# team-attention/nobs-whisper

Measured on AMD Instinct MI355X. Metric: audio-sec/s (RTF⁻¹) large-v3 greedy, batch 128; 1/2/4/8 MI355X, higher is better.
Workload: dtype bf16

## Files before the change

### include/whisper_mi355x.h

```cpp
#ifndef WHISPER_MI355X_H
#define WHISPER_MI355X_H

#include "whisper.h"

#ifdef __cplusplus
extern "C" {
#endif

#define WHISPER_MI355X_ERR_RUNTIME (-10)

enum whisper_mi355x_dtype { WHISPER_MI355X_F16 = 0, WHISPER_MI355X_BF16 = 1, WHISPER_MI355X_FP8_ENC = 2 };

WHISPER_API struct whisper_context * whisper_mi355x_init(const char * path_model, struct whisper_context_params params,
                                                         int dtype, bool load_weights);

WHISPER_API int whisper_mi355x_weight_arena(struct whisper_context * ctx, void ** dev_ptr, size_t * bytes);

WHISPER_API int whisper_mi355x_rccl_unique_id(char out[128]);
WHISPER_API int whisper_mi355x_broadcast_weights(struct whisper_context * ctx, const char unique_id[128], int rank, int world);

WHISPER_API int whisper_mi355x_full_batch(struct whisper_context * ctx, struct whisper_state * state,
                                          struct whisper_full_params params, const float * const * pcm,
                                          const int * n_samples, int n_jobs, bool pcm_on_device, int fixed_tokens);
WHISPER_API int whisper_mi355x_full_batch_forced(struct whisper_context * ctx, struct whisper_state * state,
                                                 struct whisper_full_params params, const float * const * pcm,
                                                 const int * n_samples, int n_jobs, bool pcm_on_device, int fixed_tokens,
                                                 const int * forced, const int * spot, int n_spot, float * spot_logits);
#define WHISPER_MI355X_BEAM_COMPLETED 1
#define WHISPER_MI355X_BEAM_FAILED 2
#define WHISPER_MI355X_BEAM_WINNER 4
WHISPER_API int whisper_mi355x_beam_info(struct whisper_state * state, int job, int beam, int * tokens, int cap,
                                         double * sum_logprobs_all, int * flags);
WHISPER_API int whisper_mi355x_cand_info(struct whisper_state * state, int job, int cand, int * tokens, int cap,
                                         double * sum_logprobs_all, int * flags);
WHISPER_API void whisper_mi355x_set_sample_seed(struct whisper_state * state, uint64_t seed);
WHISPER_API int whisper_mi355x_batch_n_segments(struct whisper_state * state, int job);
WHISPER_API const char * whisper_mi355x_batch_segment_text(struct whisper_state * state, int job, int i_segment);
WHISPER_API int64_t whisper_mi355x_batch_segment_t0(struct whisper_state * state, int job, int i_segment);
WHISPER_API int64_t whisper_mi355x_batch_segment_t1(struct whisper_state * state, int job, int i_segment);
WHISPER_API int whisper_mi355x_batch_segment_n_tokens(struct whisper_state * state, int job, int i_segment);
WHISPER_API whisper_token_data whisper_mi355x_batch_token_data(struct whisper_state * state, int job, int i_segment, int i_token);
WHISPER_API bool whisper_mi355x_batch_segment_speaker_turn_next(struct whisper_state * state, int job, int i_segment);
WHISPER_API int whisper_mi355x_batch_lang_id(struct whisper_state * state, int job);
WHISPER_API long whisper_mi355x_batch_decoded_tokens(struct whisper_state * state);
WHISPER_API long whisper_mi355x_decoded_tokens_total(void);
WHISPER_API void * whisper_mi355x_debug_ws(struct whisper_state * state, int which);

struct whisper_mi355x_window_decision {
    int32_t seek;
    int32_t temp_idx;
    int32_t failed0;
    int32_t logprob_fail0;
    int32_t result_len0;
    int32_t no_speech;
    float   avg_logprob0;
    float   entropy0;
    float   no_speech_prob;
    float   pad;
};
WHISPER_API int whisper_mi355x_window_decisions(struct whisper_state * state, int job,
                                                struct whisper_mi355x_window_decision * out, int cap);

WHISPER_API int whisper_mi355x_full_parallel(struct whisper_context * ctx, struct whisper_state * state,
                                             struct whisper_full_params params, const float * pcm, int n_samples,
                                             int n_processors, int snap_ms, bool pcm_on_device);
WHISPER_API int whisper_mi355x_parallel_cuts(struct whisper_state * state, int * cuts, int cap);

WHISPER_API int whisper_mi355x_phase_ms(struct whisper_state * state, double out[5]);

WHISPER_API double whisper_mi355x_align_ms(struct whisper_state * state);
WHISPER_API int whisper_mi355x_align_cost(struct whisper_state * state, int job, float * out, long cap_floats,
                                          int * rows, int * frames);

WHISPER_API double whisper_mi355x_token_times_ms(struct whisper_state * state);
struct whisper_mi355x_token_span {
    int64_t t0, t1;
    int32_t is_text, pad;
};
WHISPER_API int whisper_mi355x_debug_signal_energy(struct whisper_context * ctx, const float * pcm, const int * n_samples,
                                                   int n_clips, float * energy_out);
WHISPER_API int whisper_mi355x_debug_token_vad(struct whisper_context * ctx, const float * energy, const int * n_samples,
                                               int n_clips, const int * seg_clip, const int * seg_n_tokens, int n_segs,
                                               struct whisper_mi355x_token_span * spans);

WHISPER_API int whisper_mi355x_get_mel(struct whisper_state * state, float * out, int cap_floats);
WHISPER_API int whisper_mi355x_get_encoder_out(struct whisper_state * state, float * out, int cap_floats);
WHISPER_API int whisper_mi355x_set_audio_ctx(struct whisper_state * state, int audio_ctx);

WHISPER_API int whisper_mi355x_kernel_timing(struct whisper_state * state, int class_mask);
WHISPER_API int whisper_mi355x_kernel_stats(struct whisper_state * state, int cls, double out[3]);
#define WHISPER_MI355X_KSTAT_PDEC_GIVE_UPS 100
WHISPER_API long whisper_mi355x_pdec_give_ups(struct whisper_state * state);
#define WHISPER_MI355X_KSTAT_BEAM_GATHER 101
#define WHISPER_MI355X_KSTAT_VAD_FRONTEND 102
#define WHISPER_MI355X_KSTAT_VAD_LSTM 103
#define WHISPER_MI355X_KSTAT_VAD_GATHER 104
#define WHISPER_MI355X_KSTAT_LOGITS_STAGE 105

WHISPER_API int whisper_mi355x_debug_gemm(struct whisper_context * ctx, int epi, const void * A, int M, int K,
                                          const void * B, int N, const float * bias, void * out, int reps, float * ms);
WHISPER_API void whisper_mi355x_set_gemm_variant(int variant);
WHISPER_API void whisper_mi355x_set_gemm_stamps(void * dev);
WHISPER_API int whisper_mi355x_debug_gemm_small(struct whisper_context * ctx, int epi, const void * A, int M, int K,
                                                const void * B, int N, const float * bias, void * out,
                                                const float * ln_w, const float * ln_b, int reps, float * ms);
WHISPER_API int whisper_mi355x_debug_dequant(struct whisper_context * ctx, int type, const void * qs, const void * qh,
                                             const void * dm, long rows, int K, void * out);
WHISPER_API int whisper_mi355x_debug_dequant_multi(struct whisper_context * ctx, const int * type, int n,
                                                   const void * const * qs, const void * const * qh,
                                                   const void * const * dm, const long * rows, const int * K,
                                                   void * const * out);
WHISPER_API int whisper_mi355x_debug_gemm_small_q(struct whisper_context * ctx, int epi, const void * A, int M, int K,
                                                  int type, const void * qs, const void * qh, const void * dm, int N,
                                                  const float * bias, float scale, void * out, const float * ln_w,
                                                  const float * ln_b);
WHISPER_API void whisper_mi355x_set_dec_splits(int splits);
WHISPER_API void whisper_mi355x_set_dec_bm(int rows);
WHISPER_API void whisper_mi355x_set_pdec_spin(long ticks);
WHISPER_API void whisper_mi355x_set_pdec_stamps(void * dev);
WHISPER_API void whisper_mi355x_set_pdec_blocks(int on);
WHISPER_API int whisper_mi355x_debug_gemm_fp8(struct whisper_context * ctx, int epi, const void * A8,
                                              const float * a_scale, int M, int K, const void * B8,
                                              const float * b_scale, int N, const float * bias, void * out,
                                              int reps, float * ms);
WHISPER_API int whisper_mi355x_debug_gemm_w8(struct whisper_context * ctx, int epi, const void * A, int M, int K,
                                             const void * B8, const float * b_scale, int N, const float * bias,
                                             void * out, const float * ln_w, const float * ln_b, void * y);
WHISPER_API int whisper_mi355x_debug_quant_fp8(struct whisper_context * ctx, const void * x, long rows, int K,
                                               void * q, float * s);
WHISPER_API int whisper_mi355x_debug_attn_encoder(struct whisper_context * ctx, const void * qkv, int B, int T, int d,
                                                  int H, int variant, void * out, int reps, float * ms);
WHISPER_API int whisper_mi355x_debug_gemm_ln(struct whisper_context * ctx, const void * A, int M, int K,
                                             const void * B, int N, const float * bias, float * x,
                                             const float * ln_w, const float * ln_b, void * y, int reps, float * ms);

WHISPER_API int whisper_mi355x_debug_xattn(struct whisper_context * ctx, const void * enc, const int * slot,
                                           const void * q, const void * wkt, const void * wv, const float * bv,
                                           int n, int n_ctx, int d, float scale, int splits, float rescale_thr,
                                           void * out, int reps, float * ms);

WHISPER_API int whisper_mi355x_debug_attn_self_step(struct whisper_context * ctx, const float * slabs, int splits,
                                                    const float * bias, float scale, void * cache, const int * slot,
                                                    const int * pos, int n, int L, int layer, int H, int n_ctx,
                                                    void * out);
WHISPER_API int whisper_mi355x_debug_attn_cross_step(struct whisper_context * ctx, const float * slabs, int splits,
                                                     const float * bias, float scale, const void * cache,
                                                     const int * slot, const int * n_kv, int n, int L, int layer,
                                                     int H, int n_ctx, void * out);
WHISPER_API int whisper_mi355x_debug_attn_prefill(struct whisper_context * ctx, const void * q, int q_stride,
                                                  const void * cache, const int * slot, const int * n_kv,
                                                  const void * tiles, int n_tiles, int L, int layer, int H, int n_ctx,
                                                  void * out);

struct whisper_mi355x_cand {
    int32_t id, tid;
    float   p, plog, pt, ptsum, no_speech_prob, pad;
};
WHISPER_API int whisper_mi355x_debug_logits_topk(struct whisper_context * ctx, const float * logits, int n,
                                                 const int * rules, const float * temperature, int k, int split,
                                                 struct whisper_mi355x_cand * cand, struct whisper_mi355x_cand * greedy);
WHISPER_API int whisper_mi355x_debug_kv_gather(struct whisper_context * ctx, void * cache, int n_slots, int L, int H,
                                               int n_ctx, const int * copies, int n_copies, int * n_staged);

WHISPER_API int whisper_mi355x_debug_sample(struct whisper_context * ctx, const float * probs,
                                            const struct whisper_mi355x_cand * rec_in, int n, int n_vocab, uint64_t seed,
                                            const int * counters, const uint32_t * words, struct whisper_mi355x_cand * rec_out);

struct whisper_mi355x_seq_ctl {
    int32_t is_initial, last_ts, penult_ts, has_ts, seek_delta;
    float   temperature;
    int32_t suppress_blank, no_timestamps, suppress_eot, tid0_initial;
    int32_t want_probs, want_nosp;
};
WHISPER_API int whisper_mi355x_debug_logits(struct whisper_context * ctx, const float * logits, int n,
                                            const struct whisper_mi355x_seq_ctl * ctl, int form,
                                            struct whisper_mi355x_cand * out, float * probs);
WHISPER_API int whisper_mi355x_debug_decode_advance(struct whisper_context * ctx, int n, int ct, int beg,
                                                    const struct whisper_mi355x_cand * tout, int * ints,
                                                    struct whisper_mi355x_seq_ctl * ctl, const unsigned * err,
                                                    struct whisper_mi355x_cand * ring, unsigned * ring_err);

WHISPER_API int  whisper_mi355x_suppress_mask(struct whisper_context * ctx, bool suppress_nst, const char * regex,
                                              uint32_t * words, int cap_words);
WHISPER_API long whisper_mi355x_suppress_builds(struct whisper_context * ctx);
WHISPER_API int whisper_mi355x_debug_logits_deny(struct whisper_context * ctx, const float * logits, int n,
                                                 const struct whisper_mi355x_seq_ctl * ctl, int form,
                                                 struct whisper_mi355x_cand * out, float * probs, const uint32_t * deny);
WHISPER_API int whisper_mi355x_debug_logits_topk_deny(struct whisper_context * ctx, const float * logits, int n,
                                                      const int * rules, const float * temperature, int k, int split,
                                                      struct whisper_mi355x_cand * cand, struct whisper_mi355x_cand * greedy,
                                                      const uint32_t * deny);

WHISPER_API int whisper_mi355x_grammar_mask(struct whisper_context * ctx, const whisper_grammar_element ** rules,
                                            size_t n_rules, size_t i_start, const whisper_token * accepted_tokens,
                                            int n_accepted, uint32_t * words, int cap_words);
struct whisper_mi355x_grammar_stats { long rows_device, rows_patched, rows_host; double kernel_ms; long kernel_launches; };
WHISPER_API int whisper_mi355x_grammar_stats(struct whisper_state * state, struct whisper_mi355x_grammar_stats * out);
WHISPER_API int whisper_mi355x_debug_grammar_reject(struct whisper_context * ctx, const whisper_grammar_element ** rules,
                                                    size_t n_rules, size_t i_start, const whisper_token * accepted_tokens,
                                                    const int * n_accepted, int n_rows, uint32_t * words, int * flags);
WHISPER_API int whisper_mi355x_debug_logits_gram(struct whisper_context * ctx, const float * logits, int n,
                                                 const struct whisper_mi355x_seq_ctl * ctl, int form,
                                                 struct whisper_mi355x_cand * out, float * probs, const uint32_t * deny,
                                                 const uint32_t * gram, float penalty);
WHISPER_API int whisper_mi355x_debug_logits_topk_gram(struct whisper_context * ctx, const float * logits, int n,
                                                      const int * rules, const float * temperature, int k, int split,
                                                      struct whisper_mi355x_cand * cand, struct whisper_mi355x_cand * greedy,
                                                      const uint32_t * deny, const uint32_t * gram, float penalty);

WHISPER_API int whisper_mi355x_debug_logits_stage(struct whisper_context * ctx, const float * logits, int n,
                                                  const struct whisper_mi355x_seq_ctl * ctl, int flags, float * out_rows);
WHISPER_API int whisper_mi355x_debug_logits_ex(struct whisper_context * ctx, const float * raw, const float * filtered, int n,
                                               const struct whisper_mi355x_seq_ctl * ctl, int form, int flags,
                                               struct whisper_mi355x_cand * out, float * probs);
WHISPER_API int whisper_mi355x_debug_logits_topk_ex(struct whisper_context * ctx, const float * raw, const float * filtered,
                                                    int n, const struct whisper_mi355x_seq_ctl * ctl, int k, int split,
                                                    int flags, struct whisper_mi355x_cand * cand,
                                                    struct whisper_mi355x_cand * greedy);

struct whisper_vad_context;
WHISPER_API double whisper_mi355x_vad_ms(struct whisper_state * state);
WHISPER_API int whisper_mi355x_vad_map(struct whisper_state * state, int job, int * out, int cap);
WHISPER_API int whisper_mi355x_vad_probs_batch(struct whisper_vad_context * vctx, const float * const * pcm,
                                               const int * n_samples, int n_clips, bool pcm_on_device, float * probs_out,
                                               int * n_probs);
WHISPER_API int whisper_mi355x_debug_vad_frontend(struct whisper_vad_context * vctx, const float * pcm, int n_samples,
                                                  float * xg_out);
WHISPER_API int whisper_mi355x_debug_vad_gather(struct whisper_context * ctx, const float * const * pcm,
                                                const int * n_samples, int n_clips, const int * pieces,
                                                const int * n_pieces, float * out);

WHISPER_API int whisper_mi355x_debug_align_scores(struct whisper_context * ctx, const void * q, const void * cross,
                                                  int n_slots, int n_clips, const int * slot, const int * n_rows,
                                                  const int * frames, int n_heads, const int * head_layer,
                                                  const int * head_idx, float * P);
WHISPER_API int whisper_mi355x_debug_align_cost(struct whisper_context * ctx, const float * P, int n_clips,
                                                const int * n_rows, const int * n_sot, const int * frames, int n_heads,
                                                float * cost);
WHISPER_API int whisper_mi355x_debug_align_dtw(struct whisper_context * ctx, const float * cost, int n_clips,
                                               const int * rows, const int * frames, int * fr, int * path,
                                               int * path_len);

WHISPER_API int whisper_mi355x_find_silence_boundaries(int device, const float * const * pcm, const int * n_samples,
                                                       int n_clips, int sample_rate, bool pcm_on_device, int * counts,
                                                       int * boundaries, int cap, float * noise_floor, float * rms_out,
                                                       int rms_stride);
WHISPER_API int whisper_mi355x_resample_len(int n_in, int rate_in);
WHISPER_API int whisper_mi355x_resample_chunk(int device, const float * const * audio, const int * n_in, int n_clips,
                                              int rate_in, bool on_device, float * const * out);
WHISPER_API int whisper_mi355x_resample_operator(int rate_in, int * fsi, int * fso, float * W, long cap);

WHISPER_API int whisper_mi355x_abi_layout(size_t out[8]);

WHISPER_API int whisper_mi355x_state_info(struct whisper_state * state, int out[5]);

WHISPER_API void * whisper_mi355x_state_stream(struct whisper_state * state);

WHISPER_API void * whisper_mi355x_dev_alloc(struct whisper_context * ctx, size_t bytes);
WHISPER_API void   whisper_mi355x_dev_free(struct whisper_context * ctx, void * p);
WHISPER_API int    whisper_mi355x_memcpy(struct whisper_context * ctx, void * dst, const void * src, size_t bytes, int kind);

#ifdef __cplusplus
}
#endif

#endif
```

### nobs-whisper_amd/csrc/capi.cpp

```cpp
#include <cfloat>
#include <cmath>
#include <cstring>
#include <string>
#include <thread>
#include <vector>

#include <rccl/rccl.h>

#include "../../include/whisper_mi355x.h"
#include "engine.h"
#include "suppress.h"

namespace wm { extern int g_gemm_variant; extern int g_dec_splits; extern int g_dec_bm; extern unsigned long long* g_gemm_stamps; }
using namespace wm;

static Context* C(whisper_context* ctx) { return ctx ? &ctx->c : nullptr; }

template <typename F> static int guarded(whisper_state* s, F&& f) {
    try {
        return f();
    } catch (const wm::Error&) {
    } catch (const std::bad_alloc&) {
        fprintf(stderr, "whisper_mi355x: host out of memory\n");
    }
    if (s) recover_state(s);
    return WHISPER_MI355X_ERR_RUNTIME;
}

struct HookStream {
    hipStream_t st = nullptr;
    HookStream() { WM_CHECK(hipStreamCreate(&st)); }
    ~HookStream() { hipStreamDestroy(st); }
};
struct HookBufs {
    std::vector<void*> p;
    void* get(size_t bytes) {
        void* q = nullptr;
        WM_CHECK(hipMalloc(&q, bytes));
        p.push_back(q);
        return q;
    }
    ~HookBufs() { for (void* q : p) hipFree(q); }
};
struct HookEvent {
    hipEvent_t e = nullptr;
    HookEvent() { WM_CHECK(hipEventCreate(&e)); }
    ~HookEvent() { hipEventDestroy(e); }
};
template <typename F> static float timed_ms(hipStream_t st, int reps, bool warm, F run) {
    HookEvent e0, e1;
    if (warm) run();
    WM_CHECK(hipEventRecord(e0.e, st));
    for (int r = 0; r < reps; r++) run();
    WM_CHECK(hipEventRecord(e1.e, st));
    WM_CHECK(hipStreamSynchronize(st));
    float t = 0;
    WM_CHECK(hipEventElapsedTime(&t, e0.e, e1.e));
    return reps > 0 ? t / reps : 0.0f;
}

static DType env_dtype(DType def) {
    const char* e = getenv("WHISPER_MI355X_DTYPE");
    if (!e) return def;
    return (strcmp(e, "bf16") == 0 || strcmp(e, "BF16") == 0) ? DType::BF16 : DType::F16;
}

static whisper_context* make_ctx(const char* path, whisper_context_params cp, int dtype, bool load) {
    int n_dev = 0;
    if (hipGetDeviceCount(&n_dev) != hipSuccess || n_dev == 0) {
        fprintf(stderr, "whisper_mi355x: no HIP device available (this engine has no CPU path)\n");
        return nullptr;
    }
    const int dev = cp.gpu_device >= 0 && cp.gpu_device < n_dev ? cp.gpu_device : 0;
    whisper_context* w = new whisper_context();
    w->c.fp8_enc = dtype == 2;
    if (dtype == 2) dtype = (int)DType::BF16;
    bool ok = false;
    try {
        ok = load_context(&w->c, path, dev, (DType)dtype, load);
    } catch (const wm::Error&) {
    } catch (const std::bad_alloc&) {
    }
    if (!ok) {
        free_context(&w->c);
        delete w;
        return nullptr;
    }
    if (w->c.quant && w->c.fp8_enc) {
        fprintf(stderr, "whisper_mi355x: fp8 mode needs an f16 model file; %s is block-quantized, fp8 off\n", path);
        w->c.fp8_enc = false;
    }
    if (!resolve_dtw(&w->c, cp)) {
        free_context(&w->c);
        delete w;
        return nullptr;
    }
    w->c.owner = w;
    return w;
}

extern "C" {

const char* whisper_version(void) { return "1.7.6-mi355x"; }

struct whisper_context_params whisper_context_default_params(void) {
    whisper_context_params r;
    memset(&r, 0, sizeof(r));
    r.use_gpu = true;
    r.flash_attn = false;
    r.gpu_device = 0;
    r.dtw_token_timestamps = false;
    r.dtw_aheads_preset = WHISPER_AHEADS_NONE;
    r.dtw_n_top = -1;
    r.dtw_aheads.n_heads = 0;
    r.dtw_aheads.heads = nullptr;
    r.dtw_mem_size = 1024 * 1024 * 128;
    return r;
}
struct whisper_context_params* whisper_context_default_params_by_ref(void) {
    return new whisper_context_params(whisper_context_default_params());
}
void whisper_free_context_params(struct whisper_context_params* p) { delete p; }

struct whisper_full_params whisper_full_default_params(enum whisper_sampling_strategy strategy) {
    whisper_full_params r;
    memset(&r, 0, sizeof(r));
    r.strategy = strategy;
    r.n_threads = std::min(4, (int)std::thread::hardware_concurrency());
    r.n_max_text_ctx = 16384;
    r.offset_ms = 0;
    r.duration_ms = 0;
    r.translate = false;
    r.no_context = true;
    r.no_timestamps = false;
    r.single_segment = false;
    r.print_special = false;
    r.print_progress = true;
    r.print_realtime = false;
    r.print_timestamps = true;
    r.token_timestamps = false;
    r.thold_pt = 0.01f;
    r.thold_ptsum = 0.01f;
    r.max_len = 0;
    r.split_on_word = false;
    r.max_tokens = 0;
    r.debug_mode = false;
    r.audio_ctx = 0;
    r.tdrz_enable = false;
    r.suppress_regex = nullptr;
    r.initial_prompt = nullptr;
    r.prompt_tokens = nullptr;
    r.prompt_n_tokens = 0;
    r.language = "en";
    r.detect_language = false;
    r.suppress_blank = true;
    r.suppress_nst = false;
    r.temperature = 0.0f;
    r.max_initial_ts = 1.0f;
    r.length_penalty = -1.0f;
    r.temperature_inc = 0.2f;
    r.entropy_thold = 2.4f;
    r.logprob_thold = -1.0f;
    r.no_speech_thold = 0.6f;
    r.greedy.best_of = -1;
    r.beam_search.beam_size = -1;
    r.beam_search.patience = -1.0f;
// ... 266 lines not shown
float whisper_full_get_token_p_from_state(struct whisper_state* s, int i, int t) { return tdata(seg(s, 0, i), t).p; }
float whisper_full_get_token_p(struct whisper_context* ctx, int i, int t) { return tdata(seg(ctx->c.default_state, 0, i), t).p; }
float whisper_full_get_segment_no_speech_prob_from_state(struct whisper_state* s, int i) { auto g = seg(s, 0, i); return g ? g->no_speech_prob : 0.0f; }
float whisper_full_get_segment_no_speech_prob(struct whisper_context* ctx, int i) { return whisper_full_get_segment_no_speech_prob_from_state(ctx->c.default_state, i); }

int whisper_bench_memcpy(int) { return 0; }
const char* whisper_bench_memcpy_str(int) { return "whisper_mi355x: memcpy benchmark not implemented\n"; }
int whisper_bench_ggml_mul_mat(int) { return 0; }
const char* whisper_bench_ggml_mul_mat_str(int) { return "whisper_mi355x: ggml mul_mat benchmark not applicable (no ggml)\n"; }
void whisper_log_set(ggml_log_callback, void*) {}

struct whisper_context* whisper_mi355x_init(const char* path, struct whisper_context_params p, int dtype, bool load) {
    return make_ctx(path, p, dtype, load);
}
int whisper_mi355x_weight_arena(struct whisper_context* ctx, void** ptr, size_t* bytes) {
    if (!ctx) return -1;
    *ptr = ctx->c.arena;
    *bytes = ctx->c.arena_bytes;
    return 0;
}
int whisper_mi355x_rccl_unique_id(char out[128]) {
    ncclUniqueId id;
    if (ncclGetUniqueId(&id) != ncclSuccess) return -1;
    static_assert(sizeof(id) == 128, "ncclUniqueId size");
    memcpy(out, &id, 128);
    return 0;
}
int whisper_mi355x_broadcast_weights(struct whisper_context* ctx, const char uid[128], int rank, int world) {
    if (!ctx) return -1;
    if (world <= 1) return 0;
    hipSetDevice(ctx->c.device);
    ncclUniqueId id;
    memcpy(&id, uid, 128);
    ncclComm_t comm;
    if (ncclCommInitRank(&comm, world, id, rank) != ncclSuccess) return -2;
    hipStream_t st = nullptr;
    ncclResult_t r = ncclInternalError;
    const int rc = guarded(nullptr, [&] {
        WM_CHECK(hipStreamCreate(&st));
        r = ncclBroadcast(ctx->c.arena, ctx->c.arena, ctx->c.arena_bytes, ncclChar, 0, comm, st);
        WM_CHECK(hipStreamSynchronize(st));
        return 0;
    });
    if (st) hipStreamDestroy(st);
    ncclCommDestroy(comm);
    if (rc != 0) return rc;
    return r == ncclSuccess ? 0 : -3;
}

int whisper_mi355x_full_batch(struct whisper_context* ctx, struct whisper_state* s, struct whisper_full_params p,
                              const float* const* pcm, const int* n, int n_jobs, bool on_device, int fixed_tokens) {
    if (!ctx || !s || n_jobs <= 0 || fixed_tokens > ctx->c.hp.n_text_ctx / 2 - 4) return -1;
    FullOpts o;
    o.fixed_tokens = fixed_tokens;
    return guarded(s, [&] { return full_batch(&ctx->c, s, p, pcm, n, n_jobs, on_device, o, false); });
}
int whisper_mi355x_full_batch_forced(struct whisper_context* ctx, struct whisper_state* s, struct whisper_full_params p,
                                     const float* const* pcm, const int* n, int n_jobs, bool on_device, int fixed_tokens,
                                     const int* forced, const int* spot, int n_spot, float* spot_logits) {
    if (!ctx || !s || n_jobs <= 0 || fixed_tokens <= 0 || fixed_tokens > ctx->c.hp.n_text_ctx / 2 - 4 || !forced || n_spot < 0 ||
        (n_spot && (!spot || !spot_logits)))
        return -1;
    for (int k = 0; k < n_spot; k++)
        if (spot[k] < 0 || spot[k] >= n_jobs) return -1;
    FullOpts o;
    o.fixed_tokens = fixed_tokens;
    o.forced = forced;
    o.spot = spot;
    o.n_spot = n_spot;
    o.spot_logits = spot_logits;
    return guarded(s, [&] { return full_batch(&ctx->c, s, p, pcm, n, n_jobs, on_device, o, false); });
}
int whisper_mi355x_beam_info(struct whisper_state* s, int job, int beam, int* tokens, int cap, double* sum_logprobs_all,
                             int* flags) {
    if (!s || job < 0 || job >= (int)s->beam_info.size() || beam < 0 || beam >= (int)s->beam_info[job].size()) return -1;
    const whisper_state::BeamRec& r = s->beam_info[job][beam];
    for (int i = 0; tokens && i < cap && i < (int)r.tokens.size(); i++) tokens[i] = r.tokens[i];
    if (sum_logprobs_all) *sum_logprobs_all = r.sum_logprobs_all;
    if (flags) *flags = r.flags;
    return (int)r.tokens.size();
}
int whisper_mi355x_cand_info(struct whisper_state* s, int job, int cand, int* tokens, int cap, double* sum_logprobs_all,
                             int* flags) {
    if (!s || job < 0 || job >= (int)s->cand_info.size() || cand < 0 || cand >= (int)s->cand_info[job].size()) return -1;
    const whisper_state::BeamRec& r = s->cand_info[job][cand];
    for (int i = 0; tokens && i < cap && i < (int)r.tokens.size(); i++) tokens[i] = r.tokens[i];
    if (sum_logprobs_all) *sum_logprobs_all = r.sum_logprobs_all;
    if (flags) *flags = r.flags;
    return (int)r.tokens.size();
}
void whisper_mi355x_set_sample_seed(struct whisper_state* s, uint64_t seed) {
    if (s) s->sample_seed = seed;
}
int whisper_mi355x_batch_n_segments(struct whisper_state* s, int job) {
    return s && job >= 0 && job < (int)s->results.size() ? (int)s->results[job].size() : 0;
}
const char* whisper_mi355x_batch_segment_text(struct whisper_state* s, int job, int i) { auto g = seg(s, job, i); return g ? g->text.c_str() : nullptr; }
int64_t whisper_mi355x_batch_segment_t0(struct whisper_state* s, int job, int i) { auto g = seg(s, job, i); return g ? g->t0 : 0; }
int64_t whisper_mi355x_batch_segment_t1(struct whisper_state* s, int job, int i) { auto g = seg(s, job, i); return g ? g->t1 : 0; }
int whisper_mi355x_batch_segment_n_tokens(struct whisper_state* s, int job, int i) { auto g = seg(s, job, i); return g ? (int)g->tokens.size() : 0; }
whisper_token_data whisper_mi355x_batch_token_data(struct whisper_state* s, int job, int i, int t) { return tdata(seg(s, job, i), t); }
bool whisper_mi355x_batch_segment_speaker_turn_next(struct whisper_state* s, int job, int i) { auto g = seg(s, job, i); return g && g->speaker_turn_next; }
int whisper_mi355x_batch_lang_id(struct whisper_state* s, int job) {
    return s && job >= 0 && job < (int)s->lang_ids.size() ? s->lang_ids[job] : -1;
}
long whisper_mi355x_batch_decoded_tokens(struct whisper_state* s) { return s ? s->decoded_tokens : 0; }
int whisper_mi355x_window_decisions(struct whisper_state* s, int job, struct whisper_mi355x_window_decision* out, int cap) {
    if (!s || job < 0 || job >= (int)s->decisions.size()) return 0;
    const auto& d = s->decisions[job];
    if ((int)d.size() > cap) return -(int)d.size();
    for (size_t i = 0; i < d.size(); i++) out[i] = d[i];
    return (int)d.size();
}
int whisper_mi355x_phase_ms(struct whisper_state* s, double out[5]) {
    if (!s) return -1;
    for (int i = 0; i < 5; i++) out[i] = s->phase_ms[i];
    return 0;
}
double whisper_mi355x_align_ms(struct whisper_state* s) { return s ? s->align_ms : 0.0; }
int whisper_mi355x_align_cost(struct whisper_state* s, int job, float* out, long cap, int* rows, int* frames) {
    return guarded(nullptr, [&]() -> int {
        if (!s || job < 0 || job >= (int)s->align_info.size()) return -1;
        const whisper_state::AlignInfo& a = s->align_info[job];
        if (rows) *rows = a.rows;
        if (frames) *frames = a.frames;
        if (a.rows <= 0 || !a.cost) return 0;
        const long n = (long)a.rows * a.frames;
        if (!out || cap < n) return -2;
        hipSetDevice(s->device);
        WM_CHECK(hipMemcpy(out, a.cost, (size_t)n * sizeof(float), hipMemcpyDeviceToHost));
        return 0;
    });
}
int whisper_mi355x_get_mel(struct whisper_state* s, float* out, int cap) {
    return guarded(nullptr, [&]() -> int {
        if (!s || !s->ctx || !s->ws.mel) return -1;
        Context* c = s->ctx;
        const int nm = c->hp.n_mels, nl = s->n_len;
        if ((long)nm * nl > cap) return -nm * nl;
        hipSetDevice(c->device);
        int n_samp = 0;
        WM_CHECK(hipMemcpy(&n_samp, s->ws.n_samp, sizeof(int), hipMemcpyDeviceToHost));
        float* tmp;
        WM_CHECK(hipMalloc((void**)&tmp, (size_t)nm * nl * 4));
        launch_mel_normalize(s->ws.mel, nl, n_samp, s->ws.mel_max, nm, tmp, s->stream);
        WM_CHECK(hipMemcpyAsync(out, tmp, (size_t)nm * nl * 4, hipMemcpyDeviceToHost, s->stream));
        WM_CHECK(hipStreamSynchronize(s->stream));
        WM_CHECK(hipFree(tmp));
        return nl;
    });
}
int whisper_mi355x_get_encoder_out(struct whisper_state* s, float* out, int cap) {
    return guarded(nullptr, [&]() -> int {
        if (!s || !s->ctx || !s->ws.hn || s->last_enc_windows < 1) return -1;
        Context* c = s->ctx;
        const long n = (long)enc_ctx(c, s) * c->hp.n_audio_state;
        if (n > cap) return -1;
        hipSetDevice(c->device);
        std::vector<uint16_t> h(n);
        WM_CHECK(hipMemcpy(h.data(), s->ws.hn, n * 2, hipMemcpyDeviceToHost));
        for (long i = 0; i < n; i++) {
            if (c->dt == DType::F16) out[i] = h2f(h[i]);
            else { uint32_t u = (uint32_t)h[i] << 16; memcpy(&out[i], &u, 4); }
        }
        return 0;
    });
}
int whisper_mi355x_set_audio_ctx(struct whisper_state* s, int audio_ctx) {
    if (!s || !s->ctx) return -1;
    if (audio_ctx > s->ctx->hp.n_audio_ctx) return -5;
    s->audio_ctx = audio_ctx;
    return 0;
}
int whisper_mi355x_state_info(struct whisper_state* s, int out[5]) {
    if (!s || !out) return -1;
    out[0] = s->direct ? 1 : 0;
    out[1] = s->ws.cap_jobs;
    out[2] = s->ws.cap_cross;
    out[3] = (int)s->dec_graphs.size();
    out[4] = s->pooled ? 1 : 0;
    return 5;
}
void* whisper_mi355x_state_stream(struct whisper_state* s) { return s ? (void*)s->stream : nullptr; }
int whisper_mi355x_kernel_timing(struct whisper_state* s, int class_mask) {
    if (!s) return -1;
    s->ktime_mask = class_mask;
    for (auto& k : s->kstat) k = KStat();
    for (auto& k : s->vad_kstat) k = KStat();
    return 0;
}
int whisper_mi355x_kernel_stats(struct whisper_state* s, int cls, double out[3]) {
    if (s && cls == WHISPER_MI355X_KSTAT_PDEC_GIVE_UPS) {
        out[0] = s->pdec_lost_ms;
        out[1] = (double)s->pdec_give_ups;
        out[2] = 0.0;
        return 0;
    }
    if (s && cls == WHISPER_MI355X_KSTAT_BEAM_GATHER && s->ctx) {
        const Hparams& hp = s->ctx->hp;
        const double row_bytes = (double)hp.n_text_layer * 2 * hp.n_text_head * 128;
        out[0] = s->gather_rows * row_bytes;
        out[1] = s->gather_rows_full * row_bytes;
        out[2] = 0.0;
        return 0;
    }
    if (s && cls >= WHISPER_MI355X_KSTAT_VAD_FRONTEND && cls <= WHISPER_MI355X_KSTAT_VAD_GATHER) {
        const KStat& k = s->vad_kstat[cls - WHISPER_MI355X_KSTAT_VAD_FRONTEND];
        out[0] = k.ms; out[1] = (double)k.count; out[2] = k.work;
        return 0;
    }
    if (cls == WHISPER_MI355X_KSTAT_LOGITS_STAGE) cls = K_LOGITS_STAGE;
    if (!s || cls < 0 || cls >= K_NCLASS) return -1;
    out[0] = s->kstat[cls].ms;
    out[1] = (double)s->kstat[cls].count;
    out[2] = s->kstat[cls].work;
    return 0;
}

void whisper_mi355x_set_gemm_variant(int v) { wm::g_gemm_variant = v; }
void whisper_mi355x_set_gemm_stamps(void* dev) { wm::g_gemm_stamps = (unsigned long long*)dev; }
void whisper_mi355x_set_dec_splits(int splits) { wm::g_dec_splits = splits; }
void whisper_mi355x_set_dec_bm(int rows) { wm::g_dec_bm = rows; }
void whisper_mi355x_set_pdec_spin(long ticks) {
    wm::g_pdec_spin_ticks = ticks;
    wm::g_pdec_gen.fetch_add(1, std::memory_order_release);
}
void whisper_mi355x_set_pdec_stamps(void* dev) {
    wm::g_pdec_stamps = (unsigned long long*)dev;
    wm::g_pdec_gen.fetch_add(1, std::memory_order_release);
}
void* whisper_mi355x_debug_ws(struct whisper_state* s, int which) {
    if (!s) return nullptr;
    const wm::Workspace& w = s->ws;
    void* p[9] = {w.dx, w.dh, nullptr, w.datt, w.dff, w.dq, w.qx, w.xo, w.xml};
    return which >= 0 && which < 9 ? p[which] : nullptr;
}
long whisper_mi355x_decoded_tokens_total(void) { return wm::g_decoded_tokens_total.load(); }
long whisper_mi355x_pdec_give_ups(struct whisper_state* s) { return s ? s->pdec_give_ups : wm::g_pdec_give_ups_total.load(); }
void whisper_mi355x_set_pdec_blocks(int on) { wm::g_pdec_blocks = on != 0; }
int whisper_mi355x_debug_gemm(struct whisper_context* ctx, int epi, const void* A, int M, int K, const void* B, int N,
                              const float* bias, void* out, int reps, float* ms) {
    return guarded(nullptr, [&]() -> int {
        if (!ctx) return -1;
        const int T = ctx->c.hp.n_audio_ctx;
        if (epi == EPI_CROSSKV && (M % T != 0 || K % 64 != 0 || N % (2 * K) != 0)) return -1;
        hipSetDevice(ctx->c.device);
        HookBufs b;
        HookStream hs;
        GemmArgs g = gemm_plain(A, M, K, B, N, bias, out, N);
        if (M <= 128) {
            g.splitk_ws_elems = 64L * M * N;
            g.splitk_ws = (float*)b.get(g.splitk_ws_elems * sizeof(float));
        }
        if (epi == EPI_CROSSKV) {
            std::vector<int> slots(M / T);
            for (int i = 0; i < M / T; i++) slots[i] = i;
            int* dslot = (int*)b.get(slots.size() * sizeof(int));
            WM_CHECK(hipMemcpy(dslot, slots.data(), slots.size() * sizeof(int), hipMemcpyHostToDevice));
            g.cache = out; g.row_slot = dslot; g.d = K; g.H = K / 64; g.ctx = T; g.L = N / (2 * K); g.layer = 0;
        }
        const float t = timed_ms(hs.st, reps, true, [&] { launch_gemm(ctx->c.dt, epi, g, hs.st); });
        if (ms) *ms = t;
        return 0;
    });
}
int whisper_mi355x_debug_gemm_small(struct whisper_context* ctx, int epi, const void* A, int M, int K, const void* B,
                                    int N, const float* bias, void* out, const float* ln_w, const float* ln_b, int reps,
                                    float* ms) {
    return guarded(nullptr, [&]() -> int {
        if (!ctx || !gemm_small_ok(M, K, ln_w != nullptr)) return -1;
        hipSetDevice(ctx->c.device);
        HookStream hs;
        GemmArgs g = gemm_plain(A, M, K, B, N, bias, out, N);
        g.a_ln_w = ln_w; g.a_ln_b = ln_b;
        const float t = timed_ms(hs.st, reps, true, [&] { launch_gemm_small(ctx->c.dt, epi, g, ln_w != nullptr, hs.st); });
        if (ms) *ms = t;
        return 0;
    });
}
static bool debug_qmat(QMat* q, int type, const void* qs, const void* qh, const void* dm) {
    const bool known = type == 2 || type == 3 || type == 6 || type == 7 || type == 8;
    if (!known || !qs || !dm || ((type == 6 || type == 7) && !qh)) return false;
    q->type = type;
    q->qs = (const uint8_t*)qs;
    q->qh = (const uint32_t*)qh;
    q->dm = (const uint16_t*)dm;
    return true;
}
int whisper_mi355x_debug_dequant(struct whisper_context* ctx, int type, const void* qs, const void* qh, const void* dm,
                                 long rows, int K, void* out) {
    return guarded(nullptr, [&]() -> int {
        QMat q;
        if (!ctx || !out || rows < 1 || K < 1 || !debug_qmat(&q, type, qs, qh, dm)) return -1;
        hipSetDevice(ctx->c.device);
        launch_dequant(ctx->c.dt, q, rows, K, out, nullptr);
        WM_CHECK(hipDeviceSynchronize());
        return 0;
    });
}
int whisper_mi355x_debug_dequant_multi(struct whisper_context* ctx, const int* type, int n, const void* const* qs,
                                       const void* const* qh, const void* const* dm, const long* rows, const int* K,
                                       void* const* out) {
    return guarded(nullptr, [&]() -> int {
        if (!ctx || !type || !qs || !qh || !dm || !rows || !K || !out || n < 1 || n > 6) return -1;
        DequantJobs J;
        J.n = n;
        for (int j = 0; j < n; j++) {
            if (!out[j] || rows[j] < 1 || K[j] < 1 || !debug_qmat(&J.q[j], type[j], qs[j], qh[j], dm[j])) return -1;
            J.rows[j] = rows[j];
            J.K[j] = K[j];
            J.out[j] = out[j];
        }
        hipSetDevice(ctx->c.device);
        launch_dequant_multi(ctx->c.dt, J, nullptr);
        WM_CHECK(hipDeviceSynchronize());
        return 0;
    });
}
int whisper_mi355x_debug_gemm_small_q(struct whisper_context* ctx, int epi, const void* A, int M, int K, int type,
                                      const void* qs, const void* qh, const void* dm, int N, const float* bias,
                                      float scale, void* out, const float* ln_w, const float* ln_b) {
    return guarded(nullptr, [&]() -> int {
        QMat q;
        if (!ctx || !A || !out || N < 1 || !gemm_small_ok(M, K, ln_w != nullptr) || (ln_w && !ln_b) ||
            !debug_qmat(&q, type, qs, qh, dm))
            return -1;
        hipSetDevice(ctx->c.device);
        HookStream hs;
        GemmArgs g = gemm_plain(A, M, K, nullptr, N, bias, out, N);
        g.q = q;
        g.sc_div = N; g.sc_mod = 1; g.sc_lim = 1; g.scale = scale;
        g.a_ln_w = ln_w; g.a_ln_b = ln_b;
        launch_gemm_small(ctx->c.dt, epi, g, ln_w != nullptr, hs.st);
        WM_CHECK(hipStreamSynchronize(hs.st));
        return 0;
    });
}
int whisper_mi355x_debug_gemm_fp8(struct whisper_context* ctx, int epi, const void* A8, const float* a_scale, int M,
                                  int K, const void* B8, const float* b_scale, int N, const float* bias, void* out,
                                  int reps, float* ms) {
    return guarded(nullptr, [&]() -> int {
        if (!ctx) return -1;
        hipSetDevice(ctx->c.device);
        HookStream hs;
        const GemmArgs g = gemm_plain(A8, M, K, B8, N, bias, out, N);
        const float t = timed_ms(hs.st, reps, true, [&] { launch_gemm_fp8(ctx->c.dt, epi, g, a_scale, b_scale, hs.st); });
        if (ms) *ms = t;
        return 0;
    });
}
int whisper_mi355x_debug_gemm_w8(struct whisper_context* ctx, int epi, const void* A, int M, int K, const void* B8,
                                 const float* b_scale, int N, const float* bias, void* out, const float* ln_w,
                                 const float* ln_b, void* y) {
    return guarded(nullptr, [&]() -> int {
        if (!ctx || !b_scale || M < 1 || M > 128 || K % 64 || (epi == EPI_RESID && (!ln_w || !y))) return -1;
        hipSetDevice(ctx->c.device);
        HookBufs b;
        HookStream hs;
        GemmArgs g = gemm_plain(A, M, K, B8, N, bias, out, N);
        g.w8_scale = b_scale;
        if (epi == EPI_RESID) { g.ln_w = ln_w; g.ln_b = ln_b; g.ln_out = y; }
        g.splitk_ws_elems = 16L * M * N;
        g.splitk_ws = (float*)b.get(g.splitk_ws_elems * sizeof(float));
        launch_gemm(ctx->c.dt, epi, g, hs.st);
        WM_CHECK(hipStreamSynchronize(hs.st));
        return 0;
    });
}
int whisper_mi355x_debug_quant_fp8(struct whisper_context* ctx, const void* x, long rows, int K, void* q, float* s) {
    return guarded(nullptr, [&]() -> int {
        if (!ctx) return -1;
        hipSetDevice(ctx->c.device);
        launch_quant_rows_fp8(ctx->c.dt, x, rows, K, q, s, nullptr);
        WM_CHECK(hipDeviceSynchronize());
        return 0;
// ... 862 lines not shown
```

### nobs-whisper_amd/csrc/engine.cpp

```cpp
#include <optional>
#include <algorithm>
#include <chrono>
#include <cmath>
#include <cstring>
#include <exception>
#include <thread>

#include "engine.h"
#include "suppress.h"
#include "token_times.h"

namespace wm {

static size_t esize(DType) { return 2; }

static void dfree(void*& p) {
    if (p) { void* q = p; p = nullptr; WM_CHECK(hipFree(q)); }
}
template <typename T> static void dfree(T*& p) {
    void* q = (void*)p;
    p = nullptr;
    dfree(q);
}
template <typename T> static void dalloc(T*& p, size_t bytes) {
    void* q = nullptr;
    p = nullptr;
    WM_CHECK(hipMalloc(&q, bytes));
    p = (T*)q;
}

static hipEvent_t kt_event(whisper_state* s) {
    if (!s->kpool.empty()) { hipEvent_t e = s->kpool.back(); s->kpool.pop_back(); return e; }
    hipEvent_t e;
    WM_CHECK(hipEventCreate(&e));
    return e;
}
static void kt_record(whisper_state* s, hipEvent_t e, hipStream_t st) {
    if (!s->capture_ev) { WM_CHECK(hipEventRecord(e, st)); return; }
    hipStreamCaptureStatus cs;
    unsigned long long id = 0;
    hipGraph_t g = nullptr;
    const hipGraphNode_t* deps = nullptr;
    size_t nd = 0;
    WM_CHECK(hipStreamGetCaptureInfo_v2(st, &cs, &id, &g, &deps, &nd));
    hipGraphNode_t node;
    WM_CHECK(hipGraphAddEventRecordNode(&node, g, deps, nd, e));
    WM_CHECK(hipStreamUpdateCaptureDependencies(st, &node, 1, hipStreamSetCaptureDependencies));
}
struct KT {
    whisper_state* s;
    int cls;
    double work;
    hipStream_t st;
    hipEvent_t a = nullptr;
    int sub = 0;
    KT(whisper_state* s_, int c, double w, hipStream_t st_ = nullptr, bool on = true)
        : s(s_), cls(c), work(w), st(st_ ? st_ : s_->stream) {
        if (on && ((s->ktime_mask >> c) & 1)) { a = kt_event(s); kt_record(s, a, st); }
    }
    ~KT() {
        if (!a) return;
        hipEvent_t b = kt_event(s);
        kt_record(s, b, st);
        (s->capture_ev ? *s->capture_ev : s->kpending).push_back({cls, a, b, work, sub});
    }
};
static void drop_graphs(whisper_state* s) {
    for (auto& g : s->dec_graphs) {
        hipGraphExecDestroy(g.exec);
        for (auto& e : g.ev) { hipEventDestroy(e.a); hipEventDestroy(e.b); }
    }
    s->dec_graphs.clear();
}
static void kt_flush_graph(whisper_state* s, const whisper_state::DecGraph& g) {
    for (auto& p : g.ev) {
        if (!((s->ktime_mask >> p.cls) & 1)) continue;
        float ms = 0.0f;
        const hipError_t e = hipEventElapsedTime(&ms, p.a, p.b);
        if (e != hipSuccess) {
            static bool warned = false;
            if (!warned) fprintf(stderr, "whisper_mi355x: graph kernel timing unavailable (%s)\n", hipGetErrorString(e));
            warned = true;
            continue;
        }
        s->kstat[p.cls].ms += ms;
        s->kstat[p.cls].work += p.cls == K_ATTN_SELF ? s->cur_self_work * p.work : p.work;
        s->kstat[p.cls].count++;
    }
}
void kt_flush(whisper_state* s) {
    if (s->kpending.empty()) return;
    WM_CHECK(hipStreamSynchronize(s->stream));
    for (auto& p : s->kpending) {
        float ms = 0.0f;
        WM_CHECK(hipEventElapsedTime(&ms, p.a, p.b));
        s->kstat[p.cls].ms += ms;
        s->kstat[p.cls].work += p.cls == K_ATTN_SELF ? s->cur_self_work * p.work : p.work;
        s->kstat[p.cls].count++;
        if (p.cls == K_VAD) {
            s->vad_kstat[p.sub].ms += ms;
            s->vad_kstat[p.sub].work += p.work;
            s->vad_kstat[p.sub].count++;
        }
        s->kpool.push_back(p.a);
        s->kpool.push_back(p.b);
    }
    s->kpending.clear();
}
static void tgemm_ws(whisper_state* s, int cls, DType dt, int epi, const GemmArgs& g0, hipStream_t st, float* ws,
                     long ws_elems) {
    GemmArgs g = g0;
    if (cls == K_GEMM_DEC) { g.splitk_ws = ws; g.splitk_ws_elems = ws_elems; g.slab_wt = 1; }
    const double work = cls == K_GEMM_ENC ? 2.0 * g.M * g.N * g.K
                                          : 2.0 * g.N * g.K + 2.0 * g.M * g.K + 4.0 * g.M * g.N;
    KT kt(s, cls, work, st);
    launch_gemm(dt, epi, g, st);
}
static void tgemm(whisper_state* s, int cls, DType dt, int epi, const GemmArgs& g0, hipStream_t st) {
    tgemm_ws(s, cls, dt, epi, g0, st, s->ws.splitk, s->ws.splitk_elems);
}

static whisper_state* create_state(Context* c) {
    WM_CHECK(hipSetDevice(c->device));
    whisper_state* s = new whisper_state();
    s->ctx = c;
    s->device = c->device;
    try {
        WM_CHECK(hipStreamCreateWithFlags(&s->stream, hipStreamNonBlocking));
        WM_CHECK(hipStreamCreateWithFlags(&s->stream2, hipStreamNonBlocking));
        WM_CHECK(hipEventCreateWithFlags(&s->ev_fork, hipEventDisableTiming));
        WM_CHECK(hipEventCreateWithFlags(&s->ev_join, hipEventDisableTiming));
    } catch (...) {
        if (s->ev_join) hipEventDestroy(s->ev_join);
        if (s->ev_fork) hipEventDestroy(s->ev_fork);
        if (s->stream2) hipStreamDestroy(s->stream2);
        if (s->stream) hipStreamDestroy(s->stream);
        delete s;
        throw;
    }
    std::lock_guard<std::mutex> lk(c->pool_mu);
    c->live.push_back(s);
    return s;
}

static void reset_for_reuse(whisper_state* s) {
    s->direct = false;
    s->results.clear();
    s->lang_ids.clear();
    s->decisions.clear();
    s->prompt_past.clear();
    s->rng = std::mt19937(0);
    s->lang_id = 0;
    s->audio_ctx = 0;
    s->n_len = s->n_len_org = 0;
    s->logits_host.clear();
    for (double& t : s->phase_ms) t = 0;
    s->align_ms = 0;
    s->tokts_ms = 0;
    s->vad_ms = 0;
    s->vad_maps.clear();
    s->align_info.clear();
    s->decoded_tokens = 0;
    s->last_enc_windows = 0;
    s->mel_ready = false;
    s->ktime_mask = 0;
    for (auto& k : s->kstat) k = KStat();
    for (auto& k : s->vad_kstat) k = KStat();
    s->cur_self_work = 0;
    s->pdec_give_ups = 0;
    s->pdec_lost_ms = 0;
    s->pdec_off_until = 0;
    s->pdec_off = false;
    s->mode = StepMode{};
    s->deny_on = false;
    s->gram_on = false;
    s->filter_on = s->tdrz_on = false;
    s->ws.gd.host_masks.clear();
    s->ws.gd.rows_device = s->ws.gd.rows_patched = s->ws.gd.rows_host = 0;
    s->beam_info.clear();
    s->sample_seed = 0;
    s->cand_info.clear();
    s->gather_rows = s->gather_rows_full = 0;
    std::fill(s->ws.cross_fresh.begin(), s->ws.cross_fresh.end(), 0);
}

static int pool_states() {
    const char* e = getenv("WHISPER_MI355X_STATE_POOL");
    return e ? std::max(0, atoi(e)) : 2;
}
static const int kPoolMaxJobs = 16;

whisper_state* new_state(Context* c) {
    {
        std::lock_guard<std::mutex> lk(c->pool_mu);
        if (!c->pool.empty()) {
            whisper_state* s = c->pool.back();
            c->pool.pop_back();
            reset_for_reuse(s);
            s->pooled = true;
            return s;
        }
    }
    return create_state(c);
}

static void free_ws(Workspace& w);

static void destroy_state(whisper_state* s) {
    if (s->twin) {
        destroy_state(s->twin);
        s->twin = nullptr;
    }
    if (Context* c = s->ctx) {
        std::lock_guard<std::mutex> lk(c->pool_mu);
        c->live.erase(std::remove(c->live.begin(), c->live.end(), s), c->live.end());
    }
    hipSetDevice(s->device);
    hipStreamSynchronize(s->stream);
    hipStreamSynchronize(s->stream2);
    drop_graphs(s);
    try { free_ws(s->ws); } catch (const Error&) {}
    for (auto& p : s->kpending) { hipEventDestroy(p.a); hipEventDestroy(p.b); }
    for (hipEvent_t e : s->kpool) hipEventDestroy(e);
    hipEventDestroy(s->ev_fork);
    hipEventDestroy(s->ev_join);
    hipStreamDestroy(s->stream2);
    hipStreamDestroy(s->stream);
    delete s;
}

void free_state(whisper_state* s) {
    if (!s) return;
    Context* c = s->ctx;
    if (!c) {
        destroy_state(s);
        return;
    }
    hipSetDevice(c->device);
    const bool healthy = hipStreamSynchronize(s->stream) == hipSuccess && hipStreamSynchronize(s->stream2) == hipSuccess &&
                         s->kpending.empty();
    if (healthy && s->ws.cap_jobs <= kPoolMaxJobs) {
        std::lock_guard<std::mutex> lk(c->pool_mu);
        if ((int)c->pool.size() < pool_states()) {
            c->pool.push_back(s);
            return;
        }
    }
    destroy_state(s);
}

void drain_state_pool(Context* c) {
    std::vector<whisper_state*> p;
    {
        std::lock_guard<std::mutex> lk(c->pool_mu);
        p.swap(c->pool);
    }
    for (whisper_state* s : p) destroy_state(s);
}

void orphan_states(Context* c) {
    std::lock_guard<std::mutex> lk(c->pool_mu);
    for (whisper_state* s : c->live) s->ctx = nullptr;
    c->live.clear();
}

void recover_state(whisper_state* s) {
    if (!s) return;
    hipSetDevice(s->device);
    for (hipStream_t st : {s->stream, s->stream2}) {
        hipStreamCaptureStatus cs = hipStreamCaptureStatusNone;
        if (hipStreamIsCapturing(st, &cs) == hipSuccess && cs != hipStreamCaptureStatusNone) {
            hipGraph_t g = nullptr;
            hipStreamEndCapture(st, &g);
            if (g) hipGraphDestroy(g);
        }
    }
    s->capture_ev = nullptr;
    s->mode = StepMode{};
    hipStreamSynchronize(s->stream);
    hipStreamSynchronize(s->stream2);
    (void)hipGetLastError();
    for (auto& p : s->kpending) { s->kpool.push_back(p.a); s->kpool.push_back(p.b); }
    s->kpending.clear();
}

static void free_align(Workspace& w) {
    dfree(w.al_clips); dfree(w.al_P); dfree(w.al_stats); dfree(w.al_cost); dfree(w.al_trace); dfree(w.al_fr);
    if (w.h_al) { char* q = w.h_al; w.h_al = nullptr; WM_CHECK(hipHostFree(q)); }
    w.al_P_elems = 0;
    w.al_cap = w.al_rows = 0;
}

static void free_ws(Workspace& w) {
    free_align(w);
    dfree(w.mel_img); dfree(w.h1); dfree(w.hn); dfree(w.qkv); dfree(w.att); dfree(w.ff); dfree(w.x);
    dfree(w.cross); dfree(w.self); dfree(w.dx); dfree(w.dh); dfree(w.dq); dfree(w.datt); dfree(w.dff);
    dfree(w.lrow); dfree(w.logits); dfree(w.probs); dfree(w.tok); dfree(w.ctl); dfree(w.tout); dfree(w.lrec); dfree(w.win_job);
    dfree(w.pcm); dfree(w.mel); dfree(w.mel_ptrs); dfree(w.splitk); dfree(w.enc); dfree(w.qx); dfree(w.xo);
    dfree(w.xml); dfree(w.kvslot); dfree(w.hs); dfree(w.qtiles); dfree(w.wdq); dfree(w.pd_sync);
    dfree(w.sslot); dfree(w.cand); dfree(w.kvcp); dfree(w.kvstage); dfree(w.sctr);
    dfree(w.energy); dfree(w.tt_clips); dfree(w.tt_segs); dfree(w.tt_spans); dfree(w.deny); dfree(w.gram);
    if (w.h_gram) hipHostFree(w.h_gram);
    dfree(w.frows);
    if (w.h_frows) hipHostFree(w.h_frows);
    gram_dev_free(w.gd);
    vad_scratch_free(w.vad);
    if (w.h_sslot) hipHostFree(w.h_sslot);
    if (w.h_sctr) hipHostFree(w.h_sctr);
    if (w.h_cand) hipHostFree(w.h_cand);
    if (w.h_kvcp) hipHostFree(w.h_kvcp);
    if (w.h_pd_err) hipHostFree(w.h_pd_err);
    if (w.h_ring) hipHostFree(w.h_ring);
    for (auto& e : w.ring_ev)
        if (e) hipEventDestroy(e);
    if (w.h_ints) hipHostFree(w.h_ints);
    if (w.h_qtiles) hipHostFree(w.h_qtiles);
    if (w.h_tout) hipHostFree(w.h_tout);
    if (w.h_ctl) hipHostFree(w.h_ctl);
    w = Workspace();
}

static const int kXDirectMaxTok = 8;
static const float kXattnThr = 8.0f;

static bool pick_direct(Context* c, int n_jobs) {
    if (!c->cross_direct) return false;
    const char* e = getenv("WHISPER_MI355X_CROSS");
    if (e && strcmp(e, "direct") == 0) return true;
    if (e && strcmp(e, "cache") == 0) return false;
    return n_jobs > 32;
}

static int enc_batch() {
    static const int v = getenv("WHISPER_MI355X_ENC_BATCH") ? std::max(1, atoi(getenv("WHISPER_MI355X_ENC_BATCH"))) : 128;
    return v;
}

static void ensure_cross(Context* c, whisper_state* s, int slots) {
    Workspace& w = s->ws;
    if (w.cross && w.cap_cross >= slots) return;
    const Hparams& hp = c->hp;
    WM_CHECK(hipStreamSynchronize(s->stream));
    WM_CHECK(hipStreamSynchronize(s->stream2));
    drop_graphs(s);
    dfree(w.cross);
    w.cap_cross = 0;
    std::fill(w.cross_fresh.begin(), w.cross_fresh.end(), 0);
    dalloc(w.cross, (size_t)slots * hp.n_text_layer * 2 * hp.n_audio_ctx * hp.n_audio_state * esize(c->dt));
    w.cap_cross = slots;
}

static void ensure_ws_impl(Context* c, whisper_state* s, int n_jobs, int n_clips) {
    Workspace& w = s->ws;
    const Hparams& hp = c->hp;
    const size_t d = hp.n_audio_state, nm = hp.n_mels, T = hp.n_audio_ctx, E = esize(c->dt);
    const int n_enc = std::min(n_clips, enc_batch());
    if (n_enc > w.cap_enc || n_jobs > w.cap_jobs) drop_graphs(s);
    if (!w.deny) dalloc(w.deny, (size_t)suppress_words(hp.n_vocab) * sizeof(uint32_t));
    if (n_enc > w.cap_enc) {
        dfree(w.mel_img); dfree(w.h1); dfree(w.hn); dfree(w.qkv); dfree(w.att); dfree(w.ff); dfree(w.x);
        dfree(w.win_job); dfree(w.hs);
        w.cap_enc = 0;
        dalloc(w.mel_img, (size_t)n_enc * 3002 * nm * E);
        dalloc(w.h1, (size_t)n_enc * 3002 * d * E);
        WM_CHECK(hipMemset(w.h1, 0, (size_t)n_enc * 3002 * d * E));
        dalloc(w.hn, (size_t)n_enc * T * d * E);
        dalloc(w.qkv, (size_t)n_enc * T * 3 * d * E);
        dalloc(w.att, (size_t)n_enc * T * d * E);
        dalloc(w.ff, (size_t)n_enc * T * 4 * d * E);
        dalloc(w.x, (size_t)n_enc * T * d * 4);
        if (c->fp8_enc) {
            dalloc(w.hs, (size_t)n_enc * T * sizeof(float));
        }
        dalloc(w.win_job, (size_t)n_enc * 3 * sizeof(int));
        w.win_seek = w.win_job + n_enc;
        w.win_slot = w.win_job + 2 * n_enc;
        w.cap_enc = n_enc;
    }
    if (n_jobs > w.cap_jobs) {
        const int L = hp.n_text_layer;
        const int n_tok = n_jobs * (hp.n_text_ctx / 2 + 8);
        dfree(w.cross); dfree(w.self); dfree(w.dx); dfree(w.dh); dfree(w.dq); dfree(w.datt); dfree(w.dff);
        dfree(w.lrow); dfree(w.logits); dfree(w.probs); dfree(w.tok); dfree(w.ctl); dfree(w.tout); dfree(w.lrec); dfree(w.mel_ptrs);
        dfree(w.splitk); dfree(w.enc); dfree(w.qx); dfree(w.xo); dfree(w.xml); dfree(w.kvslot); dfree(w.qtiles);
        free_align(w);
        for (auto& a : s->align_info) a = {};
        if (w.h_ring) { WM_CHECK(hipHostFree(w.h_ring)); w.h_ring = nullptr; w.ring = nullptr; }
        dfree(w.sslot); dfree(w.cand); dfree(w.kvcp); dfree(w.sctr); dfree(w.gram);
        dfree(w.frows);
        for (void** h : {(void**)&w.h_qtiles, (void**)&w.h_ints, (void**)&w.h_tout, (void**)&w.h_ctl, (void**)&w.h_sslot,
                         (void**)&w.h_cand, (void**)&w.h_kvcp, (void**)&w.h_sctr, (void**)&w.h_gram, (void**)&w.h_frows})
            if (*h) { void* q = *h; *h = nullptr; WM_CHECK(hipHostFree(q)); }
        w.cap_jobs = w.cap_tok = w.cap_cross = w.cap_xq = 0;
        w.splitk_elems = std::max(16L * std::min(n_tok, 256) * 4 * (long)d, std::min(16384L * n_tok, 12L << 22));
        dalloc(w.splitk, w.splitk_elems * 4);
        w.cross_fresh.assign(n_jobs, 0);
        {
            std::vector<int> ident(n_jobs);
            for (int k = 0; k < n_jobs; k++) ident[k] = k;
            dalloc(w.kvslot, (size_t)n_jobs * sizeof(int));
            WM_CHECK(hipMemcpy(w.kvslot, ident.data(), (size_t)n_jobs * sizeof(int), hipMemcpyHostToDevice));
        }
        dalloc(w.self, (size_t)n_jobs * L * 2 * hp.n_text_ctx * d * E);
        dalloc(w.dx, (size_t)n_tok * d * 4);
        dalloc(w.dh, (size_t)n_tok * d * E);
        dalloc(w.dq, (size_t)n_tok * d * E);
        dalloc(w.datt, (size_t)n_tok * d * E);
        dalloc(w.dff, (size_t)n_tok * 4 * d * E);
        dalloc(w.lrow, (size_t)n_jobs * d * E);
        dalloc(w.logits, (size_t)n_jobs * hp.n_vocab * 4);
        dalloc(w.probs, (size_t)n_jobs * 2 * hp.n_vocab * 4);
        dalloc(w.tok, ((size_t)5 * n_tok + n_jobs) * sizeof(int));
        w.pos = w.tok + n_tok;
        w.slot = w.tok + 2 * n_tok;
        w.nkv_self = w.tok + 3 * n_tok;
        w.nkv_cross = w.tok + 4 * n_tok;
        w.lrows = w.tok + 5 * n_tok;
        dalloc(w.ctl, (size_t)n_jobs * sizeof(SeqCtl));
        dalloc(w.tout, (size_t)n_jobs * sizeof(TokOut));
        dalloc(w.lrec, logits_rec_bytes(n_jobs));
        dalloc(w.mel_ptrs, (size_t)n_jobs * (2 * sizeof(void*) + 3 * sizeof(int)));
        w.pcm_ptrs = (const float**)(w.mel_ptrs + n_jobs);
        w.n_samp = (int*)(w.pcm_ptrs + n_jobs);
        w.n_len = w.n_samp + n_jobs;
        w.mel_max = w.n_len + n_jobs;
        WM_CHECK(hipHostMalloc((void**)&w.h_ints, ((size_t)5 * n_tok + n_jobs) * sizeof(int) + 64, 0));
        dalloc(w.qtiles, (size_t)n_tok * sizeof(int2));
        WM_CHECK(hipHostMalloc((void**)&w.h_qtiles, (size_t)n_tok * sizeof(int2), 0));
        WM_CHECK(hipHostMalloc((void**)&w.h_tout, (size_t)n_jobs * sizeof(TokOut), 0));
        WM_CHECK(hipHostMalloc((void**)&w.h_ctl, (size_t)n_jobs * sizeof(SeqCtl), 0));
        dalloc(w.sslot, (size_t)n_jobs * sizeof(int));
        dalloc(w.cand, (size_t)n_jobs * kTopkMax * sizeof(TokOut));
        dalloc(w.kvcp, (size_t)n_jobs * sizeof(KvCopy));
        WM_CHECK(hipHostMalloc((void**)&w.h_sslot, (size_t)n_jobs * sizeof(int), 0));
        WM_CHECK(hipHostMalloc((void**)&w.h_cand, (size_t)n_jobs * kTopkMax * sizeof(TokOut), 0));
        WM_CHECK(hipHostMalloc((void**)&w.h_kvcp, (size_t)n_jobs * sizeof(KvCopy), 0));
        dalloc(w.sctr, (size_t)n_jobs * 4 * sizeof(int));
        WM_CHECK(hipHostMalloc((void**)&w.h_sctr, (size_t)n_jobs * 4 * sizeof(int), 0));
        dalloc(w.gram, (size_t)n_jobs * grammar_words(hp.n_vocab) * sizeof(uint32_t));
        WM_CHECK(hipHostMalloc((void**)&w.h_gram, (size_t)n_jobs * grammar_words(hp.n_vocab) * sizeof(uint32_t), 0));
        w.cap_jobs = n_jobs;
        w.cap_tok = n_tok;
    }
    if (s->direct && !w.enc) {
        const int H = hp.n_text_head;
        w.cap_xq = std::max(kXDirectMaxTok * w.cap_jobs, 128);
        const size_t xo_rows = (size_t)std::max(w.cap_xq, 512) + w.cap_jobs + 512;
        dalloc(w.enc, (size_t)w.cap_jobs * T * d * E);
        dalloc(w.qx, (size_t)w.cap_xq * 2 * H * d * E);
        dalloc(w.xo, xo_rows * H * d * 4);
        dalloc(w.xml, xo_rows * H * 2 * 4);
    }
    if (!s->direct) ensure_cross(c, s, n_clips);
    if (c->quant && !w.wdq) dalloc(w.wdq, (size_t)16 * d * d * E);
}

static void ensure_ws(Context* c, whisper_state* s, int n_jobs, int n_clips = -1) {
    try {
        ensure_ws_impl(c, s, n_jobs, n_clips < 0 ? n_jobs : n_clips);
    } catch (const Error&) {
        hipStreamSynchronize(s->stream);
        hipStreamSynchronize(s->stream2);
        drop_graphs(s);
        free_ws(s->ws);
        throw;
    }
}

static inline int mel_n_len(int n) { return (n + 16000 * 30) / 160; }
static inline int mel_n_len_org(int n) { return 1 + (int)(((int64_t)n + 200 - 400) / 160); }

int compute_mel(Context* c, whisper_state* s, const float* const* pcm, const int* n, int n_jobs, bool on_device) {
    s->direct = pick_direct(c, n_jobs);
    ensure_ws(c, s, n_jobs);
    Workspace& w = s->ws;
    const int nm = c->hp.n_mels;
    size_t pcm_tot = 0, mel_tot = 0;
    int max_frames = 1;
    for (int j = 0; j < n_jobs; j++) {
        pcm_tot += ((size_t)n[j] + 63) & ~(size_t)63;
        mel_tot += (size_t)nm * mel_n_len(n[j]);
        max_frames = std::max(max_frames, std::min((n[j] + 200) / 160 + 1, mel_n_len(n[j])));
    }
    if (!on_device && pcm_tot > w.cap_pcm) {
        dfree(w.pcm);
        w.cap_pcm = 0;
        dalloc(w.pcm, pcm_tot * 4);
        w.cap_pcm = pcm_tot;
    }
    if (mel_tot > w.cap_mel) {
        dfree(w.mel);
        w.cap_mel = 0;
        dalloc(w.mel, mel_tot * 4);
        w.cap_mel = mel_tot;
    }
    std::vector<const float*> pp(n_jobs);
    std::vector<float*> mp(n_jobs);
    std::vector<int> ints(3 * n_jobs);
    size_t po = 0, mo = 0;
    for (int j = 0; j < n_jobs; j++) {
        if (on_device) pp[j] = pcm[j];
        else {
            pp[j] = w.pcm + po;
            if (n[j] > 0) WM_CHECK(hipMemcpyAsync(w.pcm + po, pcm[j], (size_t)n[j] * 4, hipMemcpyHostToDevice, s->stream));
            po += ((size_t)n[j] + 63) & ~(size_t)63;
        }
        mp[j] = w.mel + mo;
        mo += (size_t)nm * mel_n_len(n[j]);
        ints[j] = n[j];
        ints[n_jobs + j] = mel_n_len(n[j]);
    }
    const size_t cap = w.cap_jobs;
    std::vector<char> blk(cap * (2 * sizeof(void*) + 2 * sizeof(int)));
    memcpy(blk.data(), mp.data(), n_jobs * sizeof(void*));
    memcpy(blk.data() + cap * sizeof(void*), pp.data(), n_jobs * sizeof(void*));
    memcpy(blk.data() + 2 * cap * sizeof(void*), ints.data(), n_jobs * sizeof(int));
    memcpy(blk.data() + 2 * cap * sizeof(void*) + cap * sizeof(int), ints.data() + n_jobs, n_jobs * sizeof(int));
    WM_CHECK(hipMemcpyAsync(w.mel_ptrs, blk.data(), blk.size(), hipMemcpyHostToDevice, s->stream));
    {
        double bytes = 0;
        for (int j = 0; j < n_jobs; j++)
            bytes += 4.0 * n[j] + 4.0 * nm * std::min((n[j] + 200) / 160 + 1, mel_n_len(n[j]));
        KT kt(s, K_MEL, bytes);
        launch_mel(w.pcm_ptrs, w.n_samp, c->w.mel_tab, c->w.filt_t, nm, w.mel_ptrs, w.n_len, w.mel_max, n_jobs, max_frames,
                   s->stream);
    }
    WM_CHECK(hipStreamSynchronize(s->stream));
    s->n_len = mel_n_len(n[0]);
    s->n_len_org = mel_n_len_org(n[0]);
    s->mel_ready = true;
    return 0;
}

template <typename T> static void tt_grow(T*& p, int& cap, size_t need) {
    if ((size_t)cap >= need) return;
    dfree(p);
// ... 58 lines not shown
        f.s2 = (float*)p; p += d * sizeof(float);
        launch_quant_rows_fp8(c->dt, L.wqkv, 3 * d, (int)d, f.wqkv, f.sqkv, nullptr);
        launch_quant_rows_fp8(c->dt, L.w1, 4 * d, (int)d, f.w1, f.s1, nullptr);
        launch_quant_rows_fp8(c->dt, L.w2, d, (int)(4 * d), f.w2, f.s2, nullptr);
    }
    c->dec8.assign(nd, Context::Fp8Dec{});
    for (size_t l = 0; l < nd; l++) {
        Context::Fp8Dec& f = c->dec8[l];
        const LayerW& L = c->w.dec[l];
        auto q = [&](const void* w, size_t rows, size_t cols, void*& q8, float*& sc) {
            q8 = p; p += rows * cols;
            sc = (float*)p; p += rows * sizeof(float);
            launch_quant_rows_fp8(c->dt, w, (long)rows, (int)cols, q8, sc, nullptr);
        };
        q(L.wqkv, 3 * t, t, f.wqkv, f.sqkv);
        q(L.wo, t, t, f.wo, f.so);
        q(L.wxq, t, t, f.wxq, f.sxq);
        q(L.wxo, t, t, f.wxo, f.sxo);
        q(L.w1, 4 * t, t, f.w1, f.s1);
        q(L.w2, t, 4 * t, f.w2, f.s2);
    }
    WM_CHECK(hipDeviceSynchronize());
    c->fp8_ready = true;
}

static void tgemm_fp8(whisper_state* s, int epi, const GemmArgs& g, const float* sa, const float* sb, hipStream_t st) {
    KT kt(s, K_GEMM_ENC, 2.0 * g.M * g.N * g.K, st);
    launch_gemm_fp8(s->ctx->dt, epi, g, sa, sb, st);
}

static int enc_gelu_epi(DType dt) { return dt == DType::BF16 ? EPI_GELU_F : EPI_GELU; }

using LayerMats = Context::LayerMats;
static char* dequant_layer(Context* c, const LayerW& L, char* p, LayerMats& m, hipStream_t st) {
    const int d = c->hp.n_audio_state;
    const size_t E = esize(c->dt);
    DequantJobs J;
    bool one_type = true;
    auto one = [&](const QMat& q, long rows, int K, const void*& dst) {
        if (!q.type) return;
        if (J.n && q.type != J.q[0].type) one_type = false;
        J.q[J.n] = q; J.rows[J.n] = rows; J.K[J.n] = K; J.out[J.n] = p; J.n++;
        dst = p;
        p += (size_t)rows * K * E;
    };
    one(L.qqkv, 3L * d, d, m.wqkv);
    one(L.qo, d, d, m.wo);
    one(L.qxq, d, d, m.wxq);
    one(L.qxo, d, d, m.wxo);
    one(L.q1, 4L * d, d, m.w1);
    one(L.q2, d, 4 * d, m.w2);
    if (one_type) launch_dequant_multi(c->dt, J, st);
    else
        for (int j = 0; j < J.n; j++) launch_dequant(c->dt, J.q[j], J.rows[j], J.K[j], J.out[j], st);
    return p;
}

static void ensure_expanded(Context* c, hipStream_t st) {
    if (!c->quant || c->expanded.load(std::memory_order_acquire)) return;
    hipStreamCaptureStatus cs = hipStreamCaptureStatusNone;
    WM_CHECK(hipStreamIsCapturing(st, &cs));
    if (cs != hipStreamCaptureStatusNone) return;
    std::lock_guard<std::mutex> lk(c->exp_mu);
    if (c->expanded.load(std::memory_order_relaxed)) return;
    const size_t d = c->hp.n_audio_state;
    dalloc(c->arena_exp, (12 * c->w.enc.size() + 14 * c->w.dec.size()) * d * d * esize(c->dt));
    char* p = c->arena_exp;
    auto fill = [&](const std::vector<LayerW>& layers, std::vector<LayerMats>& out) {
        out.resize(layers.size());
        for (size_t l = 0; l < layers.size(); l++) {
            const LayerW& L = layers[l];
            out[l] = LayerMats{L.wqkv, L.wo, L.wxq, L.wxo, L.w1, L.w2};
            p = dequant_layer(c, L, p, out[l], st);
        }
    };
    fill(c->w.enc, c->exp_enc);
    fill(c->w.dec, c->exp_dec);
    WM_CHECK(hipStreamSynchronize(st));
    c->expanded.store(true, std::memory_order_release);
}

static LayerMats layer_mats(Context* c, whisper_state* s, bool dec, int l, hipStream_t st) {
    const LayerW& L = dec ? c->w.dec[l] : c->w.enc[l];
    LayerMats m{L.wqkv, L.wo, L.wxq, L.wxo, L.w1, L.w2};
    if (!c->quant) return m;
    ensure_expanded(c, st);
    if (c->expanded.load(std::memory_order_acquire)) return dec ? c->exp_dec[l] : c->exp_enc[l];
    dequant_layer(c, L, (char*)s->ws.wdq, m, st);
    return m;
}

int encode_windows(Context* c, whisper_state* s, const int* jobs, const int* seeks, const int* slots, int n_win) {
    const Hparams& hp = c->hp;
    Workspace& w = s->ws;
    const int d = hp.n_audio_state, nm = hp.n_mels, T = enc_ctx(c, s), H = hp.n_audio_head;
    const DType dt = c->dt;
    const size_t E = esize(dt);
    const int KCLS = K_GEMM_ENC;
    const Weights& W = c->w;
    hipStream_t st = s->stream;
    const bool fp8 = c->fp8_enc && d % 128 == 0;
    if (fp8) ensure_fp8(c);
    for (int b0 = 0; b0 < n_win; b0 += w.cap_enc) {
        const int nb = std::min(w.cap_enc, n_win - b0);
        int* hi = w.h_ints;
        for (int i = 0; i < nb; i++) { hi[i] = jobs[b0 + i]; hi[nb + i] = seeks[b0 + i]; hi[2 * nb + i] = slots[b0 + i]; }
        WM_CHECK(hipMemcpyAsync(w.win_job, hi, 3 * nb * sizeof(int), hipMemcpyHostToDevice, st));
        const int* d_job = w.win_job;
        const int* d_seek = w.win_job + nb;
        const int* d_slot = w.win_job + 2 * nb;
        launch_mel_window(dt, w.mel_ptrs, w.n_len, w.n_samp, w.mel_max, d_job, d_seek, nb, nm, 2 * T, w.mel_img, st);
        {
            GemmArgs g = gemm_plain(w.mel_img, nb * 2 * T, 3 * nm, W.conv1_w, d, W.conv1_b, w.h1, d);
            g.a_rpb = 2 * T; g.a_bstride = (long)3002 * nm; g.a_rstride = nm;
            g.o_rpb = 2 * T; g.o_bstride = 3002; g.o_off = 1;
            tgemm(s, KCLS, dt, EPI_GELU, g, st);
        }
        {
            GemmArgs g = gemm_plain(w.h1, nb * T, 3 * d, W.conv2_w, d, W.conv2_b, w.x, d);
            g.a_rpb = T; g.a_bstride = (long)3002 * d; g.a_rstride = 2 * d;
            g.pos = W.pos_e; g.pos_rows = T;
            tgemm(s, KCLS, dt, EPI_GELU_POS, g, st);
        }
        const int M = nb * T;
        for (int l = 0; l < hp.n_audio_layer; l++) {
            const LayerW& L = W.enc[l];
            if (fp8) {
                const Context::Fp8Layer& F = c->enc8[l];
                launch_layernorm_fp8(w.x, M, d, L.ln1_w, L.ln1_b, w.hn, w.hs, st);
                tgemm_fp8(s, EPI_STORE, gemm_plain(w.hn, M, d, F.wqkv, 3 * d, L.bqkv, w.qkv, 3 * d), w.hs, F.sqkv, st);
                {
                    KT kt(s, K_ATTN_ENC, 4.0 * nb * H * (double)T * T * 64);
                    launch_attn_encoder(dt, w.qkv, w.att, nb, T, d, H, st);
                }
                tgemm(s, KCLS, dt, EPI_RESID, gemm_plain(w.att, M, d, L.wo, d, L.bo, w.x, d), st);
                launch_layernorm_fp8(w.x, M, d, L.ln2_w, L.ln2_b, w.hn, w.hs, st);
                tgemm_fp8(s, EPI_GELU_F, gemm_plain(w.hn, M, d, F.w1, 4 * d, L.b1, w.ff, 4 * d), w.hs, F.s1, st);
                launch_quant_rows_fp8(dt, w.ff, M, 4 * d, w.qkv, w.hs, st);
                tgemm_fp8(s, EPI_RESID, gemm_plain(w.qkv, M, 4 * d, F.w2, d, L.b2, w.x, d), w.hs, F.s2, st);
                continue;
            }
            const LayerMats Wm = layer_mats(c, s, false, l, st);
            launch_layernorm(dt, w.x, nullptr, M, d, L.ln1_w, L.ln1_b, w.hn, st);
            tgemm(s, KCLS, dt, EPI_STORE, gemm_plain(w.hn, M, d, Wm.wqkv, 3 * d, L.bqkv, w.qkv, 3 * d), st);
            {
                KT kt(s, K_ATTN_ENC, 4.0 * nb * H * (double)T * T * 64);
                launch_attn_encoder(dt, w.qkv, w.att, nb, T, d, H, st);
            }
            tgemm(s, KCLS, dt, EPI_RESID, gemm_plain(w.att, M, d, Wm.wo, d, L.bo, w.x, d), st);
            launch_layernorm(dt, w.x, nullptr, M, d, L.ln2_w, L.ln2_b, w.hn, st);
            tgemm(s, KCLS, dt, enc_gelu_epi(dt), gemm_plain(w.hn, M, d, Wm.w1, 4 * d, L.b1, w.ff, 4 * d), st);
            tgemm(s, KCLS, dt, EPI_RESID, gemm_plain(w.ff, M, 4 * d, Wm.w2, d, L.b2, w.x, d), st);
        }
        launch_layernorm(dt, w.x, nullptr, M, d, W.lnpost_w, W.lnpost_b, w.hn, st);
        if (s->direct) {
            for (int k = 0; k < nb; k++) {
                WM_CHECK(hipMemcpyAsync((char*)w.enc + (size_t)slots[b0 + k] * T * d * E, (const char*)w.hn + (size_t)k * T * d * E,
                                        (size_t)T * d * E, hipMemcpyDeviceToDevice, st));
                w.cross_fresh[slots[b0 + k]] = 0;
            }
        } else {
            GemmArgs g = gemm_plain(w.hn, M, d, W.wkv_cross, 2 * hp.n_text_layer * d, W.bkv_cross, nullptr, 0);
            g.scale = c->k_scale;
            g.cache = w.cross; g.row_slot = d_slot; g.L = hp.n_text_layer; g.H = hp.n_text_head; g.ctx = hp.n_audio_ctx; g.d = d;
            g.rpw = T;
            tgemm(s, KCLS, dt, EPI_CROSSKV, g, st);
            for (int k = 0; k < nb; k++) w.cross_fresh[slots[b0 + k]] = 1;
        }
        WM_CHECK(hipStreamSynchronize(st));
    }
    s->last_enc_windows = n_win;
    return 0;
}

static void decoder_upload(Context* c, whisper_state* s, int n_tok, int n_rows, bool tiles) {
    const Hparams& hp = c->hp;
    Workspace& w = s->ws;
    int* hi = w.h_ints;
    const int ct = w.cap_tok;
    double self_kv = 0;
    for (int i = 0; i < n_tok; i++) {
        hi[3 * ct + i] = hi[ct + i] + 1;
        hi[4 * ct + i] = enc_ctx(c, s);
        self_kv += hi[ct + i] + 1;
    }
    s->cur_self_work = self_kv * hp.n_text_head * 64 * 2 * 2;
    WM_CHECK(hipMemcpyAsync(w.tok, hi, ((size_t)5 * ct + n_rows) * sizeof(int), hipMemcpyHostToDevice, s->stream));
    if (!tiles) return;
    int nt = 0;
    for (int i = 0; i < n_tok; i++) {
        const bool cont = i > 0 && hi[2 * ct + i] == hi[2 * ct + i - 1] && hi[ct + i] > hi[ct + i - 1] &&
                          w.h_qtiles[nt - 1].y < 64;
        if (cont) w.h_qtiles[nt - 1].y++;
        else w.h_qtiles[nt++] = make_int2(i, 1);
    }
    w.n_qtiles = nt;
    WM_CHECK(hipMemcpyAsync(w.qtiles, w.h_qtiles, (size_t)nt * sizeof(int2), hipMemcpyHostToDevice, s->stream));
}

struct DecView {
    int r0, n;
    hipStream_t st;
    float* splitk;
    long splitk_elems;
    float *xo, *xml;
};

static int small_m_max() {
    const char* e = getenv("WHISPER_MI355X_SMALLM");
    if (!e) return 4;
    const int v = atoi(e);
    return v == 1 ? 32 : std::max(0, std::min(32, v));
}

static int quant_small_max() {
    const char* e = getenv("WHISPER_MI355X_QSMALL_MAX");
    return e ? atoi(e) : 32;
}

static int pdec_max() {
    const char* e = getenv("WHISPER_MI355X_PDEC");
    return e ? std::max(0, std::min(kPdecMaxRows, atoi(e))) : kPdecMaxRows;
}

static int small_rows_max(Context* c) { return c->quant ? std::max(quant_small_max(), small_m_max()) : small_m_max(); }

static bool dec_fp8(Context* c) { return c->fp8_enc && !c->dec8.empty(); }

static int dec_path_sig() {
    return small_m_max() | (std::min(std::max(quant_small_max(), 0), 1023) << 6) |
           (std::min(std::max(attn_cross_wide_max(), 0), 1023) << 16) | (pdec_max() << 26) | ((g_pdec_blocks & 1) << 29);
}

static bool pdec_blocks(Context* c) {
    return c->quant && (g_pdec_blocks || !c->expanded.load(std::memory_order_acquire));
}

static bool pdec_use(Context* c, whisper_state* s, int n, bool xdirect) {
    if (xdirect || s->pdec_off || s->mode.split_slots || n < 1 || n > pdec_max()) return false;
    if (dec_fp8(c)) return false;
    const bool quant = c->w.dec[0].qqkv.type != 0;
    for (const LayerW& L : c->w.dec)
        for (const QMat* q : {&L.qqkv, &L.qo, &L.qxq, &L.qxo, &L.q1, &L.q2})
            if ((q->type != 0) != quant) return false;
    const bool blocks = pdec_blocks(c);
    if (blocks && c->dt != DType::F16) return false;
    if (!pdec_supported(c->hp.n_text_state, c->hp.n_text_head, blocks)) return false;
    static const int cus = [] {
        int dev = 0, v = 0;
        hipGetDevice(&dev);
        hipDeviceGetAttribute(&v, hipDeviceAttributeMultiprocessorCount, dev);
        return v;
    }();
    return cus == 256;
}

static int dec_groups(int n_tok) { return cdiv(n_tok, 128); }

enum StepPath { STEP_PDEC, STEP_SMALL, STEP_SPLITK };
struct StepPlan {
    int n;
    int groups, gsz;
    StepPath path, tail_path;
    bool xdirect;
    bool w8;
    bool pdec_ok;
    bool pipe;
};
static StepPlan step_plan(Context* c, whisper_state* s, int n, bool xdirect, bool pdec_ok = true) {
    StepPlan P{};
    P.n = n; P.groups = dec_groups(n); P.gsz = cdiv(n, P.groups);
    P.xdirect = xdirect; P.w8 = dec_fp8(c); P.pdec_ok = pdec_ok;
    const int d = c->hp.n_text_state;
    const bool pd = pdec_ok && pdec_use(c, s, n, xdirect);
    auto path = [&](int rows) {
        if (pd) return STEP_PDEC;
        const bool small = !P.w8 && !s->mode.split_slots && rows <= small_rows_max(c) && gemm_small_ok(rows, d, true) &&
                           gemm_small_ok(rows, 4 * d, false);
        return small ? STEP_SMALL : STEP_SPLITK;
    };
    P.path = path(P.gsz);
    P.tail_path = P.groups == 1 ? P.path : path(n - (P.groups - 1) * P.gsz);
    return P;
}

static const PdecLayer* pdec_layers(Context* c, bool blocks) {
    std::lock_guard<std::mutex> lk(c->pdec_mu);
    void*& slot = blocks || !c->quant ? c->pdec_layers : c->pdec_layers_exp;
    if (!slot) {
        std::vector<PdecLayer> h(c->hp.n_text_layer);
        for (int l = 0; l < c->hp.n_text_layer; l++) {
            const LayerW& L = c->w.dec[l];
            LayerMats m{L.wqkv, L.wo, L.wxq, L.wxo, L.w1, L.w2};
            if (c->quant && !blocks) m = c->exp_dec[l];
            auto mat = [&](const void* w, const QMat& q) {
                return q.type && blocks ? PdecMat{q.qs, q.qh, q.dm, q.type} : PdecMat{w, nullptr, nullptr, 0};
            };
            h[l] = PdecLayer{mat(m.wqkv, L.qqkv), mat(m.wo, L.qo), mat(m.wxq, L.qxq), mat(m.wxo, L.qxo), mat(m.w1, L.q1),
                             mat(m.w2, L.q2), L.bqkv, L.bo, L.bxq, L.bxo, L.b1, L.b2,
                             L.ln1_w, L.ln1_b, L.lnx_w, L.lnx_b, L.ln2_w, L.ln2_b};
        }
        void* p = nullptr;
        WM_CHECK(hipMalloc(&p, h.size() * sizeof(PdecLayer)));
        WM_CHECK(hipMemcpy(p, h.data(), h.size() * sizeof(PdecLayer), hipMemcpyHostToDevice));
        slot = p;
    }
    return (const PdecLayer*)slot;
}

static void pdec_prepare(Context* c, whisper_state* s) {
    Workspace& w = s->ws;
    pdec_layers(c, pdec_blocks(c));
    if (w.pd_sync) return;
    dalloc(w.pd_sync, pdec_granules(c->hp.n_text_state, c->hp.n_text_layer, c->hp.n_text_head).bytes);
// ... 2455 lines not shown
```

### nobs-whisper_amd/csrc/engine.h

```cpp
#pragma once
#include <map>
#include <memory>
#include <atomic>
#include <cstring>
#include <mutex>
#include <random>
#include <string>
#include <unordered_map>
#include <vector>

#include "../../include/whisper_mi355x.h"
#include "beam.h"
#include "common.h"
#include "grammar.h"
#include "kernels.h"
#include "parallel.h"
#include "vad.h"

namespace wm {

struct Hparams {
    int32_t n_vocab, n_audio_ctx, n_audio_state, n_audio_head, n_audio_layer;
    int32_t n_text_ctx, n_text_state, n_text_head, n_text_layer, n_mels, ftype;
};
// ... 104 lines not shown
    GramTable gram_tab{};
    void* gram_tab_mem[4] = {nullptr, nullptr, nullptr, nullptr};
    std::mutex vad_mu;
    std::string vad_path;
    std::shared_ptr<VadModel> vad;
};

struct GramDev {
    GramElem* elems = nullptr;
    int* rule_off = nullptr;
    size_t cap_elems = 0, cap_rules = 0;
    GramRow *rows = nullptr, *h_rows = nullptr;
    unsigned *over = nullptr, *h_over = nullptr;
    int cap_rows = 0;
    std::unordered_map<std::string, std::vector<uint32_t>> host_masks;
    long rows_device = 0, rows_patched = 0, rows_host = 0;
};
void gram_dev_free(GramDev& d);
void gram_dev_rules(GramDev& d, const GrammarRules& g, hipStream_t st);
void gram_masks(Context* c, GramDev& d, const GrammarRules& g, const Grammar* const* states, int n, uint32_t* gram,
                uint32_t* h_stage, int* flags, hipStream_t st, whisper_state* s);

struct TokenData {
    int id, tid;
    float p, plog, pt, ptsum;
    int64_t t_dtw = -1;
    int64_t t0 = -1, t1 = -1;
    float vlen = 0.0f;
};
inline whisper_token_data token_data(const TokenData& x) {
    whisper_token_data r;
    memset(&r, 0, sizeof(r));
    r.id = x.id; r.tid = x.tid; r.p = x.p; r.plog = x.plog; r.pt = x.pt; r.ptsum = x.ptsum;
    r.t0 = x.t0; r.t1 = x.t1; r.t_dtw = x.t_dtw; r.vlen = x.vlen;
    return r;
}

struct Segment {
    int64_t t0, t1;
    std::string text;
    float no_speech_prob;
    std::vector<TokenData> tokens;
    bool speaker_turn_next = false;
};

struct Workspace {
    int cap_jobs = 0, cap_enc = 0, cap_tok = 0;
    int cap_cross = 0;
    size_t cap_mel = 0, cap_pcm = 0;
    void *mel_img = nullptr, *h1 = nullptr, *hn = nullptr, *qkv = nullptr, *att = nullptr, *ff = nullptr;
    float* x = nullptr;
    float* hs = nullptr;
    void *cross = nullptr, *self = nullptr;
    std::vector<char> cross_fresh;
    int* kvslot = nullptr;
    void* wdq = nullptr;
    void *enc = nullptr, *qx = nullptr;
    float *xo = nullptr, *xml = nullptr;
    int cap_xq = 0;
    float* dx = nullptr;
    void *dh = nullptr, *dq = nullptr, *datt = nullptr, *dff = nullptr, *lrow = nullptr;
    float *logits = nullptr, *probs = nullptr;
    float* splitk = nullptr;
    long splitk_elems = 0;
    int *tok = nullptr, *pos = nullptr, *slot = nullptr, *nkv_self = nullptr, *nkv_cross = nullptr, *lrows = nullptr;
    SeqCtl* ctl = nullptr;
    TokOut* tout = nullptr;
    void* lrec = nullptr;
    uint32_t* deny = nullptr;
    bool deny_held = false;
    Context::DenyKey deny_key;
    uint32_t* gram = nullptr;
    uint32_t* h_gram = nullptr;
    GramDev gd;
    float *frows = nullptr, *h_frows = nullptr;
    int *win_job = nullptr, *win_seek = nullptr, *win_slot = nullptr;
    unsigned* pd_sync = nullptr;
    unsigned* h_pd_err = nullptr;
    char* ring = nullptr;
    char* h_ring = nullptr;
    hipEvent_t ring_ev[2] = {nullptr, nullptr};
    int *sslot = nullptr, *h_sslot = nullptr;
    int *sctr = nullptr, *h_sctr = nullptr;
    TokOut *cand = nullptr, *h_cand = nullptr;
    KvCopy *kvcp = nullptr, *h_kvcp = nullptr;
    void* kvstage = nullptr;
    long kvstage_units = 0;
    float* pcm = nullptr;
    float* mel = nullptr;
    float** mel_ptrs = nullptr;
    const float** pcm_ptrs = nullptr;
    int *n_samp = nullptr, *n_len = nullptr, *mel_max = nullptr;
    int* h_ints = nullptr;
    int2* qtiles = nullptr;
    int2* h_qtiles = nullptr;
    int n_qtiles = 0;
    TokOut* h_tout = nullptr;
    SeqCtl* h_ctl = nullptr;
    AlignClip* al_clips = nullptr;
    float *al_P = nullptr, *al_stats = nullptr, *al_cost = nullptr;
    size_t al_P_elems = 0;
    unsigned char* al_trace = nullptr;
    int* al_fr = nullptr;
    char* h_al = nullptr;
    int al_cap = 0, al_rows = 0;
    float* energy = nullptr;
    size_t cap_energy = 0;
    TtClip* tt_clips = nullptr;
    TtSeg* tt_segs = nullptr;
    TtSpan* tt_spans = nullptr;
    int tt_cap_clips = 0, tt_cap_segs = 0, tt_cap_spans = 0;
    VadScratch vad;
};

enum KClass { K_GEMM_ENC = 0, K_ATTN_ENC, K_ATTN_CROSS, K_ATTN_SELF, K_GEMM_DEC, K_LOGITS, K_MEL, K_PDEC, K_OTHER,
              K_ALIGN_SCORES, K_ALIGN_COST, K_ALIGN_DTW, K_TOPK, K_KV_GATHER, K_SAMPLE, K_TOKTS, K_GRAMMAR, K_VAD, K_LOGITS_STAGE, K_NCLASS };
struct KStat { double ms = 0, work = 0; long count = 0; };

struct StepMode {
    int topk = 0;
    bool split_slots = false, sample = false;
    int key() const { return topk | (split_slots ? 1 << 8 : 0) | (sample ? 1 << 9 : 0); }
};

}

struct whisper_state {
    wm::Context* ctx = nullptr;
    int device = 0;
    hipStream_t stream = nullptr;
    hipStream_t stream2 = nullptr;
    hipEvent_t ev_fork = nullptr, ev_join = nullptr;
    wm::Workspace ws;
    bool direct = false;
    std::vector<std::vector<wm::Segment>> results;
    std::vector<int> lang_ids;
    std::vector<std::vector<whisper_mi355x_window_decision>> decisions;
    std::vector<int> prompt_past;
    std::mt19937 rng{0};
    int lang_id = 0;
    int n_len = 0, n_len_org = 0;
    int audio_ctx = 0;
    std::vector<float> logits_host;
    double phase_ms[5] = {0, 0, 0, 0, 0};
    double align_ms = 0;
    double tokts_ms = 0;
    double vad_ms = 0;
    std::vector<std::vector<wm::VadPiece>> vad_maps;
    std::vector<int> par_cuts;
    struct AlignInfo { int rows = 0, frames = 0; const float* cost = nullptr; };
    std::vector<AlignInfo> align_info;
    long decoded_tokens = 0;
    int last_enc_windows = 0;
    bool mel_ready = false;
    bool pooled = false;
    int ktime_mask = 0;
    wm::KStat kstat[wm::K_NCLASS];
    wm::KStat vad_kstat[3];
    struct KPending { int cls; hipEvent_t a, b; double work; int sub = 0; };
    std::vector<KPending> kpending;
    std::vector<hipEvent_t> kpool;
    struct DecGraph { int n_tok, n_rows, mask; bool direct; int sig; int pdec; int gen; int par; int beam; hipGraphExec_t exec; std::vector<KPending> ev; uint64_t seed = 0; int actx = 0; bool deny = false; bool gram = false; float gram_pen = 0.0f; bool filt = false; bool tdrz = false; };
    std::vector<DecGraph> dec_graphs;
    std::vector<KPending>* capture_ev = nullptr;
    double cur_self_work = 0;
    whisper_state* twin = nullptr;
    long pdec_give_ups = 0;
    double pdec_lost_ms = 0;
    double pdec_off_until = 0;
    bool pdec_off = false;
    wm::StepMode mode;
    bool deny_on = false;
    bool gram_on = false;
    wm::GrammarRules gram_rules;
    float gram_penalty = 0.0f;
    bool filter_on = false, tdrz_on = false;
    struct BeamRec { std::vector<int> tokens; double sum_logprobs_all = 0; int flags = 0; };
    std::vector<std::vector<BeamRec>> beam_info;
    uint64_t sample_seed = 0;
    std::vector<std::vector<BeamRec>> cand_info;
    double gather_rows = 0, gather_rows_full = 0;
};

struct whisper_context {
    wm::Context c;
};

namespace wm {
inline int enc_ctx(const Context* c, const whisper_state* s) { return s->audio_ctx > 0 ? s->audio_ctx : c->hp.n_audio_ctx; }
bool load_context(Context* c, const char* path, int device, DType dt, bool load_weights);
void free_context(Context* c);
whisper_state* new_state(Context* c);
void free_state(whisper_state* s);
void recover_state(whisper_state* s);
void drain_state_pool(Context* c);
void orphan_states(Context* c);
bool resolve_dtw(Context* c, const whisper_context_params& cp);

struct FullOpts {
    int fixed_tokens = 0;
    const int* forced = nullptr;
    const int* spot = nullptr;
    int n_spot = 0;
    float* spot_logits = nullptr;
    bool pieces = false;
    bool* stopped = nullptr;
};
extern std::atomic<long> g_decoded_tokens_total;
int full_batch(Context* c, whisper_state* s, const whisper_full_params& p, const float* const* pcm, const int* n,
               int n_jobs, bool on_device, const FullOpts& o, bool single_api);
int full_parallel(Context* c, whisper_state* s, const whisper_full_params& p, const float* pcm, int n_samples,
                  int n_processors, int snap_ms, bool on_device);
int deny_lookup(Context* c, bool suppress_nst, const char* regex, std::vector<uint32_t>* words);
int grammar_check(const whisper_full_params& p, GrammarRules& rules);
std::shared_ptr<VadModel> vad_lookup(Context* c, const char* path);
const GramVocab& gram_vocab(Context* c);

int compute_mel(Context* c, whisper_state* s, const float* const* pcm, const int* n, int n_jobs, bool on_device);
int encode_windows(Context* c, whisper_state* s, const int* jobs, const int* seeks, const int* slots, int n_win);
int decode_tokens(Context* c, whisper_state* s, const int* tokens, const int* pos, const int* slots, int n_tok,
                  const int* logit_rows, int n_logit_rows);
std::vector<std::pair<float, int>> rank_languages(const float* logits);
}
```

### nobs-whisper_amd/csrc/kernels.h

```cpp
#pragma once
#include <atomic>

#include "common.h"
#include "gemm_plan.h"
#include "grammar.h"

namespace wm {

void launch_mel(const float* const* d_pcm, const int* d_n, const void* d_tab, const float* d_filt_t, int n_mel,
                float* const* d_mel, const int* d_nlen, int* d_max, int n_jobs, int max_frames, hipStream_t st);
void launch_mel_window(DType dt, float* const* d_mel, const int* d_nlen, const int* d_n, const int* d_max,
                       const int* d_win_job, const int* d_win_seek, int n_win, int n_mel, int frames, void* out,
                       hipStream_t st);
void launch_mel_normalize(const float* d_mel, int nl, int n_samples, const int* d_max, int n_mel, float* out, hipStream_t st);
void launch_silence_boundaries(const float* const* pcm, const int* n_samples, int n_clips, int max_n, int sample_rate,
                               float* rms, int rms_stride, int* counts, int* bounds, int cap, float* floor_out,
                               hipStream_t st);
void launch_resample(const float* const* in, const int* n_in, int n_clips, int max_out, const float* W, int ldw, int fsi,
                     int fso, float* const* out, const int* n_out, hipStream_t st);

void launch_layernorm(DType dt, const float* x, const int* rows, int M, int D, const float* w, const float* b,
                      void* y, hipStream_t st);
void launch_embed(DType dt, const void* tok_emb, bool te_f32, const float* pos_emb, const int* tok, const int* pos,
                  int n, int D, float* x, hipStream_t st);
void launch_embed_ln(DType dt, const void* tok_emb, bool te_f32, const float* pos_emb, const int* tok, const int* pos,
                     int n, int D, float* x, const float* w, const float* b, void* y, hipStream_t st);


struct QMat {
    int type = 0;
    const uint8_t* qs = nullptr;
    const uint32_t* qh = nullptr;
    const uint16_t* dm = nullptr;
};

struct GemmArgs {
    const void* A; long a_rpb, a_bstride, a_rstride;
    const void* B;
    const float* bias;
    int M, N, K;
    void* out; long ldo; long o_rpb, o_bstride, o_off;
    const float* pos; int pos_rows;
    float scale; int sc_div, sc_mod, sc_lim;
    void* cache; const int* row_slot; const int* row_pos; int L, layer, H, ctx, d;
    int rpw;
    float* splitk_ws; long splitk_ws_elems;
    const float* ln_w; const float* ln_b; void* ln_out;
    const float* a_ln_w; const float* a_ln_b;
    QMat q;
    int slab_wt;
    const float* w8_scale;
    unsigned long long* stamps;
};
extern unsigned long long* g_gemm_stamps;
inline GemmArgs gemm_plain(const void* A, int M, int K, const void* B, int N, const float* bias, void* out, long ldo) {
    GemmArgs g{};
    g.A = A; g.a_rpb = M > 0 ? M : 1; g.a_bstride = 0; g.a_rstride = K;
    g.B = B; g.bias = bias; g.M = M; g.N = N; g.K = K;
    g.out = out; g.ldo = ldo; g.o_rpb = M > 0 ? M : 1; g.o_bstride = 0; g.o_off = 0;
    g.sc_div = 0; g.sc_mod = 1; g.sc_lim = 0; g.scale = 1.0f;
    return g;
}

GemmKnobs current_knobs();
void launch_gemm(DType dt, int epi, const GemmArgs& a, hipStream_t st);
void launch_gemm_fp8(DType dt, int epi, const GemmArgs& a, const float* a_scale, const float* b_scale, hipStream_t st);
void launch_quant_rows_fp8(DType dt, const void* x, long rows, int K, void* q, float* s, hipStream_t st);
void launch_layernorm_fp8(const float* x, int M, int D, const float* w, const float* b, void* q, float* s,
                          hipStream_t st);
void init_gelu_table();
int launch_gemm_partials(DType dt, const GemmArgs& a, hipStream_t st);
bool gemm_small_ok(int M, int K, bool lna);
void launch_dequant(DType dt, const QMat& q, long rows, int K, void* out, hipStream_t st);
struct DequantJobs {
    int n = 0;
    QMat q[6];
    long rows[6];
    int K[6];
    void* out[6];
    long start[7];
};
void launch_dequant_multi(DType dt, DequantJobs J, hipStream_t st);
void launch_gemm_small(DType dt, int epi, const GemmArgs& a, bool lna, hipStream_t st);

void launch_attn_encoder(DType dt, const void* qkv, void* out, int B, int T, int d, int H, hipStream_t st,
                         int variant = -1);
void launch_attn_prefill(DType dt, const void* q, int q_stride, const void* cache, const int* slot, const int* n_kv,
                         const void* tiles, int n_tiles, int L, int layer, int H, int ctx, int d, void* out,
                         hipStream_t st);

struct DecSlabs {
    const float* ws; int splits; long zstride; int ld; const float* bias; float scale;
};
void launch_attn_self_step(DType dt, const DecSlabs& sl, void* cache, const int* slot, const int* pos, int n, int L,
                           int layer, int H, int ctx, int d, void* out, hipStream_t st);
int attn_cross_wide_max();
void launch_attn_cross_step(DType dt, const DecSlabs& sl, const void* cache, const int* slot, const int* n_kv, int n,
                            int L, int layer, int H, int ctx, int d, void* out, hipStream_t st);

bool xattn_supported(int d);
int xattn_splits(int n, int Tn);
void launch_xattn_qproj(DType dt, const void* q, const void* wkt, int n, int d, int H, float scale, void* qx,
                        hipStream_t st);
void launch_xattn_step(DType dt, const void* enc, const int* slot, const void* qx, int n, int Tn, int d, int splits,
                       float thr, float* opart, float* ml, hipStream_t st);
void launch_xattn_combine(DType dt, const float* opart, const float* ml, int splits, const void* wv, const float* bv, int n,
                          int d, int H, void* out, hipStream_t st);

struct AlignClip {
    int slot, row0, n_rows, n_sot, frames, pad;
    long p_off, st_off, cost_off, tr_off, fr_off, path_off;
};
void launch_align_scores(DType dt, const void* q, int q_stride, const void* cross, const AlignClip* clips, int n_clips,
                         int max_rows, int L, int layer, int H, int ctx, int n_keys, const int2* heads, int n_heads,
                         float* P, hipStream_t st);
void launch_align_cost(const float* P, const AlignClip* clips, int n_clips, int A, int max_rows, int max_frames, float* stats,
                       float* cost, hipStream_t st);
void launch_align_dtw(const float* cost, const AlignClip* clips, int n_clips, int max_n, unsigned char* trace, int* fr,
                      int* path, int* path_len, hipStream_t st);

constexpr int kPdecMaxRows = 4;
struct PdecMat {
    const void* w;
    const uint32_t* qh;
    const uint16_t* dm;
    int qt;
};
struct PdecLayer {
    PdecMat qkv, o, xq, xo, f1, f2;
    const float *bqkv, *bo, *bxq, *bxo, *b1, *b2;
    const float *ln1_w, *ln1_b, *lnx_w, *lnx_b, *ln2_w, *ln2_b;
};
struct PdecGranules {
    long x0, x1, x2, qkv, so, qx, xo, ff, part;
    long err_bytes, zero_bytes, bytes;
};
PdecGranules pdec_granules(int d, int L, int H);
struct PdecLds {
    int xs, xf, sc, red, qf, res, ost, lred, lnp, part, lflag, gtab, bytes, rows, cmax;
};
constexpr int kPdecGeluHalf = 0x4900;
__host__ __device__ inline PdecLds pdec_lds(int d, int M, int S) {
    auto up = [](int b) { return (b + 15) & ~15; };
    PdecLds l{};
    l.rows = M <= 2 ? M : kPdecMaxRows;
    const int c1 = 2 * ((3 * d / 2 + 255) / 256), c4 = 2 * ((2 * d + 255) / 256);
    l.cmax = c1 > c4 ? c1 : c4;
    int o = 0;
    l.xs = o; o += up(l.rows * 4 * d * 2);
    l.xf = o; o += up(l.rows * d * 4);
    l.sc = o; o += 1536 * 4;
    l.red = o; o += up((8 + 256) * 4);
    l.qf = o; o += 192 * 4;
    l.res = o; o += up(68 * 4);
    l.ost = o; o += up(l.rows * l.cmax * 4);
    l.lred = o; o += 2 * kPdecMaxRows * 4 * 8;
    l.lnp = o; o += up(6 * d * 4);
    l.part = o; o += up(S * 66 * 4);
    l.lflag = o; o += 16;
    l.gtab = o; o += M <= 2 ? up(2 * kPdecGeluHalf * 2) : 0;
    l.bytes = o;
    return l;
}
struct PdecArgs {
    const PdecLayer* layers;
    int L, M, d, n_text_ctx, n_audio_ctx;
    int n_audio_len;
    const void* tok_emb; int te_f32; const float* pos_d;
    const float *lnd_w, *lnd_b;
    const int *tok, *pos, *slot;
    void* self_cache; const void* cross_cache;
    float k_scale;
    int s_cross;
    int quant;
    void* sync;
// ... 70 lines not shown
```

### nobs-whisper_amd/csrc/kernels/attn.hip

```cpp
#include "../common.h"
#include "../kernels.h"

namespace wm {

typedef uint32_t u32x4 __attribute__((ext_vector_type(4)));

__device__ __forceinline__ int swz(int row, int ch) { return ch ^ ((row >> 1) & 7); }

template <typename T, int MINW = 1, bool PK = true>
__global__ void __launch_bounds__(512, MINW) attn_enc2_kernel(const T* __restrict__ qkv, T* __restrict__ out, int Tn, int d,
                                                             int nqb = 0, int H = 0) {
    typedef typename Frag<T>::type FT;
    typedef short v4s __attribute__((ext_vector_type(4)));
    typedef __attribute__((address_space(3))) v4s* lds_v4s_t;
    int qb = blockIdx.x, h = blockIdx.y, b = blockIdx.z;
    if (nqb > 0) {
        const int L = blockIdx.x, G = gridDim.x;
        const int p = (L & 7) * (G >> 3) + (L >> 3);
        qb = p % nqb;
        h = (p / nqb) % H;
        b = p / (nqb * H);
    }
    const int tid = threadIdx.x, wave = tid >> 6, lane = tid & 63;
    const int hh = lane >> 5, ql = lane & 31;
// ... 175 lines not shown
                                              const int* __restrict__ n_kv_arr, int L, int layer, int H, int ctx, int d,
                                              T* __restrict__ out) {
    const int i = blockIdx.x, h = blockIdx.y;
    constexpr int NG = NTH / 8, NW = NTH / 64;
    const int tid = threadIdx.x, lane8 = tid & 7, grp = tid >> 3;
    const int n_kv = n_kv_arr[i];
    const long s = slot[i];
    const T* K = cache + (((s * L + layer) * 2 + 0) * H + h) * (long)ctx * 64;
    const T* V = cache + (((s * L + layer) * 2 + 1) * H + h) * (long)ctx * 64;
    __shared__ float sc[1536];
    __shared__ float red[NTH];
    __shared__ float acc_s[NG][65];

    constexpr int CHR = NG * U;
    const u32x4 zero = {0, 0, 0, 0};
    auto load_rows = [&](const T* base, int t0, u32x4 (&raw)[U]) {
#pragma unroll
        for (int u = 0; u < U; u++) {
            const int t = t0 + NG * u;
            raw[u] = t < n_kv ? *(const u32x4*)(base + (long)t * 64 + lane8 * 8) : zero;
        }
    };
    u32x4 ra[U], rb[U];
    load_rows(K, grp, ra);
    float qv[8];
    if constexpr (FQ) {
        if (tid < 64) {
            const float* p = sl.ws + (long)i * sl.ld + h * 64 + tid;
            float pz[16], v = 0.0f;
#pragma unroll
            for (int z = 0; z < 16; z++)
                if (z < sl.splits) pz[z] = p[z * sl.zstride];
#pragma unroll
            for (int z = 0; z < 16; z++)
                if (z < sl.splits) v += pz[z];
            if (sl.bias) v = v + sl.bias[h * 64 + tid];
            red[tid] = (float)(T)(v * sl.scale);
        }
        __syncthreads();
#pragma unroll
        for (int e = 0; e < 8; e++) qv[e] = red[lane8 * 8 + e];
        __syncthreads();
    } else {
        const u32x4 raw = *(const u32x4*)(q + (long)i * q_stride + h * 64 + lane8 * 8);
        const T* qe = (const T*)&raw;
#pragma unroll
        for (int e = 0; e < 8; e++) qv[e] = (float)qe[e];
    }
    float lmax = -INFINITY;
    auto scores = [&](int t0, const u32x4 (&raw)[U]) {
#pragma unroll
        for (int u = 0; u < U; u++) {
            const int t = t0 + NG * u;
            const T* ke = (const T*)&raw[u];
            float a = 0.0f;
#pragma unroll
            for (int e = 0; e < 8; e++) a += qv[e] * (float)ke[e];
            a = sum8(a);
            if (t < n_kv) {
                if (lane8 == 0) sc[t] = a;
                lmax = fmaxf(lmax, a);
            }
        }
    };
    {
        int t0 = grp;
        for (; t0 + CHR < n_kv; t0 += 2 * CHR) {
            load_rows(K, t0 + CHR, rb);
            scores(t0, ra);
            if (t0 + 2 * CHR < n_kv) load_rows(K, t0 + 2 * CHR, ra);
            scores(t0 + CHR, rb);
        }
        if (t0 < n_kv) scores(t0, ra);
    }
    load_rows(V, grp, ra);
    const int wave = tid >> 6, lane = tid & 63;
    for (int o = 32; o > 0; o >>= 1) lmax = fmaxf(lmax, __shfl_xor(lmax, o));
    if (lane == 0) red[wave] = lmax;
    __syncthreads();
    float mx = red[0];
#pragma unroll
    for (int w = 1; w < NW; w++) mx = fmaxf(mx, red[w]);
    float lsum = 0.0f;
    for (int t = tid; t < n_kv; t += NTH) {
        const float e = expf(sc[t] - mx);
        sc[t] = e;
        lsum += e;
    }
    __syncthreads();
    red[tid] = lsum;
    __syncthreads();
    if (wave == 0) {
        float r;
        if constexpr (NTH == 256) {
            r = (red[lane] + red[lane + 128]) + (red[lane + 64] + red[lane + 192]);
        } else {
            r = red[lane];
#pragma unroll
            for (int w = 1; w < NW; w++) r = r + red[lane + 64 * w];
        }
        for (int o = 32; o > 0; o >>= 1) r = r + __shfl_down(r, o);
        if (lane == 0) red[0] = r;
    }
    __syncthreads();
    const float inv = 1.0f / red[0];
    for (int t = tid; t < n_kv; t += NTH) sc[t] = (float)(T)(sc[t] * inv);
    __syncthreads();
    float acc[8];
#pragma unroll
    for (int e = 0; e < 8; e++) acc[e] = 0.0f;
    auto pv = [&](int t0, const u32x4 (&raw)[U]) {
#pragma unroll
        for (int u = 0; u < U; u++) {
            const int t = t0 + NG * u;
            const T* ve = (const T*)&raw[u];
            const float p = t < n_kv ? sc[t] : 0.0f;
#pragma unroll
            for (int e = 0; e < 8; e++) acc[e] += p * (float)ve[e];
        }
    };
    {
        int t0 = grp;
        for (; t0 + CHR < n_kv; t0 += 2 * CHR) {
            load_rows(V, t0 + CHR, rb);
            pv(t0, ra);
            if (t0 + 2 * CHR < n_kv) load_rows(V, t0 + 2 * CHR, ra);
            pv(t0 + CHR, rb);
        }
        if (t0 < n_kv) pv(t0, ra);
    }
#pragma unroll
    for (int e = 0; e < 8; e++) acc_s[grp][lane8 * 8 + e] = acc[e];
    __syncthreads();
    if (tid < 64) {
        float a = 0.0f;
        for (int g2 = 0; g2 < NG; g2++) a += acc_s[g2][tid];
        out[(long)i * d + h * 64 + tid] = (T)a;
    }
}

template <typename T>
__global__ void __launch_bounds__(256) attn_cross_step_kernel(const DecSlabs sl, const T* __restrict__ cache,
                                                              const int* __restrict__ slot, const int* __restrict__ n_kv_arr,
                                                              int L, int layer, int H, int ctx, int d, T* __restrict__ out) {
    attn_dec_body<T, true>(nullptr, 0, sl, cache, slot, n_kv_arr, L, layer, H, ctx, d, out);
}
template <typename T>
__global__ void __launch_bounds__(1024) attn_cross_step_wide_kernel(const DecSlabs sl, const T* __restrict__ cache,
                                                                    const int* __restrict__ slot, const int* __restrict__ n_kv_arr,
                                                                    int L, int layer, int H, int ctx, int d, T* __restrict__ out) {
    attn_dec_body<T, true, 1024, 4>(nullptr, 0, sl, cache, slot, n_kv_arr, L, layer, H, ctx, d, out);
}

template <typename T, int HPB>
__global__ void __launch_bounds__(64 * HPB) attn_self_step_kernel(const DecSlabs sl, T* __restrict__ cache,
                                                                  const int* __restrict__ slot,
                                                                  const int* __restrict__ pos_arr, int L, int layer,
                                                                  int H, int ctx, int d, T* __restrict__ out) {
    const int i = blockIdx.x, w = threadIdx.x >> 6, lane = threadIdx.x & 63;
    const int h = blockIdx.y * HPB + w;
    const int lane8 = lane & 7, grp = lane >> 3;
    __shared__ float qs[HPB][64], ks[HPB][64], vs[HPB][64];
    __shared__ float sc[HPB][448];
    const int pos = pos_arr[i];
    const long s = slot[i];
    T* K = cache + (((s * L + layer) * 2 + 0) * H + h) * (long)ctx * 64;
    T* V = cache + (((s * L + layer) * 2 + 1) * H + h) * (long)ctx * 64;
    constexpr int U = 8;
    const u32x4 zero = {0, 0, 0, 0};
    u32x4 raw[U];
    auto kload = [&](int t0) {
#pragma unroll
        for (int u = 0; u < U; u++) {
            const int t = t0 + 8 * u;
            const u32x4* src = (const u32x4*)(K + (long)t * 64 + lane8 * 8);
            raw[u] = t < pos ? *src : zero;
        }
    };
    kload(grp);
    {
        const float* p = sl.ws + (long)i * sl.ld + h * 64 + lane;
        float pq[16], pk[16], pv[16];
#pragma unroll
        for (int z = 0; z < 16; z++)
            if (z < sl.splits) {
                const float* pz = p + z * sl.zstride;
                pq[z] = pz[0];
                pk[z] = pz[d];
                pv[z] = pz[2 * d];
            }
        float vq = 0.0f, vk = 0.0f, vv = 0.0f;
#pragma unroll
        for (int z = 0; z < 16; z++)
            if (z < sl.splits) {
                vq += pq[z];
                vk += pk[z];
                vv += pv[z];
            }
        if (sl.bias) {
            vq = vq + sl.bias[h * 64 + lane];
            vk = vk + sl.bias[d + h * 64 + lane];
            vv = vv + sl.bias[2 * d + h * 64 + lane];
        }
        const T tq = (T)(vq * sl.scale), tk = (T)(vk * sl.scale), tv = (T)vv;
        K[(long)pos * 64 + lane] = tk;
        V[(long)pos * 64 + lane] = tv;
        qs[w][lane] = (float)tq;
        ks[w][lane] = (float)tk;
        vs[w][lane] = (float)tv;
    }
    __syncthreads();
    float qv[8];
#pragma unroll
    for (int e = 0; e < 8; e++) qv[e] = qs[w][lane8 * 8 + e];
    float lmax = -INFINITY;
    for (int t0 = grp; t0 < pos; t0 += 8 * U) {
        if (t0 != grp) kload(t0);
#pragma unroll
        for (int u = 0; u < U; u++) {
            const int t = t0 + 8 * u;
            const T* ke = (const T*)&raw[u];
            float a = 0.0f;
#pragma unroll
            for (int e = 0; e < 8; e++) a += qv[e] * (float)ke[e];
            a = sum8(a);
            if (t < pos) {
                if (lane8 == 0) sc[w][t] = a;
                lmax = fmaxf(lmax, a);
            }
        }
    }
    {
        float a = 0.0f;
#pragma unroll
        for (int e = 0; e < 8; e++) a += qv[e] * ks[w][lane8 * 8 + e];
        a = sum8(a);
        if (lane == 0) sc[w][pos] = a;
        lmax = fmaxf(lmax, a);
    }
    for (int o = 32; o > 0; o >>= 1) lmax = fmaxf(lmax, __shfl_xor(lmax, o));
    __syncthreads();
    const int n_kv = pos + 1;
    float lsum = 0.0f;
    for (int t = lane; t < n_kv; t += 64) {
        const float e = expf(sc[w][t] - lmax);
        sc[w][t] = e;
        lsum += e;
    }
    for (int o = 32; o > 0; o >>= 1) lsum += __shfl_xor(lsum, o);
    const float inv = 1.0f / lsum;
    for (int t = lane; t < n_kv; t += 64) sc[w][t] = (float)(T)(sc[w][t] * inv);
    __syncthreads();
    float acc[8];
#pragma unroll
    for (int e = 0; e < 8; e++) acc[e] = 0.0f;
    for (int t0 = grp; t0 < pos; t0 += 8 * U) {
        u32x4 vraw[U];
#pragma unroll
        for (int u = 0; u < U; u++) {
            const int t = t0 + 8 * u;
            const u32x4* src = (const u32x4*)(V + (long)t * 64 + lane8 * 8);
            vraw[u] = t < pos ? *src : zero;
        }
#pragma unroll
        for (int u = 0; u < U; u++) {
            const int t = t0 + 8 * u;
            const T* ve = (const T*)&vraw[u];
            const float p = t < pos ? sc[w][t] : 0.0f;
#pragma unroll
            for (int e = 0; e < 8; e++) acc[e] += p * (float)ve[e];
        }
    }
    if (grp == 0) {
        const float p = sc[w][pos];
#pragma unroll
        for (int e = 0; e < 8; e++) acc[e] += p * vs[w][lane8 * 8 + e];
    }
#pragma unroll
    for (int e = 0; e < 8; e++) {
        acc[e] += dpp8_f<0x128>(acc[e]);
        acc[e] += __shfl_xor(acc[e], 16);
        acc[e] += __shfl_xor(acc[e], 32);
    }
    if (grp == 0) {
        T o8[8];
#pragma unroll
        for (int e = 0; e < 8; e++) o8[e] = (T)acc[e];
        *(u32x4*)(out + (long)i * d + h * 64 + lane8 * 8) = *(const u32x4*)o8;
    }
}

template <typename T>
__global__ void __launch_bounds__(256) attn_prefill_kernel(const T* __restrict__ q, int q_stride, const T* __restrict__ cache,
                                                           const int* __restrict__ slot, const int* __restrict__ n_kv_arr,
                                                           const int2* __restrict__ tiles, int L, int layer, int H,
                                                           int ctx, int d, T* __restrict__ out) {
    typedef typename Frag<T>::type FT;
    const int2 tl = tiles[blockIdx.x];
    const int i0 = tl.x, cnt = tl.y, h = blockIdx.y;
    const int tid = threadIdx.x, wave = tid >> 6, lane = tid & 63;
    const long s = slot[i0];
    const T* K = cache + (((s * L + layer) * 2 + 0) * H + h) * (long)ctx * 64;
    const T* V = cache + (((s * L + layer) * 2 + 1) * H + h) * (long)ctx * 64;
    __shared__ u32x4 Ks[64 * 8];
    __shared__ u32x4 Vts[64 * 8];
    __shared__ u32x4 Ps[4][16 * 8];
    const u32x4 zero = {0, 0, 0, 0};
    const int kv_end = n_kv_arr[i0 + cnt - 1];
    FT qf[2];
    {
        const int row = wave * 16 + (lane & 15);
#pragma unroll
        for (int s2 = 0; s2 < 2; s2++) {
            const int ch = s2 * 4 + (lane >> 4);
            const u32x4 v = row < cnt ? *(const u32x4*)(q + (long)(i0 + row) * q_stride + h * 64 + ch * 8) : zero;
            qf[s2] = __builtin_bit_cast(FT, v);
        }
    }
    int nkv[4];
#pragma unroll
    for (int r = 0; r < 4; r++) {
        const int row = wave * 16 + (lane >> 4) * 4 + r;
        nkv[r] = row < cnt ? n_kv_arr[i0 + row] : 0;
    }
    const int n_kt = (kv_end + 63) / 64;
    auto stage_k = [&](int kt) {
#pragma unroll
        for (int i = 0; i < 2; i++) {
            const int c = tid + i * 256, key = c >> 3, kc = c & 7, kg = kt * 64 + key;
            Ks[key * 8 + swz(key, kc)] = kg < kv_end ? *(const u32x4*)(K + (long)kg * 64 + kc * 8) : zero;
        }
    };
    auto scores = [&](int kt, f32x4 (&sacc)[4]) {
#pragma unroll
        for (int j = 0; j < 4; j++) {
            sacc[j] = (f32x4){0.f, 0.f, 0.f, 0.f};
#pragma unroll
            for (int s2 = 0; s2 < 2; s2++) {
                const int row = j * 16 + (lane & 15);
                const FT kf = __builtin_bit_cast(FT, Ks[row * 8 + swz(row, s2 * 4 + (lane >> 4))]);
                sacc[j] = mfma16x16x32(qf[s2], kf, sacc[j]);
            }
#pragma unroll
            for (int r = 0; r < 4; r++) {
                const int key = kt * 64 + j * 16 + (lane & 15);
                if (key >= nkv[r]) sacc[j][r] = -INFINITY;
            }
        }
    };
    float m_i[4], l_i[4];
#pragma unroll
    for (int r = 0; r < 4; r++) { m_i[r] = -INFINITY; l_i[r] = 0.0f; }
    for (int kt = 0; kt < n_kt; kt++) {
        __syncthreads();
        stage_k(kt);
        __syncthreads();
        f32x4 sacc[4];
        scores(kt, sacc);
#pragma unroll
        for (int r = 0; r < 4; r++) {
            float mx = fmaxf(fmaxf(sacc[0][r], sacc[1][r]), fmaxf(sacc[2][r], sacc[3][r]));
            for (int o2 = 1; o2 < 16; o2 <<= 1) mx = fmaxf(mx, __shfl_xor(mx, o2));
            const float mn = fmaxf(m_i[r], mx);
            float sum = 0.0f;
            if (mn != -INFINITY) {
#pragma unroll
                for (int j = 0; j < 4; j++) sum += expf(sacc[j][r] - mn);
            }
            for (int o2 = 1; o2 < 16; o2 <<= 1) sum += __shfl_xor(sum, o2);
            l_i[r] = (m_i[r] == -INFINITY ? 0.0f : l_i[r] * expf(m_i[r] - mn)) + sum;
            m_i[r] = mn;
        }
    }
    float inv[4];
#pragma unroll
    for (int r = 0; r < 4; r++) inv[r] = l_i[r] > 0.0f ? 1.0f / l_i[r] : 0.0f;
    f32x4 o[4];
#pragma unroll
    for (int j = 0; j < 4; j++) o[j] = (f32x4){0.f, 0.f, 0.f, 0.f};
    T* Vt_el = (T*)Vts;
    T* P_el = (T*)Ps[wave];
    for (int kt = 0; kt < n_kt; kt++) {
        __syncthreads();
        stage_k(kt);
#pragma unroll
        for (int i = 0; i < 2; i++) {
            const int c = tid + i * 256, key = c >> 3, kc = c & 7, kg = kt * 64 + key;
            const u32x4 vv = kg < kv_end ? *(const u32x4*)(V + (long)kg * 64 + kc * 8) : zero;
            const T* ve = (const T*)&vv;
#pragma unroll
            for (int e = 0; e < 8; e++) {
                const int dim = kc * 8 + e;
                Vt_el[(dim * 8 + swz(dim, key >> 3)) * 8 + (key & 7)] = ve[e];
            }
        }
        __syncthreads();
        f32x4 sacc[4];
        scores(kt, sacc);
#pragma unroll
        for (int j = 0; j < 4; j++)
#pragma unroll
            for (int r = 0; r < 4; r++) {
                const float p = sacc[j][r] == -INFINITY ? 0.0f : expf(sacc[j][r] - m_i[r]) * inv[r];
                const int row = (lane >> 4) * 4 + r, key = j * 16 + (lane & 15);
                P_el[(row * 8 + swz(row, key >> 3)) * 8 + (key & 7)] = (T)p;
            }
        __builtin_amdgcn_s_waitcnt(0xc07f);
        __builtin_amdgcn_wave_barrier();
#pragma unroll
        for (int s2 = 0; s2 < 2; s2++) {
            const int prow = lane & 15;
            const FT pf = __builtin_bit_cast(FT, Ps[wave][prow * 8 + swz(prow, s2 * 4 + (lane >> 4))]);
#pragma unroll
            for (int j = 0; j < 4; j++) {
                const int vrow = j * 16 + (lane & 15);
                const FT vf = __builtin_bit_cast(FT, Vts[vrow * 8 + swz(vrow, s2 * 4 + (lane >> 4))]);
                o[j] = mfma16x16x32(pf, vf, o[j]);
            }
        }
    }
#pragma unroll
    for (int r = 0; r < 4; r++) {
        const int row = wave * 16 + (lane >> 4) * 4 + r;
        if (row >= cnt) continue;
#pragma unroll
        for (int j = 0; j < 4; j++) out[(long)(i0 + row) * d + h * 64 + j * 16 + (lane & 15)] = (T)o[j][r];
    }
}

void launch_attn_prefill(DType dt, const void* q, int q_stride, const void* cache, const int* slot, const int* n_kv,
                         const void* tiles, int n_tiles, int L, int layer, int H, int ctx, int d, void* out,
                         hipStream_t st) {
    if (n_tiles <= 0) return;
    dim3 grid(n_tiles, H);
    if (dt == DType::F16)
        attn_prefill_kernel<half_t><<<grid, 256, 0, st>>>((const half_t*)q, q_stride, (const half_t*)cache, slot, n_kv,
                                                          (const int2*)tiles, L, layer, H, ctx, d, (half_t*)out);
    else
        attn_prefill_kernel<bf16_t><<<grid, 256, 0, st>>>((const bf16_t*)q, q_stride, (const bf16_t*)cache, slot, n_kv,
                                                          (const int2*)tiles, L, layer, H, ctx, d, (bf16_t*)out);
}

static bool attn_enc_xcd() {
    static const bool v = !getenv("WHISPER_MI355X_ENC_ATTN_XCD") || atoi(getenv("WHISPER_MI355X_ENC_ATTN_XCD")) != 0;
    return v;
}

void launch_attn_encoder(DType dt, const void* qkv, void* out, int B, int Tn, int d, int H, hipStream_t st,
                         int variant_arg) {
    const int variant = variant_arg >= 0 ? variant_arg : 6;
    if (d != H * 64 || (variant != 2 && variant != 6)) WM_FAIL("encoder attention: d %d != 64 x %d heads, or variant %d", d, H, variant);
    const int nqb = cdiv(Tn, 256);
    const dim3 grid(nqb, H, B);
    if (variant == 2) {
        if (dt == DType::F16) attn_enc2_kernel<half_t><<<grid, 512, 0, st>>>((const half_t*)qkv, (half_t*)out, Tn, d);
        else attn_enc2_kernel<bf16_t><<<grid, 512, 0, st>>>((const bf16_t*)qkv, (bf16_t*)out, Tn, d);
        return;
    }
    if ((long)nqb * H * B % 8 == 0 && attn_enc_xcd()) {
        const int G = nqb * H * B;
        if (dt == DType::F16) attn_enc2_kernel<half_t, 4, false><<<G, 512, 0, st>>>((const half_t*)qkv, (half_t*)out, Tn, d, nqb, H);
        else attn_enc2_kernel<bf16_t, 4, false><<<G, 512, 0, st>>>((const bf16_t*)qkv, (bf16_t*)out, Tn, d, nqb, H);
        return;
    }
    if (dt == DType::F16) attn_enc2_kernel<half_t, 4, false><<<grid, 512, 0, st>>>((const half_t*)qkv, (half_t*)out, Tn, d);
    else attn_enc2_kernel<bf16_t, 4, false><<<grid, 512, 0, st>>>((const bf16_t*)qkv, (bf16_t*)out, Tn, d);
}

int attn_cross_wide_max() {
    const char* e = getenv("WHISPER_MI355X_XWIDE_MAX");
    return e ? atoi(e) : 8;
}

void launch_attn_cross_step(DType dt, const DecSlabs& sl, const void* cache, const int* slot, const int* n_kv, int n,
                            int L, int layer, int H, int ctx, int d, void* out, hipStream_t st) {
    if (n <= 0) return;
    if (ctx > 1536) WM_FAIL("attention context %d > 1536", ctx);
    dim3 grid(n, H);
    if (n <= attn_cross_wide_max()) {
        if (dt == DType::F16)
            attn_cross_step_wide_kernel<half_t><<<grid, 1024, 0, st>>>(sl, (const half_t*)cache, slot, n_kv, L, layer, H, ctx, d, (half_t*)out);
        else
            attn_cross_step_wide_kernel<bf16_t><<<grid, 1024, 0, st>>>(sl, (const bf16_t*)cache, slot, n_kv, L, layer, H, ctx, d, (bf16_t*)out);
        return;
    }
    if (dt == DType::F16)
        attn_cross_step_kernel<half_t><<<grid, 256, 0, st>>>(sl, (const half_t*)cache, slot, n_kv, L, layer, H, ctx, d, (half_t*)out);
    else
        attn_cross_step_kernel<bf16_t><<<grid, 256, 0, st>>>(sl, (const bf16_t*)cache, slot, n_kv, L, layer, H, ctx, d, (bf16_t*)out);
}

void launch_attn_self_step(DType dt, const DecSlabs& sl, void* cache, const int* slot, const int* pos, int n, int L,
                           int layer, int H, int ctx, int d, void* out, hipStream_t st) {
    if (n <= 0) return;
    if (ctx > 448) WM_FAIL("self-attention context %d > 448", ctx);
    static const int hpb_env = getenv("WHISPER_MI355X_SELF_HPB") ? atoi(getenv("WHISPER_MI355X_SELF_HPB")) : 0;
    const int want = hpb_env > 0 ? hpb_env : (n <= 32 ? 1 : 4);
    const int hpb = want >= 4 && H % 4 == 0 ? 4 : want >= 2 && H % 2 == 0 ? 2 : 1;
#define WM_SELF(TT, HB) \
    attn_self_step_kernel<TT, HB><<<dim3(n, H / HB), 64 * HB, 0, st>>>(sl, (TT*)cache, slot, pos, L, layer, H, ctx, d, (TT*)out)
#define WM_SELF_H(TT) \
    do { if (hpb == 4) WM_SELF(TT, 4); else if (hpb == 2) WM_SELF(TT, 2); else WM_SELF(TT, 1); } while (0)
    if (dt == DType::F16) WM_SELF_H(half_t);
    else WM_SELF_H(bf16_t);
#undef WM_SELF_H
#undef WM_SELF
}

}
```

### nobs-whisper_amd/csrc/kernels/norm.hip

```cpp
#include "../common.h"
#include "../kernels.h"

namespace wm {

template <typename T, int NPL>
__global__ void __launch_bounds__(256) layernorm_kernel(const float* __restrict__ x, const int* __restrict__ rows, int M, int D,
                                                        const float* __restrict__ w, const float* __restrict__ b,
                                                        T* __restrict__ y) {
    const int wave = threadIdx.x >> 6, lane = threadIdx.x & 63;
    const int i = blockIdx.x * 4 + wave;
    if (i >= M) return;
    const long r = rows ? rows[i] : i;
    const float* xr = x + r * D;
    float v[NPL];
#pragma unroll
    for (int e = 0; e < NPL; e++) {
        const int k = lane + 64 * e;
        v[e] = k < D ? xr[k] : 0.0f;
    }
    double s = 0.0;
#pragma unroll
    for (int e = 0; e < NPL; e++) s += (double)v[e];
    for (int o = 32; o > 0; o >>= 1) s += __shfl_xor(s, o);
    const float mean = (float)(s / D);
    double s2 = 0.0;
#pragma unroll
    for (int e = 0; e < NPL; e++) {
        const int k = lane + 64 * e;
        v[e] = v[e] - mean;
        if (k < D) s2 += (double)(v[e] * v[e]);
    }
    for (int o = 32; o > 0; o >>= 1) s2 += __shfl_xor(s2, o);
    const float variance = (float)(s2 / D);
    const float scale = 1.0f / sqrtf(variance + 1e-5f);
    T* yr = y + (long)i * D;
#pragma unroll
    for (int e = 0; e < NPL; e++) {
        const int k = lane + 64 * e;
        if (k < D) {
            float t = v[e] * scale;
            t = t * w[k];
            yr[k] = (T)(t + b[k]);
        }
    }
}

template <int NPL>
__global__ void __launch_bounds__(256) layernorm_fp8_kernel(const float* __restrict__ x, int M, int D,
                                                            const float* __restrict__ w, const float* __restrict__ b,
                                                            uint8_t* __restrict__ q, float* __restrict__ s) {
    const int wave = threadIdx.x >> 6, lane = threadIdx.x & 63;
    const int i = blockIdx.x * 4 + wave;
    if (i >= M) return;
    const float* xr = x + (long)i * D;
    float v[NPL];
#pragma unroll
    for (int e = 0; e < NPL; e++) {
        const int k = lane + 64 * e;
        v[e] = k < D ? xr[k] : 0.0f;
    }
    double s1 = 0.0;
#pragma unroll
    for (int e = 0; e < NPL; e++) s1 += (double)v[e];
    for (int o = 32; o > 0; o >>= 1) s1 += __shfl_xor(s1, o);
    const float mean = (float)(s1 / D);
    double s2 = 0.0;
#pragma unroll
    for (int e = 0; e < NPL; e++) {
        const int k = lane + 64 * e;
        v[e] = v[e] - mean;
        if (k < D) s2 += (double)(v[e] * v[e]);
    }
    for (int o = 32; o > 0; o >>= 1) s2 += __shfl_xor(s2, o);
    const float variance = (float)(s2 / D);
    const float scale = 1.0f / sqrtf(variance + 1e-5f);
    float amax = 0.f;
#pragma unroll
    for (int e = 0; e < NPL; e++) {
        const int k = lane + 64 * e;
        if (k < D) {
            v[e] = (v[e] * scale) * w[k] + b[k];
            amax = fmaxf(amax, fabsf(v[e]));
        }
    }
    for (int o = 32; o > 0; o >>= 1) amax = fmaxf(amax, __shfl_xor(amax, o));
    const float sc = amax > 0.f ? amax / 448.f : 1.f, inv = 1.f / sc;
    if (lane == 0) s[i] = sc;
    uint8_t* qr = q + (long)i * D;
#pragma unroll
    for (int e = 0; e < NPL; e++) {
        const int k = lane + 64 * e;
        if (k < D) {
            const float t = fminf(fmaxf(v[e] * inv, -448.f), 448.f);
            qr[k] = (uint8_t)(__builtin_amdgcn_cvt_pk_fp8_f32(t, t, 0, false) & 0xff);
        }
    }
}

template <int NV>
__global__ void __launch_bounds__(256) layernorm_fp8_v4_kernel(const float* __restrict__ x, int M, int D,
                                                               const float* __restrict__ w, const float* __restrict__ b,
                                                               uint8_t* __restrict__ q, float* __restrict__ s) {
    const int wave = threadIdx.x >> 6, lane = threadIdx.x & 63;
    const int i = blockIdx.x * 4 + wave;
    if (i >= M) return;
    const float4* xr = (const float4*)(x + (long)i * D);
    float4 v[NV];
    double s1 = 0.0;
#pragma unroll
    for (int e = 0; e < NV; e++) {
        v[e] = xr[lane + 64 * e];
        s1 += (double)v[e].x + (double)v[e].y + (double)v[e].z + (double)v[e].w;
    }
    for (int o = 32; o > 0; o >>= 1) s1 += __shfl_xor(s1, o);
    const float mean = (float)(s1 / D);
    double s2 = 0.0;
#pragma unroll
    for (int e = 0; e < NV; e++) {
        v[e].x -= mean; v[e].y -= mean; v[e].z -= mean; v[e].w -= mean;
        s2 += (double)(v[e].x * v[e].x) + (double)(v[e].y * v[e].y) + (double)(v[e].z * v[e].z) + (double)(v[e].w * v[e].w);
    }
    for (int o = 32; o > 0; o >>= 1) s2 += __shfl_xor(s2, o);
    const float scale = 1.0f / sqrtf((float)(s2 / D) + 1e-5f);
    float amax = 0.f;
#pragma unroll
    for (int e = 0; e < NV; e++) {
        const int k = 4 * (lane + 64 * e);
        const float4 ww = *(const float4*)(w + k), bb = *(const float4*)(b + k);
        v[e].x = (v[e].x * scale) * ww.x + bb.x; v[e].y = (v[e].y * scale) * ww.y + bb.y;
        v[e].z = (v[e].z * scale) * ww.z + bb.z; v[e].w = (v[e].w * scale) * ww.w + bb.w;
        amax = fmaxf(amax, fmaxf(fmaxf(fabsf(v[e].x), fabsf(v[e].y)), fmaxf(fabsf(v[e].z), fabsf(v[e].w))));
    }
    for (int o = 32; o > 0; o >>= 1) amax = fmaxf(amax, __shfl_xor(amax, o));
    const float sc = amax > 0.f ? amax / 448.f : 1.f, inv = 1.f / sc;
    if (lane == 0) s[i] = sc;
    uint32_t* qr = (uint32_t*)(q + (long)i * D);
    auto c = [&](float t) { return fminf(fmaxf(t * inv, -448.f), 448.f); };
#pragma unroll
    for (int e = 0; e < NV; e++) {
        uint32_t u = __builtin_amdgcn_cvt_pk_fp8_f32(c(v[e].x), c(v[e].y), 0, false);
        u = __builtin_amdgcn_cvt_pk_fp8_f32(c(v[e].z), c(v[e].w), u, true);
        qr[lane + 64 * e] = u;
    }
}

void launch_layernorm_fp8(const float* x, int M, int D, const float* w, const float* b, void* q, float* s,
                          hipStream_t st) {
    if (M <= 0) return;
    if (D % 256 == 0 && D <= 2048) {
#define WM_LN8V(N)                                                                                          \
        if (D == 256 * N) {                                                                                 \
            layernorm_fp8_v4_kernel<N><<<cdiv(M, 4), 256, 0, st>>>(x, M, D, w, b, (uint8_t*)q, s);         \
            return;                                                                                         \
        }
        WM_LN8V(2) WM_LN8V(3) WM_LN8V(4) WM_LN8V(5) WM_LN8V(6) WM_LN8V(8)
#undef WM_LN8V
    }
#define WM_LN8(N)                                                                                           \
    if (D <= 64 * N) {                                                                                      \
        layernorm_fp8_kernel<N><<<cdiv(M, 4), 256, 0, st>>>(x, M, D, w, b, (uint8_t*)q, s);                 \
        return;                                                                                             \
    }
    WM_LN8(6) WM_LN8(8) WM_LN8(12) WM_LN8(16) WM_LN8(20) WM_LN8(24) WM_LN8(32)
#undef WM_LN8
    WM_FAIL("layernorm width %d > 2048", D);
}

template <typename TE>
__global__ void embed_kernel(const TE* __restrict__ te, const float* __restrict__ pe, const int* __restrict__ tok,
                             const int* __restrict__ pos, int D, float* __restrict__ x) {
    const int i = blockIdx.x;
    const long t = tok[i], p = pos[i];
    for (int k = threadIdx.x; k < D; k += blockDim.x) x[(long)i * D + k] = (float)te[t * D + k] + pe[p * D + k];
}

template <typename T, int NPT, typename TE>
__global__ void __launch_bounds__(256) embed_ln_kernel(const TE* __restrict__ te, const float* __restrict__ pe,
                                                       const int* __restrict__ tok, const int* __restrict__ pos, int D,
                                                       float* __restrict__ x, const float* __restrict__ w,
                                                       const float* __restrict__ b, T* __restrict__ y) {
    __shared__ double sh[4];
    const int i = blockIdx.x;
    const long t = tok[i], p = pos[i];
    float v[NPT];
#pragma unroll
    for (int k = 0; k < NPT; k++) {
        const int n = threadIdx.x + 256 * k;
        v[k] = 0.0f;
        if (n < D) {
            v[k] = (float)te[t * D + n] + pe[p * D + n];
            x[(long)i * D + n] = v[k];
        }
    }
    block256_layernorm<T, NPT>(v, D, w, b, y + (long)i * D, sh);
}

void launch_embed_ln(DType dt, const void* te, bool te_f32, const float* pe, const int* tok, const int* pos, int n, int D,
                     float* x, const float* w, const float* b, void* y, hipStream_t st) {
    if (n <= 0) return;
    if (D > 2048) WM_FAIL("embed LN width %d > 2048", D);
#define WM_ELN(T, NPT)                                                                                                    \
    if (te_f32) embed_ln_kernel<T, NPT, float><<<n, 256, 0, st>>>((const float*)te, pe, tok, pos, D, x, w, b, (T*)y);       \
    else embed_ln_kernel<T, NPT, T><<<n, 256, 0, st>>>((const T*)te, pe, tok, pos, D, x, w, b, (T*)y)
    if (D <= 1024) {
        if (dt == DType::F16) { WM_ELN(half_t, 4); } else { WM_ELN(bf16_t, 4); }
    } else {
        if (dt == DType::F16) { WM_ELN(half_t, 8); } else { WM_ELN(bf16_t, 8); }
    }
#undef WM_ELN
}

void launch_layernorm(DType dt, const float* x, const int* rows, int M, int D, const float* w, const float* b, void* y,
                      hipStream_t st) {
    if (M <= 0) return;
    const int npl = cdiv(D, 64);
#define WM_LN(N)                                                                                              \
    if (npl <= N) {                                                                                           \
        if (dt == DType::F16) layernorm_kernel<half_t, N><<<cdiv(M, 4), 256, 0, st>>>(x, rows, M, D, w, b, (half_t*)y); \
        else layernorm_kernel<bf16_t, N><<<cdiv(M, 4), 256, 0, st>>>(x, rows, M, D, w, b, (bf16_t*)y);     \
        return;                                                                                               \
    }
    WM_LN(1) WM_LN(2) WM_LN(4) WM_LN(6) WM_LN(8) WM_LN(12) WM_LN(16) WM_LN(20) WM_LN(24) WM_LN(32)
#undef WM_LN
    WM_FAIL("layernorm width %d > 2048", D);
}

void launch_embed(DType dt, const void* te, bool te_f32, const float* pe, const int* tok, const int* pos, int n, int D,
                  float* x, hipStream_t st) {
    if (n <= 0) return;
    if (te_f32) embed_kernel<float><<<n, 256, 0, st>>>((const float*)te, pe, tok, pos, D, x);
    else if (dt == DType::F16) embed_kernel<half_t><<<n, 256, 0, st>>>((const half_t*)te, pe, tok, pos, D, x);
    else embed_kernel<bf16_t><<<n, 256, 0, st>>>((const bf16_t*)te, pe, tok, pos, D, x);
}

}
```

### nobs-whisper_amd/csrc/kernels/xattn.hip

```cpp
#include <algorithm>

#include "../common.h"
#include "../kernels.h"

namespace wm {

typedef uint32_t u32x4 __attribute__((ext_vector_type(4)));
typedef short v4s __attribute__((ext_vector_type(4)));

__device__ __forceinline__ int xsw(int row) { return ((row & 3) << 2) | ((row >> 2) & 3); }
__device__ __forceinline__ int xphys(int row, int ch) { return (ch & ~15) | ((ch & 15) ^ xsw(row)); }

template <int N>
__device__ __forceinline__ void wait_vm() {
    if constexpr (N == 1) asm volatile("s_waitcnt vmcnt(1)" ::: "memory");
    else if constexpr (N == 2) asm volatile("s_waitcnt vmcnt(2)" ::: "memory");
    else if constexpr (N == 3) asm volatile("s_waitcnt vmcnt(3)" ::: "memory");
    else if constexpr (N == 4) asm volatile("s_waitcnt vmcnt(4)" ::: "memory");
    else if constexpr (N == 5) asm volatile("s_waitcnt vmcnt(5)" ::: "memory");
    else if constexpr (N == 6) asm volatile("s_waitcnt vmcnt(6)" ::: "memory");
    else if constexpr (N == 7) asm volatile("s_waitcnt vmcnt(7)" ::: "memory");
    else asm volatile("s_waitcnt vmcnt(0)" ::: "memory");
}
__device__ __forceinline__ v4s ds_read_tr(unsigned lds_addr) {
    v4s r;
    asm volatile("ds_read_b64_tr_b16 %0, %1" : "=v"(r) : "v"(lds_addr));
    return r;
}
template <int CTRL>
__device__ __forceinline__ float dpp_f(float x) {
    return __builtin_bit_cast(float, __builtin_amdgcn_update_dpp(0, __builtin_bit_cast(int, x), CTRL, 0xF, 0xF, false));
}
__device__ __forceinline__ float max16(float x) {
    x = fmaxf(x, dpp_f<0xB1>(x));
    x = fmaxf(x, dpp_f<0x4E>(x));
    x = fmaxf(x, dpp_f<0x141>(x));
    return fmaxf(x, dpp_f<0x140>(x));
}
__device__ __forceinline__ float sum16(float x) {
    x = x + dpp_f<0xB1>(x);
    x = x + dpp_f<0x4E>(x);
    x = x + dpp_f<0x141>(x);
    return x + dpp_f<0x140>(x);
}

__device__ __forceinline__ void lds_barrier() { asm volatile("s_waitcnt lgkmcnt(0)\n\ts_barrier" ::: "memory"); }

template <typename T, int MT, int NT, bool STG = false>
__global__ void __launch_bounds__(256) xattn_qproj_kernel(const T* __restrict__ q, const T* __restrict__ wkt, int n, int d,
                                                          int H, float scale, T* __restrict__ qx) {
    typedef typename Frag<T>::type FT;
    const int lane = threadIdx.x & 63, wave = threadIdx.x >> 6;
    const int c0 = blockIdx.x * 64 * MT + wave * 16 * MT, h = blockIdx.y, i0 = blockIdx.z * 16 * NT;
    constexpr int SW = 64 * MT + 8;
    __shared__ __attribute__((aligned(16))) T simg[STG ? 2 * 16 * NT * SW : 1];
    if (!STG && c0 >= d) return;
    const u32x4 zero = {0, 0, 0, 0};
    FT af[MT][2], bq[NT][2];
#pragma unroll
    for (int mt = 0; mt < MT; mt++) {
        const int c = c0 + mt * 16 + (lane & 15);
#pragma unroll
        for (int ks = 0; ks < 2; ks++)
            af[mt][ks] = __builtin_bit_cast(FT, *(const u32x4*)(wkt + ((long)h * d + c) * 64 + ks * 32 + 8 * (lane >> 4)));
    }
#pragma unroll
    for (int nt = 0; nt < NT; nt++) {
        const int i = i0 + nt * 16 + (lane & 15);
#pragma unroll
        for (int ks = 0; ks < 2; ks++)
            bq[nt][ks] = __builtin_bit_cast(FT, i < n ? *(const u32x4*)(q + (long)i * d + h * 64 + ks * 32 + 8 * (lane >> 4)) : zero);
    }
#pragma unroll
    for (int mt = 0; mt < MT; mt++)
#pragma unroll
        for (int nt = 0; nt < NT; nt++) {
            f32x4 acc = {0.f, 0.f, 0.f, 0.f};
#pragma unroll
            for (int ks = 0; ks < 2; ks++) acc = mfma16x16x32(af[mt][ks], bq[nt][ks], acc);
            const int i = i0 + nt * 16 + (lane & 15);
            T hi[4], lo[4];
#pragma unroll
            for (int r = 0; r < 4; r++) {
                const float v = acc[r] * scale;
                hi[r] = (T)v;
                lo[r] = (T)(v - (float)hi[r]);
            }
            if constexpr (STG) {
                const int tl = nt * 16 + (lane & 15), cl = wave * 16 * MT + mt * 16 + 4 * (lane >> 4);
                *(uint2*)(simg + tl * SW + cl) = *(const uint2*)hi;
                *(uint2*)(simg + (16 * NT + tl) * SW + cl) = *(const uint2*)lo;
                continue;
            }
            if (i >= n) continue;
            const int c = c0 + mt * 16 + 4 * (lane >> 4);
            *(uint2*)(qx + ((long)i * 2 * H + h) * d + c) = *(const uint2*)hi;
            *(uint2*)(qx + ((long)i * 2 * H + H + h) * d + c) = *(const uint2*)lo;
        }
    if constexpr (STG) {
        __syncthreads();
        constexpr int CH = 64 * MT / 8, ROWS = 2 * 16 * NT;
        const int cb = blockIdx.x * 64 * MT;
        for (int e = threadIdx.x; e < ROWS * CH; e += 256) {
            const int row = e / CH, ch = e - row * CH;
            const int part = row / (16 * NT), tl = row - part * 16 * NT, i = i0 + tl;
            if (i < n)
                *(u32x4*)(qx + ((long)i * 2 * H + part * H + h) * d + cb + ch * 8) = *(const u32x4*)(simg + row * SW + ch * 8);
        }
    }
}

template <typename T, int NW, int CT, int AUX>
__global__ void __launch_bounds__(NW * 64) xattn_step_kernel(const T* __restrict__ enc, const int* __restrict__ slot,
                                                             const T* __restrict__ qx, int Tn, int splits, float thr,
                                                             float* __restrict__ opart, float* __restrict__ ml, int ostg = 0) {
    typedef typename Frag<T>::type FT;
    typedef __attribute__((address_space(3))) void* lds_ptr_t;
    constexpr int D = NW * CT * 32, H = D / 64, NQ = (2 * H + 15) / 16;
    constexpr int RC = D / 8;
    constexpr int NS = 3;
    constexpr int TILE = 16 * RC;
    constexpr int NH = (H + 15) / 16;
    constexpr int RSR = 16 * NH + 4;
    constexpr int PS = 20;
    constexpr int STG_B = NS * TILE * 16, RED_B = NW * 16 * RSR * 4, P_B = 32 * PS * (int)sizeof(T);
    static_assert(RC % 16 == 0, "d must be a multiple of 128");
    static_assert(H * 16 <= NW * 64, "one softmax lane per (head, row)");
    static_assert(H <= 32, "heads are the N = 32 side of the P.V MFMA");
    __shared__ __attribute__((aligned(16))) char lds[STG_B + RED_B + P_B + 32 * 4 + 16];
    u32x4* stg = (u32x4*)lds;
    float* red = (float*)(lds + STG_B);
    T* pimg = (T*)(lds + STG_B + RED_B);
    float* alph = (float*)(lds + STG_B + RED_B + P_B);
    int* flag = (int*)(alph + 32);

    const int sp = blockIdx.x, i = blockIdx.y;
    const int tid = threadIdx.x, wave = tid >> 6, lane = tid & 63;
    const int nt_all = (Tn + 15) >> 4;
    const int tb = sp * nt_all / splits, ntile = (sp + 1) * nt_all / splits - tb;
    const T* E = enc + (long)slot[i] * Tn * D;
    const int cw = wave * CT * 32;

    for (int e = tid; e < 32 * PS; e += NW * 64) pimg[e] = (T)0.0f;
    if (tid < 32) alph[tid] = 1.0f;
    if (tid < 2) flag[tid] = 0;

    const u32x4 zero = {0, 0, 0, 0};
    FT qf[CT][NQ];
    {
        const T* Q = qx + (long)i * 2 * H * D;
#pragma unroll
        for (int kk = 0; kk < CT; kk++)
#pragma unroll
            for (int j = 0; j < NQ; j++) {
                const int hp = j * 16 + (lane & 15);
                qf[kk][j] = __builtin_bit_cast(
                    FT, hp < 2 * H ? *(const u32x4*)(Q + (long)hp * D + cw + kk * 32 + 8 * (lane >> 4)) : zero);
            }
#pragma unroll
        for (int kk = 0; kk < CT; kk++)
#pragma unroll
            for (int j = 0; j < NQ; j++) asm volatile("" ::"v"(qf[kk][j]));
    }
    int prow[CT], poff[CT];
#pragma unroll
    for (int k = 0; k < CT; k++) {
        const int qq = (wave + k * NW) * 64 + lane;
        const int row = qq / RC, pc = qq - row * RC;
        prow[k] = row;
        poff[k] = xphys(row, pc) * 8;
    }
    auto issue = [&](int t) {
        const int row0 = (tb + t) * 16;
        u32x4* st = stg + (t % NS) * TILE;
#pragma unroll
        for (int k = 0; k < CT; k++) {
            const int gr = min(row0 + prow[k], Tn - 1);
            __builtin_amdgcn_global_load_lds((const void*)(E + (long)gr * D + poff[k]),
                                             (lds_ptr_t)(st + (wave + k * NW) * 64), 16, 0, AUX);
        }
    };

    f32x16 oacc[CT];
#pragma unroll
    for (int k = 0; k < CT; k++)
#pragma unroll
        for (int r = 0; r < 16; r++) oacc[k][r] = 0.0f;
    float m_run = -INFINITY, l_run = 0.0f;
    const float LOG2E = 1.44269504088896340736f;
    const int hh = lane >> 5;

    issue(0);
    if (ntile > 1) issue(1);
    for (int t = 0; t < ntile; t++) {
        if (t + 1 < ntile) wait_vm<CT>();
        else wait_vm<0>();
        lds_barrier();
        if (t + 2 < ntile) issue(t + 2);
        const u32x4* st = stg + (t % NS) * TILE;

        f32x4 sacc[NQ];
#pragma unroll
        for (int j = 0; j < NQ; j++) sacc[j] = (f32x4){0.f, 0.f, 0.f, 0.f};
        {
            const int row = lane & 15;
            FT ef[CT];
#pragma unroll
            for (int kk = 0; kk < CT; kk++)
                ef[kk] = __builtin_bit_cast(FT, st[row * RC + xphys(row, (cw >> 3) + kk * 4 + (lane >> 4))]);
#pragma unroll
            for (int kk = 0; kk < CT; kk++)
#pragma unroll
                for (int j = 0; j < NQ; j++) sacc[j] = mfma16x16x32(ef[kk], qf[kk][j], sacc[j]);
        }
        {
            constexpr int J0 = H / 16, D0 = H % 16;
            float* rw = red + wave * 16 * RSR;
#pragma unroll
            for (int jh = 0; jh < NH; jh++)
#pragma unroll
                for (int r = 0; r < 4; r++) {
                    float lo;
                    if constexpr (D0 == 0) {
                        lo = sacc[jh + J0][r];
                    } else {
                        const float a = dpp_f<0x100 + D0>(sacc[jh + J0][r]);
                        const float b = jh + J0 + 1 < NQ ? dpp_f<0x110 + 16 - D0>(sacc[min(jh + J0 + 1, NQ - 1)][r]) : 0.0f;
                        lo = (lane & 15) < 16 - D0 ? a : b;
                    }
                    rw[(4 * (lane >> 4) + r) * RSR + jh * 16 + (lane & 15)] = sacc[jh][r] + lo;
                }
        }
        lds_barrier();

        if (tid < 16 * H) {
            const int h = tid >> 4, r = tid & 15;
            float sv = 0.0f;
#pragma unroll
            for (int w = 0; w < NW; w++) {
                sv += red[(w * 16 + r) * RSR + h];
            }
            const float s2 = (tb + t) * 16 + r < Tn ? sv * LOG2E : -INFINITY;
            const float mx = max16(s2);
            float alpha = 1.0f;
            if (mx > m_run + thr) {
                alpha = __builtin_amdgcn_exp2f(m_run - mx);
                m_run = mx;
                flag[t & 1] = 1;
            }
            const T pt = (T)__builtin_amdgcn_exp2f(s2 - m_run);
            l_run = l_run * alpha + sum16((float)pt);
            pimg[h * PS + r] = pt;
            if (r == 0) alph[h] = alpha;
        }
        if (tid == 0) flag[(t + 1) & 1] = 0;
        lds_barrier();

        FT pf;
        {
            const T* pr = pimg + (lane & 31) * PS + 4 * hh;
            const v4s lo = *(const v4s*)pr;
            const v4s hi = *(const v4s*)(pr + 8);
            pf = __builtin_bit_cast(FT, __builtin_shufflevector(lo, hi, 0, 1, 2, 3, 4, 5, 6, 7));
        }
        const int tg = (lane >> 4) & 1, tq = (lane & 15) >> 2, tp = lane & 3;
        const int rlo = 4 * hh + tq, rhi = rlo + 8;
        const unsigned img = (unsigned)(unsigned long)(lds_ptr_t)(const void*)st;
        v4s elo[CT], ehi[CT];
#pragma unroll
        for (int k = 0; k < CT; k++) {
            const int ch = ((cw + k * 32) >> 3) + tg * 2 + (tp >> 1);
            elo[k] = ds_read_tr(img + rlo * RC * 16 + 16 * xphys(rlo, ch) + 8 * (tp & 1));
            ehi[k] = ds_read_tr(img + rhi * RC * 16 + 16 * xphys(rhi, ch) + 8 * (tp & 1));
        }
        const int fl = flag[t & 1];
        const float al = alph[lane & 31];
        asm volatile("s_waitcnt lgkmcnt(0)" ::: "memory");
        __builtin_amdgcn_sched_barrier(0);
        if (fl) {
#pragma unroll
            for (int k = 0; k < CT; k++)
#pragma unroll
                for (int r = 0; r < 16; r++) oacc[k][r] *= al;
        }
#pragma unroll
        for (int k = 0; k < CT; k++) {
            const FT ef = __builtin_bit_cast(FT, __builtin_shufflevector(elo[k], ehi[k], 0, 1, 2, 3, 4, 5, 6, 7));
            oacc[k] = mfma32x32x16(ef, pf, oacc[k]);
        }
    }

    const int h = lane & 31;
    if (ostg) {
        constexpr int OW = CT * 32 + 4;
        static_assert(NW * H * OW * 4 <= STG_B, "O staging fits the E stages");
        __syncthreads();
        float* so = (float*)lds + wave * H * OW;
        if (h < H) {
#pragma unroll
            for (int k = 0; k < CT; k++)
#pragma unroll
                for (int g = 0; g < 4; g++) {
                    const int c = k * 32 + 8 * g + 4 * hh;
                    *(f32x4*)(so + h * OW + c) = (f32x4){oacc[k][4 * g], oacc[k][4 * g + 1], oacc[k][4 * g + 2], oacc[k][4 * g + 3]};
                }
        }
        asm volatile("s_waitcnt lgkmcnt(0)" ::: "memory");
        __builtin_amdgcn_wave_barrier();
        float* ob = opart + ((long)i * splits + sp) * H * D + cw;
        for (int e = lane; e < H * CT * 8; e += 64) {
            const int hr = e / (CT * 8), ch = e - hr * (CT * 8);
            *(f32x4*)(ob + (long)hr * D + ch * 4) = *(const f32x4*)(so + hr * OW + ch * 4);
        }
    } else if (h < H) {
        float* o = opart + (((long)i * splits + sp) * H + h) * D;
#pragma unroll
        for (int k = 0; k < CT; k++)
#pragma unroll
            for (int g = 0; g < 4; g++) {
                const int c = cw + k * 32 + 8 * g + 4 * hh;
                const f32x4 v = {oacc[k][4 * g], oacc[k][4 * g + 1], oacc[k][4 * g + 2], oacc[k][4 * g + 3]};
                *(f32x4*)(o + c) = v;
            }
    }
    if (tid < 16 * H && (tid & 15) == 0) {
        float* p = ml + (((long)i * splits + sp) * H + (tid >> 4)) * 2;
        p[0] = m_run;
        p[1] = l_run;
    }
}

template <typename T, int TOK, int PF, bool EARLYW>
__global__ void __launch_bounds__(512) xattn_combine_kernel(const float* __restrict__ opart, const float* __restrict__ ml,
                                                            int splits, const T* __restrict__ wv, const float* __restrict__ bv,
                                                            int n, int d, int H, T* __restrict__ out) {
    typedef typename Frag<T>::type FT;
    constexpr int DMAX = 1280;
    constexpr int NA = TOK >= 8 ? TOK / 8 : 1, RT = 16 * NA;
    const int h = blockIdx.x, i0 = blockIdx.y * TOK;
    const int tid = threadIdx.x, wave = tid >> 6, lane = tid & 63;
    __shared__ __attribute__((aligned(16))) char lds[RT * DMAX * 2 + TOK * 16 * 4];
    T* aimg = (T*)lds;
    float* red = (float*)lds;
    float* wgt = (float*)(lds + RT * DMAX * 2);
    static_assert(8 * RT * 64 * 4 <= RT * DMAX * 2, "reduce image fits the A image");
    auto slot_of = [&](int row, int ch) { return row * d + ((ch & ~15) | ((ch & 15) ^ (row & 15))) * 8; };
    if (tid < TOK) {
        const int i = i0 + tid;
        if (i < n) {
            const float* p = ml + ((long)i * splits * H + h) * 2;
            float2 q[16];
#pragma unroll
            for (int s = 0; s < 16; s++)
                if (s < splits) q[s] = *(const float2*)(p + (long)s * H * 2);
            float M = -INFINITY;
#pragma unroll
            for (int s = 0; s < 16; s++)
                if (s < splits) M = fmaxf(M, q[s].x);
            float L = 0.0f;
#pragma unroll
            for (int s = 0; s < 16; s++)
                if (s < splits) L += __builtin_amdgcn_exp2f(q[s].x - M) * q[s].y;
            const float inv = 1.0f / L;
#pragma unroll
            for (int s = 0; s < 16; s++)
                if (s < splits) wgt[tid * 16 + s] = __builtin_amdgcn_exp2f(q[s].x - M) * inv;
        } else {
            for (int s = 0; s < splits; s++) wgt[tid * 16 + s] = 0.0f;
        }
    }
    constexpr int KMAX = DMAX / 256;
    const int r16 = lane & 15, kq = lane >> 4;
    FT bfp[KMAX][4];
    auto load_wv = [&]() {
#pragma unroll
        for (int k = 0; k < KMAX; k++) {
            const int ks = wave + 8 * k;
            if (ks < d / 32) {
#pragma unroll
                for (int j = 0; j < 4; j++)
                    bfp[k][j] = __builtin_bit_cast(FT, *(const u32x4*)(wv + ((long)h * 64 + j * 16 + r16) * d + ks * 32 + 8 * kq));
            }
        }
    };
    if constexpr (EARLYW) load_wv();
    const int q4 = d / 4;
    constexpr int NE = (TOK * (DMAX / 4) + 511) / 512;
    float4 a[NE], x[PF][NE];
    const float* src[NE];
#pragma unroll
    for (int j = 0; j < NE; j++) {
        a[j] = make_float4(0.f, 0.f, 0.f, 0.f);
        const int e = min(tid + 512 * j, TOK * q4 - 1);
        const int t = e / q4, c = (e - t * q4) * 4;
        src[j] = opart + ((long)min(i0 + t, n - 1) * splits * H + h) * d + c;
    }
#pragma unroll
    for (int u = 0; u < PF; u++)
        if (u < splits) {
#pragma unroll
            for (int j = 0; j < NE; j++) x[u][j] = *(const float4*)(src[j] + (long)u * H * d);
        }
    __syncthreads();
    for (int s0 = 0; s0 < splits; s0 += PF) {
#pragma unroll
        for (int u = 0; u < PF; u++) {
            const int s = s0 + u;
            if (s >= splits) break;
#pragma unroll
            for (int j = 0; j < NE; j++) {
                const int t = min(tid + 512 * j, TOK * q4 - 1) / q4;
                const float w = wgt[t * 16 + s];
                a[j].x += w * x[u][j].x; a[j].y += w * x[u][j].y; a[j].z += w * x[u][j].z; a[j].w += w * x[u][j].w;
            }
            if (s + PF < splits) {
#pragma unroll
                for (int j = 0; j < NE; j++) x[u][j] = *(const float4*)(src[j] + (long)(s + PF) * H * d);
            }
        }
    }
#pragma unroll
    for (int j = 0; j < NE; j++) {
        const int e = tid + 512 * j;
        if (e >= TOK * q4) break;
        const int t = e / q4, c = (e - t * q4) * 4;
        const float v[4] = {a[j].x, a[j].y, a[j].z, a[j].w};
        T hi[4], lo[4];
#pragma unroll
        for (int k = 0; k < 4; k++) {
            hi[k] = (T)v[k];
            lo[k] = (T)(v[k] - (float)hi[k]);
        }
        const int ch = c >> 3, half = ((c >> 2) & 1) * 4;
        *(uint2*)(aimg + slot_of(t, ch) + half) = *(const uint2*)hi;
        *(uint2*)(aimg + slot_of(TOK + t, ch) + half) = *(const uint2*)lo;
    }
    if constexpr (!EARLYW) load_wv();
    __syncthreads();
    f32x4 acc[NA][4];
#pragma unroll
    for (int a = 0; a < NA; a++)
#pragma unroll
        for (int j = 0; j < 4; j++) acc[a][j] = (f32x4){0.f, 0.f, 0.f, 0.f};
#pragma unroll
    for (int k = 0; k < KMAX; k++) {
        const int ks = wave + 8 * k;
        if (ks >= d / 32) break;
#pragma unroll
        for (int a = 0; a < NA; a++) {
            const FT af = *(const FT*)(aimg + slot_of(a * 16 + r16, ks * 4 + kq));
#pragma unroll
            for (int j = 0; j < 4; j++) acc[a][j] = mfma16x16x32(af, bfp[k][j], acc[a][j]);
        }
    }
    __syncthreads();
#pragma unroll
    for (int a = 0; a < NA; a++)
#pragma unroll
        for (int j = 0; j < 4; j++)
#pragma unroll
            for (int r = 0; r < 4; r++) red[(wave * RT + a * 16 + 4 * kq + r) * 64 + j * 16 + r16] = acc[a][j][r];
    __syncthreads();
    for (int e = tid; e < TOK * 64; e += 512) {
        const int ti = e >> 6, j = e & 63;
        if (i0 + ti >= n) continue;
        float v = 0.0f;
#pragma unroll
        for (int w = 0; w < 8; w++) v += red[(w * RT + ti) * 64 + j] + red[(w * RT + TOK + ti) * 64 + j];
        out[(long)(i0 + ti) * d + h * 64 + j] = (T)(v + bv[h * 64 + j]);
    }
}

int xattn_splits(int n, int Tn) {
    const int nn = std::max(1, n);
    const int s = std::max(1, std::min(16, (256 + nn - 1) / nn));
    return std::min(s, (Tn + 15) / 16);
}

bool xattn_supported(int d) { return d == 384 || d == 512 || d == 768 || d == 1024 || d == 1280; }

void launch_xattn_qproj(DType dt, const void* q, const void* wkt, int n, int d, int H, float scale, void* qx,
                        hipStream_t st) {
    if (n <= 0) return;
    dim3 grid(cdiv(d, 64 * 2), H, cdiv(n, 16 * 4));
    static const int stg = getenv("WHISPER_MI355X_QPROJ_STG") ? atoi(getenv("WHISPER_MI355X_QPROJ_STG")) : 1;
    if (stg && d % 128 == 0) {
        if (dt == DType::F16)
            xattn_qproj_kernel<half_t, 2, 4, true><<<grid, 256, 0, st>>>((const half_t*)q, (const half_t*)wkt, n, d, H, scale, (half_t*)qx);
        else
            xattn_qproj_kernel<bf16_t, 2, 4, true><<<grid, 256, 0, st>>>((const bf16_t*)q, (const bf16_t*)wkt, n, d, H, scale, (bf16_t*)qx);
        return;
    }
    if (dt == DType::F16)
        xattn_qproj_kernel<half_t, 2, 4><<<grid, 256, 0, st>>>((const half_t*)q, (const half_t*)wkt, n, d, H, scale, (half_t*)qx);
    else
        xattn_qproj_kernel<bf16_t, 2, 4><<<grid, 256, 0, st>>>((const bf16_t*)q, (const bf16_t*)wkt, n, d, H, scale, (bf16_t*)qx);
}

template <typename T>
static void launch_step_t(const void* enc, const int* slot, const void* qx, int n, int Tn, int d, int splits, float thr,
                          float* opart, float* ml, hipStream_t st) {
    dim3 grid(splits, n);
    static const int ostg = getenv("WHISPER_MI355X_XSTEP_OSTG") ? atoi(getenv("WHISPER_MI355X_XSTEP_OSTG")) : 1;
#define WM_XSTEP(NW_, CT_) \
    xattn_step_kernel<T, NW_, CT_, 2><<<grid, NW_ * 64, 0, st>>>((const T*)enc, slot, (const T*)qx, Tn, splits, thr, opart, ml, ostg)
    switch (d) {
        case 384: WM_XSTEP(4, 3); break;
        case 512: WM_XSTEP(8, 2); break;
        case 768: WM_XSTEP(8, 3); break;
        case 1024: WM_XSTEP(8, 4); break;
        case 1280: WM_XSTEP(8, 5); break;
        default: WM_FAIL("direct cross attention needs d in {384,512,768,1024,1280}");
    }
#undef WM_XSTEP
}

void launch_xattn_step(DType dt, const void* enc, const int* slot, const void* qx, int n, int Tn, int d, int splits,
                       float thr, float* opart, float* ml, hipStream_t st) {
    if (n <= 0) return;
    if (splits < 1 || splits > 16 || splits > (Tn + 15) / 16) WM_FAIL("bad split count %d", splits);
    if (dt == DType::F16) launch_step_t<half_t>(enc, slot, qx, n, Tn, d, splits, thr, opart, ml, st);
    else launch_step_t<bf16_t>(enc, slot, qx, n, Tn, d, splits, thr, opart, ml, st);
}

void launch_xattn_combine(DType dt, const float* opart, const float* ml, int splits, const void* wv, const float* bv, int n,
                          int d, int H, void* out, hipStream_t st) {
    if (n <= 0) return;
    if (splits > 16 || d % 128 || d > 1280) WM_FAIL("combine shape not supported");
    static const int tok_env = getenv("WHISPER_MI355X_XCOMB_TOK") ? atoi(getenv("WHISPER_MI355X_XCOMB_TOK")) : 0;
    int tok = 4;
    for (int t : {16, 8})
        if (H * cdiv(n, t) >= 160) { tok = t; break; }
    if (tok_env == 4 || tok_env == 8 || tok_env == 16) tok = tok_env;
    const dim3 grid(H, cdiv(n, tok));
#define WM_XCOMB(T_, TOK_, PF_, E_) xattn_combine_kernel<T_, TOK_, PF_, E_><<<grid, 512, 0, st>>>(opart, ml, splits, (const T_*)wv, bv, n, d, H, (T_*)out)
#define WM_XCOMB_T(T_)                              \
    if (tok == 4) WM_XCOMB(T_, 4, 2, true);         \
    else if (tok == 16) WM_XCOMB(T_, 16, 1, false); \
    else WM_XCOMB(T_, 8, 2, true);
    if (dt == DType::F16) {
        WM_XCOMB_T(half_t)
    } else {
        WM_XCOMB_T(bf16_t)
    }
#undef WM_XCOMB_T
#undef WM_XCOMB
}

}
```

Baseline: 3451.

## Fuse encoder ln_post into slot write and retune decoder attention kernels

New measurement: 3461 (median of 6 runs). No clear change (+0.3%).

```diff
diff --git a/include/whisper_mi355x.h b/include/whisper_mi355x.h
--- a/include/whisper_mi355x.h
+++ b/include/whisper_mi355x.h
@@ -116,6 +116,9 @@
                                                   const float * ln_b);
 WHISPER_API void whisper_mi355x_set_dec_splits(int splits);
 WHISPER_API void whisper_mi355x_set_dec_bm(int rows);
+WHISPER_API void whisper_mi355x_set_xcomb_form(int form);
+WHISPER_API void whisper_mi355x_set_xstep_pro(int on);
+WHISPER_API void whisper_mi355x_set_self_step(int hpb, int wave_local);
 WHISPER_API void whisper_mi355x_set_pdec_spin(long ticks);
 WHISPER_API void whisper_mi355x_set_pdec_stamps(void * dev);
 WHISPER_API void whisper_mi355x_set_pdec_blocks(int on);
diff --git a/nobs-whisper_amd/csrc/capi.cpp b/nobs-whisper_amd/csrc/capi.cpp
--- a/nobs-whisper_amd/csrc/capi.cpp
+++ b/nobs-whisper_amd/csrc/capi.cpp
@@ -12,6 +12,7 @@
 #include "suppress.h"
 
 namespace wm { extern int g_gemm_variant; extern int g_dec_splits; extern int g_dec_bm; extern unsigned long long* g_gemm_stamps; }
+namespace wm { extern int g_xstep_pro; extern int g_xcomb_form; extern int g_self_hpb; extern int g_self_wl; }
 using namespace wm;
 
 static Context* C(whisper_context* ctx) { return ctx ? &ctx->c : nullptr; }
@@ -584,13 +585,13 @@
 }
 int whisper_mi355x_get_encoder_out(struct whisper_state* s, float* out, int cap) {
     return guarded(nullptr, [&]() -> int {
-        if (!s || !s->ctx || !s->ws.hn || s->last_enc_windows < 1) return -1;
+        if (!s || !s->ctx || !s->last_enc_out || s->last_enc_windows < 1) return -1;
         Context* c = s->ctx;
         const long n = (long)enc_ctx(c, s) * c->hp.n_audio_state;
         if (n > cap) return -1;
         hipSetDevice(c->device);
         std::vector<uint16_t> h(n);
-        WM_CHECK(hipMemcpy(h.data(), s->ws.hn, n * 2, hipMemcpyDeviceToHost));
+        WM_CHECK(hipMemcpy(h.data(), s->last_enc_out, n * 2, hipMemcpyDeviceToHost));
         for (long i = 0; i < n; i++) {
             if (c->dt == DType::F16) out[i] = h2f(h[i]);
             else { uint32_t u = (uint32_t)h[i] << 16; memcpy(&out[i], &u, 4); }
@@ -653,6 +654,9 @@
 void whisper_mi355x_set_gemm_stamps(void* dev) { wm::g_gemm_stamps = (unsigned long long*)dev; }
 void whisper_mi355x_set_dec_splits(int splits) { wm::g_dec_splits = splits; }
 void whisper_mi355x_set_dec_bm(int rows) { wm::g_dec_bm = rows; }
+void whisper_mi355x_set_xcomb_form(int form) { wm::g_xcomb_form = form; }
+void whisper_mi355x_set_xstep_pro(int on) { wm::g_xstep_pro = on; }
+void whisper_mi355x_set_self_step(int hpb, int wave_local) { wm::g_self_hpb = hpb; wm::g_self_wl = wave_local; }
 void whisper_mi355x_set_pdec_spin(long ticks) {
     wm::g_pdec_spin_ticks = ticks;
     wm::g_pdec_gen.fetch_add(1, std::memory_order_release);
diff --git a/nobs-whisper_amd/csrc/engine.cpp b/nobs-whisper_amd/csrc/engine.cpp
--- a/nobs-whisper_amd/csrc/engine.cpp
+++ b/nobs-whisper_amd/csrc/engine.cpp
@@ -162,6 +162,7 @@
     s->align_info.clear();
     s->decoded_tokens = 0;
     s->last_enc_windows = 0;
+    s->last_enc_out = nullptr;
     s->mel_ready = false;
     s->ktime_mask = 0;
     for (auto& k : s->kstat) k = KStat();
@@ -358,6 +359,7 @@
     if (n_enc > w.cap_enc || n_jobs > w.cap_jobs) drop_graphs(s);
     if (!w.deny) dalloc(w.deny, (size_t)suppress_words(hp.n_vocab) * sizeof(uint32_t));
     if (n_enc > w.cap_enc) {
+        s->last_enc_out = nullptr;
         dfree(w.mel_img); dfree(w.h1); dfree(w.hn); dfree(w.qkv); dfree(w.att); dfree(w.ff); dfree(w.x);
         dfree(w.win_job); dfree(w.hs);
         w.cap_enc = 0;
@@ -382,6 +384,7 @@
         const int n_tok = n_jobs * (hp.n_text_ctx / 2 + 8);
         dfree(w.cross); dfree(w.self); dfree(w.dx); dfree(w.dh); dfree(w.dq); dfree(w.datt); dfree(w.dff);
         dfree(w.lrow); dfree(w.logits); dfree(w.probs); dfree(w.tok); dfree(w.ctl); dfree(w.tout); dfree(w.lrec); dfree(w.mel_ptrs);
+        s->last_enc_out = nullptr;
         dfree(w.splitk); dfree(w.enc); dfree(w.qx); dfree(w.xo); dfree(w.xml); dfree(w.kvslot); dfree(w.qtiles);
         free_align(w);
         for (auto& a : s->align_info) a = {};
@@ -746,14 +749,13 @@
             tgemm(s, KCLS, dt, enc_gelu_epi(dt), gemm_plain(w.hn, M, d, Wm.w1, 4 * d, L.b1, w.ff, 4 * d), st);
             tgemm(s, KCLS, dt, EPI_RESID, gemm_plain(w.ff, M, 4 * d, Wm.w2, d, L.b2, w.x, d), st);
         }
-        launch_layernorm(dt, w.x, nullptr, M, d, W.lnpost_w, W.lnpost_b, w.hn, st);
         if (s->direct) {
-            for (int k = 0; k < nb; k++) {
-                WM_CHECK(hipMemcpyAsync((char*)w.enc + (size_t)slots[b0 + k] * T * d * E, (const char*)w.hn + (size_t)k * T * d * E,
-                                        (size_t)T * d * E, hipMemcpyDeviceToDevice, st));
-                w.cross_fresh[slots[b0 + k]] = 0;
-            }
+            launch_layernorm(dt, w.x, nullptr, M, d, W.lnpost_w, W.lnpost_b, w.enc, st, d_slot, T);
+            for (int k = 0; k < nb; k++) w.cross_fresh[slots[b0 + k]] = 0;
+            s->last_enc_out = (const char*)w.enc + (size_t)slots[b0] * T * d * E;
         } else {
+            launch_layernorm(dt, w.x, nullptr, M, d, W.lnpost_w, W.lnpost_b, w.hn, st);
+            s->last_enc_out = w.hn;
             GemmArgs g = gemm_plain(w.hn, M, d, W.wkv_cross, 2 * hp.n_text_layer * d, W.bkv_cross, nullptr, 0);
             g.scale = c->k_scale;
             g.cache = w.cross; g.row_slot = d_slot; g.L = hp.n_text_layer; g.H = hp.n_text_head; g.ctx = hp.n_audio_ctx; g.d = d;
diff --git a/nobs-whisper_amd/csrc/engine.h b/nobs-whisper_amd/csrc/engine.h
--- a/nobs-whisper_amd/csrc/engine.h
+++ b/nobs-whisper_amd/csrc/engine.h
@@ -280,6 +280,7 @@
     std::vector<AlignInfo> align_info;
     long decoded_tokens = 0;
     int last_enc_windows = 0;
+    const void* last_enc_out = nullptr;
     bool mel_ready = false;
     bool pooled = false;
     int ktime_mask = 0;
diff --git a/nobs-whisper_amd/csrc/kernels.h b/nobs-whisper_amd/csrc/kernels.h
--- a/nobs-whisper_amd/csrc/kernels.h
+++ b/nobs-whisper_amd/csrc/kernels.h
@@ -20,7 +20,7 @@
                      int fso, float* const* out, const int* n_out, hipStream_t st);
 
 void launch_layernorm(DType dt, const float* x, const int* rows, int M, int D, const float* w, const float* b,
-                      void* y, hipStream_t st);
+                      void* y, hipStream_t st, const int* out_slot = nullptr, int rpw = 0);
 void launch_embed(DType dt, const void* tok_emb, bool te_f32, const float* pos_emb, const int* tok, const int* pos,
                   int n, int D, float* x, hipStream_t st);
 void launch_embed_ln(DType dt, const void* tok_emb, bool te_f32, const float* pos_emb, const int* tok, const int* pos,
diff --git a/nobs-whisper_amd/csrc/kernels/attn.hip b/nobs-whisper_amd/csrc/kernels/attn.hip
--- a/nobs-whisper_amd/csrc/kernels/attn.hip
+++ b/nobs-whisper_amd/csrc/kernels/attn.hip
@@ -351,7 +351,7 @@
     attn_dec_body<T, true, 1024, 4>(nullptr, 0, sl, cache, slot, n_kv_arr, L, layer, H, ctx, d, out);
 }
 
-template <typename T, int HPB>
+template <typename T, int HPB, bool WL>
 __global__ void __launch_bounds__(64 * HPB) attn_self_step_kernel(const DecSlabs sl, T* __restrict__ cache,
                                                                   const int* __restrict__ slot,
                                                                   const int* __restrict__ pos_arr, int L, int layer,
@@ -361,6 +361,14 @@
     const int lane8 = lane & 7, grp = lane >> 3;
     __shared__ float qs[HPB][64], ks[HPB][64], vs[HPB][64];
     __shared__ float sc[HPB][448];
+    auto sync = [&]() {
+        if constexpr (WL) {
+            asm volatile("s_waitcnt lgkmcnt(0)" ::: "memory");
+            __builtin_amdgcn_wave_barrier();
+        } else {
+            __syncthreads();
+        }
+    };
     const int pos = pos_arr[i];
     const long s = slot[i];
     T* K = cache + (((s * L + layer) * 2 + 0) * H + h) * (long)ctx * 64;
@@ -408,7 +416,7 @@
         ks[w][lane] = (float)tk;
         vs[w][lane] = (float)tv;
     }
-    __syncthreads();
+    sync();
     float qv[8];
 #pragma unroll
     for (int e = 0; e < 8; e++) qv[e] = qs[w][lane8 * 8 + e];
@@ -438,7 +446,7 @@
         lmax = fmaxf(lmax, a);
     }
     for (int o = 32; o > 0; o >>= 1) lmax = fmaxf(lmax, __shfl_xor(lmax, o));
-    __syncthreads();
+    sync();
     const int n_kv = pos + 1;
     float lsum = 0.0f;
     for (int t = lane; t < n_kv; t += 64) {
@@ -449,7 +457,7 @@
     for (int o = 32; o > 0; o >>= 1) lsum += __shfl_xor(lsum, o);
     const float inv = 1.0f / lsum;
     for (int t = lane; t < n_kv; t += 64) sc[w][t] = (float)(T)(sc[w][t] * inv);
-    __syncthreads();
+    sync();
     float acc[8];
 #pragma unroll
     for (int e = 0; e < 8; e++) acc[e] = 0.0f;
@@ -689,15 +697,23 @@
         attn_cross_step_kernel<bf16_t><<<grid, 256, 0, st>>>(sl, (const bf16_t*)cache, slot, n_kv, L, layer, H, ctx, d, (bf16_t*)out);
 }
 
+int g_self_hpb = 0;
+int g_self_wl = -1;
+
 void launch_attn_self_step(DType dt, const DecSlabs& sl, void* cache, const int* slot, const int* pos, int n, int L,
                            int layer, int H, int ctx, int d, void* out, hipStream_t st) {
     if (n <= 0) return;
     if (ctx > 448) WM_FAIL("self-attention context %d > 448", ctx);
     static const int hpb_env = getenv("WHISPER_MI355X_SELF_HPB") ? atoi(getenv("WHISPER_MI355X_SELF_HPB")) : 0;
-    const int want = hpb_env > 0 ? hpb_env : (n <= 32 ? 1 : 4);
+    const int want = g_self_hpb > 0 ? g_self_hpb : hpb_env > 0 ? hpb_env : (n <= 32 ? 1 : 4);
+    static const int wl_env = getenv("WHISPER_MI355X_SELF_WL") ? atoi(getenv("WHISPER_MI355X_SELF_WL")) : 1;
+    const int wl = g_self_wl >= 0 ? g_self_wl : wl_env;
     const int hpb = want >= 4 && H % 4 == 0 ? 4 : want >= 2 && H % 2 == 0 ? 2 : 1;
 #define WM_SELF(TT, HB) \
-    attn_self_step_kernel<TT, HB><<<dim3(n, H / HB), 64 * HB, 0, st>>>(sl, (TT*)cache, slot, pos, L, layer, H, ctx, d, (TT*)out)
+    do { \
+        if (wl) attn_self_step_kernel<TT, HB, true><<<dim3(n, H / HB), 64 * HB, 0, st>>>(sl, (TT*)cache, slot, pos, L, layer, H, ctx, d, (TT*)out); \
+        else attn_self_step_kernel<TT, HB, false><<<dim3(n, H / HB), 64 * HB, 0, st>>>(sl, (TT*)cache, slot, pos, L, layer, H, ctx, d, (TT*)out); \
+    } while (0)
 #define WM_SELF_H(TT) \
     do { if (hpb == 4) WM_SELF(TT, 4); else if (hpb == 2) WM_SELF(TT, 2); else WM_SELF(TT, 1); } while (0)
     if (dt == DType::F16) WM_SELF_H(half_t);
diff --git a/nobs-whisper_amd/csrc/kernels/norm.hip b/nobs-whisper_amd/csrc/kernels/norm.hip
--- a/nobs-whisper_amd/csrc/kernels/norm.hip
+++ b/nobs-whisper_amd/csrc/kernels/norm.hip
@@ -6,7 +6,7 @@
 template <typename T, int NPL>
 __global__ void __launch_bounds__(256) layernorm_kernel(const float* __restrict__ x, const int* __restrict__ rows, int M, int D,
                                                         const float* __restrict__ w, const float* __restrict__ b,
-                                                        T* __restrict__ y) {
+                                                        T* __restrict__ y, const int* __restrict__ oslot, int rpw) {
     const int wave = threadIdx.x >> 6, lane = threadIdx.x & 63;
     const int i = blockIdx.x * 4 + wave;
     if (i >= M) return;
@@ -33,7 +33,8 @@
     for (int o = 32; o > 0; o >>= 1) s2 += __shfl_xor(s2, o);
     const float variance = (float)(s2 / D);
     const float scale = 1.0f / sqrtf(variance + 1e-5f);
-    T* yr = y + (long)i * D;
+    const long ro = oslot ? (long)oslot[i / rpw] * rpw + i % rpw : i;
+    T* yr = y + ro * D;
 #pragma unroll
     for (int e = 0; e < NPL; e++) {
         const int k = lane + 64 * e;
@@ -211,13 +212,14 @@
 }
 
 void launch_layernorm(DType dt, const float* x, const int* rows, int M, int D, const float* w, const float* b, void* y,
-                      hipStream_t st) {
+                      hipStream_t st, const int* out_slot, int rpw) {
     if (M <= 0) return;
+    if (out_slot && rpw <= 0) WM_FAIL("layernorm output slot map needs rows per window");
     const int npl = cdiv(D, 64);
 #define WM_LN(N)                                                                                              \
     if (npl <= N) {                                                                                           \
-        if (dt == DType::F16) layernorm_kernel<half_t, N><<<cdiv(M, 4), 256, 0, st>>>(x, rows, M, D, w, b, (half_t*)y); \
-        else layernorm_kernel<bf16_t, N><<<cdiv(M, 4), 256, 0, st>>>(x, rows, M, D, w, b, (bf16_t*)y);     \
+        if (dt == DType::F16) layernorm_kernel<half_t, N><<<cdiv(M, 4), 256, 0, st>>>(x, rows, M, D, w, b, (half_t*)y, out_slot, rpw); \
+        else layernorm_kernel<bf16_t, N><<<cdiv(M, 4), 256, 0, st>>>(x, rows, M, D, w, b, (bf16_t*)y, out_slot, rpw); \
         return;                                                                                               \
     }
     WM_LN(1) WM_LN(2) WM_LN(4) WM_LN(6) WM_LN(8) WM_LN(12) WM_LN(16) WM_LN(20) WM_LN(24) WM_LN(32)
diff --git a/nobs-whisper_amd/csrc/kernels/xattn.hip b/nobs-whisper_amd/csrc/kernels/xattn.hip
--- a/nobs-whisper_amd/csrc/kernels/xattn.hip
+++ b/nobs-whisper_amd/csrc/kernels/xattn.hip
@@ -20,7 +20,13 @@
     else if constexpr (N == 5) asm volatile("s_waitcnt vmcnt(5)" ::: "memory");
     else if constexpr (N == 6) asm volatile("s_waitcnt vmcnt(6)" ::: "memory");
     else if constexpr (N == 7) asm volatile("s_waitcnt vmcnt(7)" ::: "memory");
-    else asm volatile("s_waitcnt vmcnt(0)" ::: "memory");
+    else if constexpr (N == 8) asm volatile("s_waitcnt vmcnt(8)" ::: "memory");
+    else if constexpr (N == 9) asm volatile("s_waitcnt vmcnt(9)" ::: "memory");
+    else if constexpr (N == 10) asm volatile("s_waitcnt vmcnt(10)" ::: "memory");
+    else {
+        static_assert(N == 0, "no counted wait of this depth");
+        asm volatile("s_waitcnt vmcnt(0)" ::: "memory");
+    }
 }
 __device__ __forceinline__ v4s ds_read_tr(unsigned lds_addr) {
     v4s r;
@@ -113,7 +119,8 @@
 template <typename T, int NW, int CT, int AUX>
 __global__ void __launch_bounds__(NW * 64) xattn_step_kernel(const T* __restrict__ enc, const int* __restrict__ slot,
                                                              const T* __restrict__ qx, int Tn, int splits, float thr,
-                                                             float* __restrict__ opart, float* __restrict__ ml, int ostg = 0) {
+                                                             float* __restrict__ opart, float* __restrict__ ml, int ostg = 0,
+                                                             int pro = 0) {
     typedef typename Frag<T>::type FT;
     typedef __attribute__((address_space(3))) void* lds_ptr_t;
     constexpr int D = NW * CT * 32, H = D / 64, NQ = (2 * H + 15) / 16;
@@ -157,11 +164,15 @@
                 qf[kk][j] = __builtin_bit_cast(
                     FT, hp < 2 * H ? *(const u32x4*)(Q + (long)hp * D + cw + kk * 32 + 8 * (lane >> 4)) : zero);
             }
+    }
+    auto consume_q = [&]() {
 #pragma unroll
         for (int kk = 0; kk < CT; kk++)
 #pragma unroll
             for (int j = 0; j < NQ; j++) asm volatile("" ::"v"(qf[kk][j]));
-    }
+    };
+    if (!pro) consume_q();
+    else asm volatile("" ::: "memory");
     int prow[CT], poff[CT];
 #pragma unroll
     for (int k = 0; k < CT; k++) {
@@ -191,7 +202,13 @@
     const int hh = lane >> 5;
 
     issue(0);
-    if (ntile > 1) issue(1);
+    if (ntile > 1) {
+        issue(1);
+        if (pro) wait_vm<2 * CT>();
+    } else if (pro) {
+        wait_vm<CT>();
+    }
+    if (pro) consume_q();
     for (int t = 0; t < ntile; t++) {
         if (t + 1 < ntile) wait_vm<CT>();
         else wait_vm<0>();
@@ -330,77 +347,94 @@
     }
 }
 
-template <typename T, int TOK, int PF, bool EARLYW>
-__global__ void __launch_bounds__(512) xattn_combine_kernel(const float* __restrict__ opart, const float* __restrict__ ml,
+template <typename T, int TOK, int PF, bool EARLYW, int NWV = 8, int MINW = 1>
+__global__ void __launch_bounds__(NWV * 64, MINW) xattn_combine_kernel(const float* __restrict__ opart, const float* __restrict__ ml,
                                                             int splits, const T* __restrict__ wv, const float* __restrict__ bv,
                                                             int n, int d, int H, T* __restrict__ out) {
     typedef typename Frag<T>::type FT;
     constexpr int DMAX = 1280;
     constexpr int NA = TOK >= 8 ? TOK / 8 : 1, RT = 16 * NA;
     const int h = blockIdx.x, i0 = blockIdx.y * TOK;
-    const int tid = threadIdx.x, wave = tid >> 6, lane = tid & 63;
+    static_assert(NWV == 8 || NWV == 16, "8 k-step waves x 1 or 2 column halves");
+    constexpr int NT = NWV * 64, JW = 4 / (NWV / 8);
+    const int tid = threadIdx.x, wave = tid >> 6 & 7, jb = (tid >> 9) * JW, lane = tid & 63;
     __shared__ __attribute__((aligned(16))) char lds[RT * DMAX * 2 + TOK * 16 * 4];
     T* aimg = (T*)lds;
     float* red = (float*)lds;
     float* wgt = (float*)(lds + RT * DMAX * 2);
     static_assert(8 * RT * 64 * 4 <= RT * DMAX * 2, "reduce image fits the A image");
     auto slot_of = [&](int row, int ch) { return row * d + ((ch & ~15) | ((ch & 15) ^ (row & 15))) * 8; };
-    if (tid < TOK) {
-        const int i = i0 + tid;
-        if (i < n) {
-            const float* p = ml + ((long)i * splits * H + h) * 2;
-            float2 q[16];
-#pragma unroll
-            for (int s = 0; s < 16; s++)
-                if (s < splits) q[s] = *(const float2*)(p + (long)s * H * 2);
-            float M = -INFINITY;
-#pragma unroll
-            for (int s = 0; s < 16; s++)
-                if (s < splits) M = fmaxf(M, q[s].x);
-            float L = 0.0f;
-#pragma unroll
-            for (int s = 0; s < 16; s++)
-                if (s < splits) L += __builtin_amdgcn_exp2f(q[s].x - M) * q[s].y;
-            const float inv = 1.0f / L;
-#pragma unroll
-            for (int s = 0; s < 16; s++)
-                if (s < splits) wgt[tid * 16 + s] = __builtin_amdgcn_exp2f(q[s].x - M) * inv;
-        } else {
-            for (int s = 0; s < splits; s++) wgt[tid * 16 + s] = 0.0f;
-        }
-    }
+    auto weights = [&]() {
+        if (tid < TOK) {
+            const int i = i0 + tid;
+            if (i < n) {
+                const float* p = ml + ((long)i * splits * H + h) * 2;
+                float2 q[16];
+    #pragma unroll
+                for (int s = 0; s < 16; s++)
+                    if (s < splits) q[s] = *(const float2*)(p + (long)s * H * 2);
+                float M = -INFINITY;
+    #pragma unroll
+                for (int s = 0; s < 16; s++)
+                    if (s < splits) M = fmaxf(M, q[s].x);
+                float L = 0.0f;
+    #pragma unroll
+                for (int s = 0; s < 16; s++)
+                    if (s < splits) L += __builtin_amdgcn_exp2f(q[s].x - M) * q[s].y;
+                const float inv = 1.0f / L;
+    #pragma unroll
+                for (int s = 0; s < 16; s++)
+                    if (s < splits) wgt[tid * 16 + s] = __builtin_amdgcn_exp2f(q[s].x - M) * inv;
+            } else {
+                for (int s = 0; s < splits; s++) wgt[tid * 16 + s] = 0.0f;
+            }
+        }
+    };
     constexpr int KMAX = DMAX / 256;
     const int r16 = lane & 15, kq = lane >> 4;
-    FT bfp[KMAX][4];
+    FT bfp[KMAX][JW];
     auto load_wv = [&]() {
 #pragma unroll
         for (int k = 0; k < KMAX; k++) {
             const int ks = wave + 8 * k;
             if (ks < d / 32) {
 #pragma unroll
-                for (int j = 0; j < 4; j++)
-                    bfp[k][j] = __builtin_bit_cast(FT, *(const u32x4*)(wv + ((long)h * 64 + j * 16 + r16) * d + ks * 32 + 8 * kq));
+                for (int j = 0; j < JW; j++)
+                    bfp[k][j] = __builtin_bit_cast(FT, *(const u32x4*)(wv + ((long)h * 64 + (jb + j) * 16 + r16) * d + ks * 32 + 8 * kq));
             }
         }
     };
-    if constexpr (EARLYW) load_wv();
     const int q4 = d / 4;
-    constexpr int NE = (TOK * (DMAX / 4) + 511) / 512;
+    constexpr int NE = (TOK * (DMAX / 4) + NT - 1) / NT;
+    const float* obase = opart + ((long)i0 * splits * H + h) * d;
+    unsigned src[NE];
     float4 a[NE], x[PF][NE];
-    const float* src[NE];
+    auto xload = [&](int u, int s) {
+        const char* sb = (const char*)(obase + (long)s * H * d);
+        asm volatile("" : "+s"(sb));
+#pragma unroll
+        for (int j = 0; j < NE; j++) x[u][j] = *(const float4*)(sb + src[j]);
+    };
 #pragma unroll
     for (int j = 0; j < NE; j++) {
         a[j] = make_float4(0.f, 0.f, 0.f, 0.f);
-        const int e = min(tid + 512 * j, TOK * q4 - 1);
+        const int e = min((int)threadIdx.x + NT * j, TOK * q4 - 1);
         const int t = e / q4, c = (e - t * q4) * 4;
-        src[j] = opart + ((long)min(i0 + t, n - 1) * splits * H + h) * d + c;
-    }
-#pragma unroll
-    for (int u = 0; u < PF; u++)
-        if (u < splits) {
-#pragma unroll
-            for (int j = 0; j < NE; j++) x[u][j] = *(const float4*)(src[j] + (long)u * H * d);
-        }
+        src[j] = (unsigned)((min(i0 + t, n - 1) - i0) * splits * H * d + c) * 4u;
+    }
+    auto issue_x = [&]() {
+#pragma unroll
+        for (int u = 0; u < PF; u++)
+            if (u < splits) xload(u, u);
+    };
+    constexpr bool XFIRST = NWV == 16 || MINW > 1;
+    if constexpr (XFIRST) {
+        issue_x();
+        __builtin_amdgcn_sched_barrier(0);
+    }
+    weights();
+    if constexpr (EARLYW) load_wv();
+    if constexpr (!XFIRST) issue_x();
     __syncthreads();
     for (int s0 = 0; s0 < splits; s0 += PF) {
 #pragma unroll
@@ -409,19 +443,16 @@
             if (s >= splits) break;
 #pragma unroll
             for (int j = 0; j < NE; j++) {
-                const int t = min(tid + 512 * j, TOK * q4 - 1) / q4;
+                const int t = min((int)threadIdx.x + NT * j, TOK * q4 - 1) / q4;
                 const float w = wgt[t * 16 + s];
                 a[j].x += w * x[u][j].x; a[j].y += w * x[u][j].y; a[j].z += w * x[u][j].z; a[j].w += w * x[u][j].w;
             }
-            if (s + PF < splits) {
-#pragma unroll
-                for (int j = 0; j < NE; j++) x[u][j] = *(const float4*)(src[j] + (long)(s + PF) * H * d);
-            }
+            if (s + PF < splits) xload(u, s + PF);
         }
     }
 #pragma unroll
     for (int j = 0; j < NE; j++) {
-        const int e = tid + 512 * j;
+        const int e = threadIdx.x + NT * j;
         if (e >= TOK * q4) break;
         const int t = e / q4, c = (e - t * q4) * 4;
         const float v[4] = {a[j].x, a[j].y, a[j].z, a[j].w};
@@ -437,11 +468,11 @@
     }
     if constexpr (!EARLYW) load_wv();
     __syncthreads();
-    f32x4 acc[NA][4];
+    f32x4 acc[NA][JW];
 #pragma unroll
     for (int a = 0; a < NA; a++)
 #pragma unroll
-        for (int j = 0; j < 4; j++) acc[a][j] = (f32x4){0.f, 0.f, 0.f, 0.f};
+        for (int j = 0; j < JW; j++) acc[a][j] = (f32x4){0.f, 0.f, 0.f, 0.f};
 #pragma unroll
     for (int k = 0; k < KMAX; k++) {
         const int ks = wave + 8 * k;
@@ -450,18 +481,18 @@
         for (int a = 0; a < NA; a++) {
             const FT af = *(const FT*)(aimg + slot_of(a * 16 + r16, ks * 4 + kq));
 #pragma unroll
-            for (int j = 0; j < 4; j++) acc[a][j] = mfma16x16x32(af, bfp[k][j], acc[a][j]);
+            for (int j = 0; j < JW; j++) acc[a][j] = mfma16x16x32(af, bfp[k][j], acc[a][j]);
         }
     }
     __syncthreads();
 #pragma unroll
     for (int a = 0; a < NA; a++)
 #pragma unroll
-        for (int j = 0; j < 4; j++)
-#pragma unroll
-            for (int r = 0; r < 4; r++) red[(wave * RT + a * 16 + 4 * kq + r) * 64 + j * 16 + r16] = acc[a][j][r];
+        for (int j = 0; j < JW; j++)
+#pragma unroll
+            for (int r = 0; r < 4; r++) red[(wave * RT + a * 16 + 4 * kq + r) * 64 + (jb + j) * 16 + r16] = acc[a][j][r];
     __syncthreads();
-    for (int e = tid; e < TOK * 64; e += 512) {
+    for (int e = threadIdx.x; e < TOK * 64; e += NT) {
         const int ti = e >> 6, j = e & 63;
         if (i0 + ti >= n) continue;
         float v = 0.0f;
@@ -470,6 +501,9 @@
         out[(long)(i0 + ti) * d + h * 64 + j] = (T)(v + bv[h * 64 + j]);
     }
 }
+
+int g_xstep_pro = -1;
+int g_xcomb_form = -1;
 
 int xattn_splits(int n, int Tn) {
     const int nn = std::max(1, n);
@@ -502,8 +536,10 @@
                           float* opart, float* ml, hipStream_t st) {
     dim3 grid(splits, n);
     static const int ostg = getenv("WHISPER_MI355X_XSTEP_OSTG") ? atoi(getenv("WHISPER_MI355X_XSTEP_OSTG")) : 1;
+    static const int pro_env = getenv("WHISPER_MI355X_XSTEP_PRO") ? atoi(getenv("WHISPER_MI355X_XSTEP_PRO")) : 1;
+    const int pro = g_xstep_pro >= 0 ? g_xstep_pro : pro_env;
 #define WM_XSTEP(NW_, CT_) \
-    xattn_step_kernel<T, NW_, CT_, 2><<<grid, NW_ * 64, 0, st>>>((const T*)enc, slot, (const T*)qx, Tn, splits, thr, opart, ml, ostg)
+    xattn_step_kernel<T, NW_, CT_, 2><<<grid, NW_ * 64, 0, st>>>((const T*)enc, slot, (const T*)qx, Tn, splits, thr, opart, ml, ostg, pro)
     switch (d) {
         case 384: WM_XSTEP(4, 3); break;
         case 512: WM_XSTEP(8, 2); break;
@@ -532,12 +568,20 @@
     for (int t : {16, 8})
         if (H * cdiv(n, t) >= 160) { tok = t; break; }
     if (tok_env == 4 || tok_env == 8 || tok_env == 16) tok = tok_env;
+    static const int form_env = getenv("WHISPER_MI355X_XCOMB_FORM") ? atoi(getenv("WHISPER_MI355X_XCOMB_FORM")) : 1;
+    int form = g_xcomb_form >= 0 ? g_xcomb_form : (tok == 16 && !tok_env ? form_env : 0);
+    if (form < 0 || form > 2) form = 0;
+    if (form == 1) tok = 16;
+    if (form == 2) tok = 8;
     const dim3 grid(H, cdiv(n, tok));
-#define WM_XCOMB(T_, TOK_, PF_, E_) xattn_combine_kernel<T_, TOK_, PF_, E_><<<grid, 512, 0, st>>>(opart, ml, splits, (const T_*)wv, bv, n, d, H, (T_*)out)
-#define WM_XCOMB_T(T_)                              \
-    if (tok == 4) WM_XCOMB(T_, 4, 2, true);         \
-    else if (tok == 16) WM_XCOMB(T_, 16, 1, false); \
-    else WM_XCOMB(T_, 8, 2, true);
+#define WM_XCOMB(T_, TOK_, PF_, E_, NWV_, MINW_) \
+    xattn_combine_kernel<T_, TOK_, PF_, E_, NWV_, MINW_><<<grid, NWV_ * 64, 0, st>>>(opart, ml, splits, (const T_*)wv, bv, n, d, H, (T_*)out)
+#define WM_XCOMB_T(T_)                                      \
+    if (form == 1) WM_XCOMB(T_, 16, 2, false, 16, 1);       \
+    else if (form == 2) WM_XCOMB(T_, 8, 2, false, 8, 4);    \
+    else if (tok == 4) WM_XCOMB(T_, 4, 2, true, 8, 1);      \
+    else if (tok == 16) WM_XCOMB(T_, 16, 1, false, 8, 1);   \
+    else WM_XCOMB(T_, 8, 2, true, 8, 1);
     if (dt == DType::F16) {
         WM_XCOMB_T(half_t)
     } else {
```
